# maruscia/fastkmer

Hardware: AMD Instinct MI355X
Metric: input bases/sec (whole node), k=28 short reads, 1/2/4/8 GPUs (higher is better)
Workload: dtype u64; 1 GPU; BASELINE configs[1]: k=28 m=10 x=3 B=2048, 1 GB synthetic 100 bp reads per GPU; k=28, m=10, x=3, B=2048, useHT=0, sequenceType=0, fasta_bytes_per_gpu=999999906, bases_per_gpu=877192900, parallelism=one GPU

## Files before the change

fastkmer_amd/__init__.py:

```python
from __future__ import annotations

import ctypes
import dataclasses
import os
import re

import numpy as np

_PKG = os.path.dirname(os.path.abspath(__file__))
LIB_PATH = os.environ.get("FASTKMER_LIB") or os.path.join(_PKG, "lib", "libfastkmer.so")
CLI_PATH = os.path.join(_PKG, "bin", "fastkmer-cli")
HEADER_PATH = os.path.join(os.path.dirname(_PKG), "include", "fastkmer.h")

FK_OK = 0
ERRORS = {-1: "FK_E_INVALID", -2: "FK_E_STATE", -3: "FK_E_DEVICE", -4: "FK_E_NOMEM", -5: "FK_E_IO",
          -6: "FK_E_RANGE", -7: "FK_E_COMM"}
ABI_VERSION = 3


class FastKmerError(RuntimeError):
    def __init__(self, code: int, message: str):
        super().__init__(f"{ERRORS.get(code, code)}: {message}")
        self.code = code

# ... 121 lines not shown
        "fk_bin_sizes_range": (ctypes.c_int, [P, ctypes.c_uint32, ctypes.c_uint32, P]),
        "fk_get_bin_range": (ctypes.c_int, [P, I32, ctypes.c_uint32, ctypes.c_uint32, P, P, SZ,
                                            ctypes.POINTER(SZ)]),
        "fk_write_bins_range": (ctypes.c_int, [P, ctypes.c_char_p, ctypes.c_uint32, ctypes.c_uint32]),
        "fk_compare": (ctypes.c_int, [P, P, P, SZ, SZ]),
        "fk_compare_device": (ctypes.c_int, [P, P, P, SZ, SZ]),
        "fk_bin_sizes_joined": (ctypes.c_int, [P, P, ctypes.c_uint32, ctypes.c_uint32, ctypes.c_uint32,
                                               ctypes.c_uint32, P]),
        "fk_get_bin_joined": (ctypes.c_int, [P, P, I32, ctypes.c_uint32, ctypes.c_uint32, ctypes.c_uint32,
                                             ctypes.c_uint32, P, P, P, SZ, ctypes.POINTER(SZ)]),
        "fk_map_bin_kmers": (ctypes.c_int, [P, P]),
        "fk_lpt_owners": (ctypes.c_int, [P, I32, I32, P]),
        "fk_set_bin_owners": (ctypes.c_int, [P, P, P]),
        "fk_bin_owners": (ctypes.c_int, [P, P]),
        "fk_signature_slots": (U64, [P]),
        "fk_signature_counts": (ctypes.c_int, [P, P, U64]),
        "fk_write_bin_signatures": (ctypes.c_int, [P, P, U64, ctypes.c_char_p]),
        "fk_find_bin_signatures": (ctypes.c_int, [P, ctypes.c_char_p]),
        "fk_comm_unique_id": (ctypes.c_int, [P]),
        "fk_comm_init": (ctypes.c_int, [P, P]),
        "fk_comm_init_local": (ctypes.c_int, [P, I32]),
        "fk_comm_transport": (ctypes.c_char_p, [P]),
        "fk_comm_allreduce_u64": (ctypes.c_int, [P, P, SZ]),
        "fk_balance_bins": (ctypes.c_int, [P, ctypes.c_char_p, SZ]),
        "fk_balance_bins_file": (ctypes.c_int, [P, ctypes.c_char_p, I32, I32, ctypes.c_double]),
        "fk_exchange_plan": (ctypes.c_int, [I32, I32, P, P, U64, P, P, P, P, P]),
        "fk_debug_map_cycles": (ctypes.c_int, [P, I32]),
        "fk_debug_comm_hold": (ctypes.c_int, [P, I32]),
        "fk_debug_comm_release": (ctypes.c_int, [P]),
        "fk_debug_comm_held": (ctypes.c_int, [P]),
        "fk_debug_fingerprint_bits": (ctypes.c_int, [I32, I32]),
        "fk_debug_wave_count": (ctypes.c_int, [I32, I32, I32, ctypes.c_uint32, ctypes.c_uint32, I32, P,
                                               ctypes.c_uint32, P, P, P]),
    }
    for name, (res, args) in sig.items():
        fn = getattr(L, name)
        fn.restype = res
        fn.argtypes = args
    if L.fk_abi_version() != ABI_VERSION:
        raise RuntimeError(f"{LIB_PATH} has ABI version {L.fk_abi_version()}, this binding mirrors {ABI_VERSION}: "
                           "rebuild it (python -m fastkmer_amd.build)")
    _lib = L
    return L


def _check(rc: int) -> None:
    if rc != FK_OK:
        raise FastKmerError(rc, lib().fk_last_error().decode(errors="replace"))


def make_config(k: int, m: int, x: int = 3, B: int = 2048, use_ht: bool = False, sequence_type: int = 0,
                write: bool = False, n_ranks: int = 1, rank: int = 0, device: int = -1) -> fk_config:
    c = fk_config()
    lib().fk_config_init(ctypes.byref(c))
    c.k, c.m, c.x, c.B = k, m, x, B
    c.use_ht, c.sequence_type, c.write = int(bool(use_ht)), sequence_type, int(bool(write))
    c.n_ranks, c.rank, c.device = n_ranks, rank, device
    return c


def validate(**kw) -> None:
    c = make_config(**kw)
    _check(lib().fk_config_validate(ctypes.byref(c)))


def clamped_bins(m: int, B: int) -> int:
# ... 505 lines not shown
            return ""
        return "".join(lines) + ("" if self.use_ht else "EOF")

    def write_bins(self, out_dir: str, min_count: int = 1, max_count: int | None = None) -> None:
        rg = _count_range(min_count, max_count)
        if rg is None:
            _check(lib().fk_write_bins(self._h, out_dir.encode()))
        else:
            _check(lib().fk_write_bins_range(self._h, out_dir.encode(), rg[0], rg[1]))

    def signature_counts(self, out=None):
        import torch
        n = lib().fk_signature_slots(self._h)
        if out is None:
            out = torch.empty(n, dtype=torch.int64, device=self._torch_device())
        if out.numel() < n or out.dtype != torch.int64 or not out.is_cuda or not out.is_contiguous():
            raise ValueError(f"signature counts need a contiguous device int64 tensor of {n} entries")
        _check(lib().fk_signature_counts(self._h, ctypes.c_void_p(out.data_ptr()), out.numel()))
        return out

    def write_bin_signatures(self, counts, out_dir: str) -> None:
        _check(lib().fk_write_bin_signatures(self._h, ctypes.c_void_p(counts.data_ptr()), counts.numel(),
                                             out_dir.encode()))

    def _torch_device(self):
        import torch
        return torch.device("cuda", self._device if self._device >= 0 else torch.cuda.current_device())

    def stats(self) -> dict:
        st = fk_stats()
        _check(lib().fk_get_stats(self._h, ctypes.byref(st)))
        return {n: getattr(st, n) for n, _ in fk_stats._fields_}


def debug_wave_count(keys: np.ndarray, k: int, F: int, c0: int, c1: int, slots: int, device: int = 0):
    kw = 1 if k <= 32 else 2
    keys = np.ascontiguousarray(keys, dtype=np.uint64).reshape(-1, kw)
    n = len(keys)
    ok = np.zeros(n * kw, dtype=np.uint64)
    oc = np.zeros(n, dtype=np.uint32)
    nout = ctypes.c_uint32(0)
    _check(lib().fk_debug_wave_count(device, k, F, c0, c1, slots, keys.ctypes.data, n, ok.ctypes.data,
                                     oc.ctypes.data, ctypes.byref(nout)))
    u = nout.value
    return (ok[:u] if kw == 1 else ok[:2 * u].reshape(-1, 2)), oc[:u]


def comm_unique_id() -> bytes:
    buf = ctypes.create_string_buffer(COMM_ID_BYTES)
    _check(lib().fk_comm_unique_id(buf))
    return buf.raw


def comm_init_local(counters) -> None:
    arr = (ctypes.c_void_p * len(counters))(*[c._h.value for c in counters])
    _check(lib().fk_comm_init_local(arr, len(counters)))


def exchange_plan(sent, received, record_bytes: int):
    snd = np.ascontiguousarray(sent, dtype=np.uint64)
    rcv = np.ascontiguousarray(received, dtype=np.uint64)
    if snd.ndim != 2 or snd.shape != rcv.shape or snd.shape[1] % 2 != 1:
        raise ValueError("sent / received must be [n_ranks, 2 * parts + 1] arrays of one shape")
    n, parts = snd.shape[0], (snd.shape[1] - 1) // 2
    so, sb, ro, rb = (np.zeros(n, dtype=np.uint64) for _ in range(4))
    fin = ctypes.c_int32(0)
    _check(lib().fk_exchange_plan(n, parts, snd.ctypes.data, rcv.ctypes.data, record_bytes, so.ctypes.data,
                                  sb.ctypes.data, ro.ctypes.data, rb.ctypes.data, ctypes.byref(fin)))
    return so, sb, ro, rb, bool(fin.value)


def lpt_owners(sizes, n_ranks: int) -> np.ndarray:
    sz = np.ascontiguousarray(sizes, dtype=np.uint64)
    owner = np.zeros(len(sz), dtype=np.int32)
    _check(lib().fk_lpt_owners(sz.ctypes.data, len(sz), n_ranks, owner.ctypes.data))
    return owner
# ... 26 lines not shown
```

fastkmer_amd/csrc/fk_api.cpp:

```cpp
#include <errno.h>
#include <fcntl.h>
#include <unistd.h>
#include <stdarg.h>
#include <stdio.h>
#include <string.h>
#include <sys/stat.h>

#include <unordered_map>
#include <chrono>
#include <cstdlib>
#include <cstring>
#include <thread>

#include "fk_ctx.h"
#include "fk_split.h"

static thread_local std::string g_err;
int fk::set_err(int code, const char *fmt, ...) {
    char buf[1024];
    va_list ap;
    va_start(ap, fmt);
    vsnprintf(buf, sizeof(buf), fmt, ap);
    va_end(ap);
    g_err = buf;
// ... 198 lines not shown
    c->Bc = clamp_bins(cfg->m, cfg->B);
    c->G = (uint32_t)cfg->n_ranks;
    c->nlb = (uint32_t)((c->Bc - cfg->rank + (int)c->G - 1) / (int)c->G);
    if (cfg->rank >= c->Bc) c->nlb = 0;
    c->W = cfg->k <= 32 ? 2 : 3;
    c->KW = cfg->k <= 32 ? 1 : 2;
    c->fm = make_fastmod((uint32_t)c->Bc);
    auto env = [](const char *name) -> const char * {
        const char *v = getenv(name);
        return v && v[0] ? v : nullptr;
    };
    if (const char *v = env("FASTKMER_PIECE_BYTES")) {
        c->piece_bytes = std::max(1ull << 16, strtoull(v, nullptr, 10));
        c->piece_bytes_set = true;
    }
    if (const char *v = env("FASTKMER_PIECE_CUTS")) {
        c->st_cuts.clear();
        c->xst_cuts.clear();
        for (const char *q = v; *q;) {
            char *e = nullptr;
            const double f = strtod(q, &e);
            if (e == q) break;
            if (f > 0.0 && f < 1.0 && c->st_cuts.size() < STAGE_MAXP - 1) c->st_cuts.push_back(f), c->xst_cuts.push_back(f);
            c->cuts_env = true;
            q = *e == ',' ? e + 1 : e;
        }
    }
    if (const char *v = env("FASTKMER_INGEST_SEG")) c->ingest_seg = std::max(1ull << 16, strtoull(v, nullptr, 10));
    if (const char *v = env("FASTKMER_DEBUG_LARGE_BUCKETS")) c->force_large = v[0] == '1';
    if (const char *v = env("FASTKMER_DEBUG_CELL_TARGET")) c->cell_target = (uint32_t)atoi(v);
    if (const char *v = env("FASTKMER_DEBUG_MID_PARTS")) c->mid_parts = atoi(v);
    if (const char *v = env("FASTKMER_DEBUG_SPLIT_RETRY")) c->split_retry = v[0] == '1';
    if (const char *v = env("FASTKMER_DEBUG_SPECTRUM_WIDE")) c->spectrum_wide = v[0] == '1';
    if (const char *v = env("FASTKMER_X2_L1")) c->x2_l1 = atoi(v);
    if (const char *v = env("FASTKMER_FUSED")) c->fused = atoi(v);
#ifdef FK_PROBES
    if (const char *v = env("FASTKMER_DEBUG_PHASE")) c->dbg_phase = atoi(v);
    if (const char *v = env("FASTKMER_FUSED_PROBE")) c->fused_probe = atoi(v);
    if (const char *v = env("FASTKMER_SPLIT_MAP")) c->split_map = atoi(v);
#endif
    if (cfg->device >= 0) {
        if (cfg->device >= ndev) {
            delete c;
            return set_err(FK_E_DEVICE, "device %d out of range (%d devices)", cfg->device, ndev);
        }
        c->device = cfg->device;
    } else {
        (void)hipGetDevice(&c->device);
    }
    DeviceGuard dg_(c->device);
    {
        int cur = -1;
        if (hipGetDevice(&cur) != hipSuccess || cur != c->device) {
            (void)hipGetLastError();
            delete c;
            return set_err(FK_E_DEVICE, "cannot select device %d", c->device);
        }
    }
    e = hipStreamCreateWithFlags(&c->stream, hipStreamNonBlocking);
    if (e != hipSuccess) {
        delete c;
        return set_err(FK_E_DEVICE, "hipStreamCreate: %s", hipGetErrorString(e));
    }
    c->own_stream = true;
    e = hipStreamCreateWithFlags(&c->copy_stream, hipStreamNonBlocking);
    if (e == hipSuccess) e = hipEventCreateWithFlags(&c->seg_ev, hipEventDisableTiming);
// ... 40 lines not shown
FK_EXPORT void fk_destroy(fk_ctx *c) {
    if (!c) return;
    DeviceGuard dg_(c->device);
    if (c->hold_flag) __atomic_store_n(c->hold_flag, 1u, __ATOMIC_RELEASE);
    if (c->copy_stream) (void)hipStreamSynchronize(c->copy_stream);
    if (c->stream) (void)hipStreamSynchronize(c->stream);
    if (c->xstage) (void)hipStreamSynchronize(c->xstage);
    if (c->tier_side) (void)hipStreamSynchronize(c->tier_side);
    DevBuf *bufs[] = {&c->fasta_own, &c->tile_last_nl, &c->tile_off,
                      &c->npos_dev, &c->codes, &c->valid, &c->records, &c->counters, &c->sig_status, &c->sig_kmers, &c->tcnt, &c->rec_hdr, &c->rec_pos, &c->rec_code, &c->tstat, &c->map_vslots,
                      &c->precs, &c->chunks, &c->bin_chunk_begin, &c->hpieces, &c->hpiece_first, &c->hpiece_tot, &c->chunk_nk, &c->grp_table,
                      &c->chunk_base, &c->lp, &c->scratch,
                      &c->cell_total, &c->cell_base, &c->flags, &c->flag_scan, &c->buckets, &c->keys,
                      &c->out_keys, &c->out_counts, &c->bucket_unique, &c->dense_off, &c->dense_keys,
                      &c->dense_counts, &c->bin_off, &c->misc, &c->tier_list, &c->mid, &c->sc_total,
                      &c->sp_base, &c->sp_keys, &c->sp_subs, &c->sp_par, &c->sp_fb, &c->mid_fb};
    for (DevBuf *b : bufs) release(*b);
    c->vw.release_all();
    release(c->fq_ws);
    release(c->fq_info);
    for (auto &e : c->fq_evs)
        if (e) (void)hipEventDestroy(e);
    c->fq_pin.release();
    for (int i = 0; i < 2; ++i) {
        if (c->pinned[i]) (void)hipHostFree(c->pinned[i]);
        if (c->pin_ev[i]) (void)hipEventDestroy(c->pin_ev[i]);
    }
    if (c->comm_stream) (void)hipStreamSynchronize(c->comm_stream);
    delete c->comm;
    c->comm = nullptr;
    c->pin_up.release();
    c->pin_down.release();
    c->pin_tier.release();
    c->file_pin[0].release();
    c->file_pin[1].release();
    if (c->tier_ev) (void)hipEventDestroy(c->tier_ev);
    if (c->pin_up_ev) (void)hipEventDestroy(c->pin_up_ev);
    if (c->cmp_ev) (void)hipEventDestroy(c->cmp_ev);
    if (c->hold_flag) (void)hipHostFree(c->hold_flag);
    release(c->xsend);
    release(c->xrecv);
    for (auto &e : c->xev)
        if (e) (void)hipEventDestroy(e);
    for (auto &e : c->seg_evs)
        if (e) (void)hipEventDestroy(e);
    for (auto &e : c->map_evs)
        if (e) (void)hipEventDestroy(e);
    if (c->emit_ev) (void)hipEventDestroy(c->emit_ev);
    if (c->comm_stream) (void)hipStreamDestroy(c->comm_stream);
    if (c->xstage) (void)hipStreamSynchronize(c->xstage), (void)hipStreamDestroy(c->xstage);
    if (c->xstage_ev) (void)hipEventDestroy(c->xstage_ev);
    if (c->ws_x.ptr) (void)hipFree(c->ws_x.ptr);
    c->dest.release_all();
    c->part.release_all();
    c->binhist.release_all();
    release(c->d_owner);
    release(c->d_local);
    if (c->ws.ptr) (void)hipFree(c->ws.ptr);
    for (auto &ev : c->ev)
        if (ev) (void)hipEventDestroy(ev);
    for (auto &ev : c->st_ev)
        if (ev) (void)hipEventDestroy(ev);
    for (int p = 0; p < STAGE_MAXP; ++p) release(c->st_keys[p]), release(c->st_cb[p]);
    release(c->st_total);
    release(c->piece_starts);
    if (c->seg_ev) (void)hipEventDestroy(c->seg_ev);
    for (auto &ev : c->h2d_ev)
        if (ev) (void)hipEventDestroy(ev);
    if (c->tier_side) (void)hipStreamSynchronize(c->tier_side), (void)hipStreamDestroy(c->tier_side);
    for (auto &ev : c->side_ev)
        if (ev) (void)hipEventDestroy(ev);
    if (c->copy_stream) (void)hipStreamDestroy(c->copy_stream);
    if (c->own_stream && c->stream) (void)hipStreamDestroy(c->stream);
    delete c;
}

FK_EXPORT int fk_set_stream(fk_ctx *c, void *s) {
    if (!c) return set_err(FK_E_INVALID, "null ctx");
    DeviceGuard dg_(c->device);
    if (c->own_stream && c->stream) {
        (void)hipStreamSynchronize(c->stream);
        (void)hipStreamDestroy(c->stream);
    }
    c->stream = (hipStream_t)s;
    c->own_stream = false;
    return FK_OK;
}

FK_EXPORT size_t fk_record_bytes(const fk_ctx *c) { return c ? (size_t)c->W * 8 : 0; }
FK_EXPORT int32_t fk_num_bins(const fk_ctx *c) { return c ? c->Bc : 0; }

static void reset_results(fk_ctx *c) {
    c->mapped = false;
    c->have_result = false;
    c->gapped = c->dense_ready = false;
    c->distinct = 0;
    c->h_bin_off.clear();
// ... 1022 lines not shown
};

static hipError_t launch_wave_tier(const BucketCount &t, hipStream_t s) {
    if (t.c->KW == 1)
        return launch_bucket_count64_wave(t.src, t.buckets(), t.nbuckets, t.k, t.out_keys(), t.out_counts(), t.unique(),
                                          nullptr, s, t.ordered);
    return launch_bucket_count128_wave(t.src, t.buckets(), t.nbuckets, t.k, t.out_keys(), t.out_counts(), t.unique(), s,
                                       t.ordered);
}
static hipError_t launch_wave_mid(const BucketCount &t, const uint32_t *list, uint32_t n, hipStream_t s) {
    if (t.c->KW == 1)
        return launch_bucket_count64_wave_mid(t.src, t.buckets(), list, n, t.k, t.out_keys(), t.out_counts(), t.unique(),
                                              s, t.ordered);
    return launch_bucket_count128_wave_mid(t.src, t.buckets(), list, n, t.k, t.out_keys(), t.out_counts(), t.unique(), s,
                                           t.ordered);
}
static hipError_t launch_split(const BucketCount &t, const uint32_t *l1, uint32_t nl, SubBucket *subs,
                               unsigned int *counts, uint32_t *fb, hipStream_t s) {
    fk_ctx *c = t.c;
    return launch_bucket_split64(t.src, t.buckets(), t.lists, 0, l1, nl, c->sp_base.as<uint64_t>(),
                                 c->sp_keys.as<uint64_t>(), subs, c->sp_par.as<SplitParent>(), counts, fb, fb + nl,
                                 t.cap, t.k, t.src.F, s, c->split_retry);
}
static hipError_t launch_split(const BucketCount &t, const uint32_t *l1, uint32_t nl, SubBucket128 *subs,
                               unsigned int *counts, uint32_t *fb, hipStream_t s) {
    fk_ctx *c = t.c;
    return launch_bucket_split128(t.src, t.buckets(), l1, nl, c->sp_base.as<uint64_t>(), c->sp_keys.as<uint64_t>(), subs,
                                  c->sp_par.as<SplitParent>(), counts, fb, fb + nl, t.cap, t.k, t.src.F, s,
                                  c->split_retry);
}
static hipError_t launch_sub_count_seq(const BucketCount &t, const uint32_t *l1, uint32_t nl, const SubBucket *subs,
                                       hipStream_t s) {
    return launch_sub_count64_seq(t.buckets(), l1, nl, t.c->sp_par.as<SplitParent>(), subs, t.c->sp_keys.as<uint64_t>(),
                                  t.out_keys(), t.out_counts(), t.unique(), s, t.ordered);
}
static hipError_t launch_sub_count_seq(const BucketCount &t, const uint32_t *l1, uint32_t nl, const SubBucket128 *subs,
                                       hipStream_t s) {
    return launch_sub_count128_seq(t.buckets(), l1, nl, t.c->sp_par.as<SplitParent>(), subs, t.c->sp_keys.as<uint64_t>(),
                                   t.out_keys(), t.out_counts(), t.unique(), s, t.ordered);
}

static int block_tier(const BucketCount &t, const uint32_t *list, uint32_t n, hipStream_t s) {
    fk_ctx *c = t.c;
    if (c->KW == 1)
        HIP_TRY(launch_bucket_count64(t.src, t.buckets(), n, t.k, t.out_keys(), t.out_counts(), t.unique(),
                                      c->misc.as<unsigned long long>() + 1, t.cap, 99, list, s, 0));
    else
        HIP_TRY(launch_bucket_sort(2, t.src, t.buckets(), n, t.k, t.out_keys(), t.out_counts(), t.unique(),
                                   c->misc.as<unsigned long long>() + 1, t.cap, list, s, 0));
    return FK_OK;
}

static int bucket_cut(BucketCount &t, const SortedPlan &pl, uint64_t total_kmers, const uint64_t *cell_total,
                      const uint64_t *cell_base) {
    fk_ctx *c = t.c;
    const CountBufs &B = t.B;
    const hipStream_t cs = t.cut.s;
    const int F = pl.F;
    const uint32_t cap = pl.cap;
    const uint64_t ncell_all = (uint64_t)c->nlb << F;
    FK_TRY(ensure(*B.flags, ncell_all * 4));
    FK_TRY(ensure(*B.flag_scan, (ncell_all + 1) * 8));
    FK_TRY(ensure(c->misc, 64));
    if (pl.tiered)
        HIP_TRY(launch_bucket_flags_greedy(cell_total, c->nlb, F, pl.wave_cap, -1, B.flags->as<uint32_t>(), cs));
    else
        HIP_TRY(launch_bucket_flags(cell_base, cell_total, c->nlb, F, cap / 4, cap - cap / 4, B.flags->as<uint32_t>(), cs));
    HIP_TRY(scan_excl_sum_u32_to_u64(B.flags->as<uint32_t>(), B.flag_scan->as<uint64_t>(), ncell_all,
                                     B.flag_scan->as<uint64_t>() + ncell_all, *t.cut.ws, cs));
    uint64_t nbuckets = 0;
    HIP_TRY(hipMemcpyAsync(&nbuckets, B.flag_scan->as<uint64_t>() + ncell_all, 8, hipMemcpyDeviceToHost, cs));
    HIP_TRY(hipStreamSynchronize(cs));
    htrace("sorted: nbuckets read");
    t.nbuckets = nbuckets;
    FK_TRY(ensure(*B.buckets, nbuckets * sizeof(Bucket)));
    FK_TRY(ensure(t.okb, total_kmers * 8 * c->KW));
    FK_TRY(ensure(*B.out_counts, total_kmers * 4));
    FK_TRY(ensure(*B.bucket_unique, (nbuckets + 1) * 8));
    HIP_TRY(launch_bucket_write(cell_base, B.flags->as<uint32_t>(), B.flag_scan->as<uint64_t>(), c->nlb, F, nbuckets,
                                total_kmers, B.buckets->as<Bucket>(), cs));
    BucketSrc &src = t.src;
    src.F = F;
    if (src.np > 0) FK_TRY(ensure(*B.piece_starts, nbuckets * sizeof(PieceStarts)));
    HIP_TRY(launch_bucket_finish(src, B.buckets->as<Bucket>(), nbuckets, c->nlb, total_kmers,
                                 src.np > 0 ? B.piece_starts->as<PieceStarts>() : nullptr, cs));
    if (src.np > 0) src.starts = B.piece_starts->as<PieceStarts>();
    HIP_TRY(hipMemsetAsync(c->misc.p, 0, 64, cs));
    c->stats.buckets = nbuckets;
    c->stats.fine_bits = (uint64_t)F;
    c->stats.heavy_keys = 0;
    c->stats.split_buckets = c->stats.sub_buckets = 0;
    return FK_OK;
}

static int wave_tier(BucketCount &t, uint32_t wave_cap) {
    fk_ctx *c = t.c;
    const hipStream_t s = t.s.s, cs = t.cut.s, hs = t.heavy.s;
    FK_TRY(ensure(*t.B.tier_list, t.nbuckets * 8));
    t.lists = t.B.tier_list->as<uint32_t>();
    HIP_TRY(launch_bucket_tiers(t.buckets(), t.nbuckets, wave_cap, t.mid_cap(), t.unique(), t.lists,
                                c->misc.as<unsigned int>(), c->misc.as<unsigned long long>() + 3, cs));
    if (c->pin_tier.ensure(64)) return set_err(FK_E_NOMEM, "hipHostMalloc failed");
    HIP_TRY(hipMemcpyAsync(c->pin_tier.p, c->misc.p, 32, hipMemcpyDeviceToHost, cs));
    HIP_TRY(hipEventRecord(c->tier_ev, cs));
    if (cs != s) {
        HIP_TRY(hipEventRecord(c->side_ev[0], cs));
        HIP_TRY(hipStreamWaitEvent(s, c->side_ev[0], 0));
    }
    HIP_TRY(hipEventRecord(c->side_ev[3], s));
    HIP_TRY(hipStreamWaitEvent(hs, c->side_ev[3], 0));
    HIP_TRY(launch_wave_tier(t, s));
    HIP_TRY(hipEventSynchronize(c->tier_ev));
    t.ntier[0] = c->pin_tier.as<uint32_t>()[0], t.ntier[1] = c->pin_tier.as<uint32_t>()[1];
    t.listed_keys = c->pin_tier.as<uint64_t>()[3];
    htrace("sorted: tiers read");
    c->stats.heavy_keys = t.listed_keys;
    c->stats.block_buckets = t.ntier[0];
// ... 430 lines not shown
    c->have_result = false;
    const uint32_t nlb = c->nlb;
    if ((uint32_t)parts_per_seg < nlb) return set_err(FK_E_INVALID, "%d parts per segment < %u local bins",
                                                      parts_per_seg, nlb);
    HIP_TRY(hipEventRecord(c->ev[4], s));
    std::vector<std::vector<std::pair<uint64_t, uint64_t>>> ranges(nlb);
    std::vector<uint64_t> bkm(nlb, 0);
    uint64_t off = 0;
    for (int32_t sg = 0; sg < nseg; ++sg) {
        for (int32_t lb = 0; lb < parts_per_seg; ++lb) {
            const uint64_t n = seg_records[(uint64_t)sg * parts_per_seg + lb];
            if (n && (uint32_t)lb >= nlb) return set_err(FK_E_INVALID, "records for local bin %d of %u", lb, nlb);
            if (n) {
                ranges[lb].push_back({off, off + n});
                bkm[lb] += seg_kmers[(uint64_t)sg * parts_per_seg + lb];
            }
            off += n;
        }
    }
    if (off != nrecv)
        return set_err(FK_E_INVALID, "segment table holds %llu records, buffer %llu", (unsigned long long)off,
                       (unsigned long long)nrecv);
    return reduce_ranges(c, (const uint64_t *)d_recv, nrecv, ranges, bkm, t0);
}


static void pieces_reset(fk_ctx *c) {
    c->st_np = 0;
    c->st_cut = 0;
    c->st_kmers = 0;
    c->pieces_void = false;
    c->tiles_counted = 0;
    c->segs_counted = 0;
}

static uint32_t stage_maxp(const fk_ctx *c) { return c->KW == 2 ? (uint32_t)STAGE_MAXP128 : (uint32_t)STAGE_MAXP; }
static const std::vector<double> &local_cuts(const fk_ctx *c) {
    if (!c->cuts_env && c->KW == 1 && c->job_bytes >= (4ull << 30) && STAGE_MAXP >= 5) return c->st_cuts5;
    return c->st_cuts;
}

static bool staged_eligible(const fk_ctx *c) { return staged_ok(c) && c->G == 1 && !c->comm; }

static int staged_expand_chunks(fk_ctx *c, StreamWs on, hipStream_t cut, uint32_t nchunks,
                                const std::vector<uint64_t> &bkm, double frac) {
    hipStream_t s = on.s;
    const uint32_t p = c->st_np;
    uint64_t pk = 0, maxb = 0;
    for (uint64_t v : bkm) pk += v, maxb = std::max(maxb, v);
    if (pk == 0) return FK_OK;
    if (p == 0) {
        const double scale = frac > 0.0 ? std::max(1.0, 1.0 / frac) : 2.0;
        c->st_plan = sorted_plan(c, (uint64_t)((double)maxb * scale));
        if (!c->st_plan.tiered || !c->st_plan.two_level)
            return set_err(FK_E_STATE, "staged pieces need the tiered two-level count");
    }
    SortedPlan pl = c->st_plan;
    HIP_TRY(hipEventRecord(c->st_ev[4 * p + 2], s));
    FK_TRY(sorted_expand(c, on, cut, pl, nchunks, pk, c->st_keys[p], c->st_cb[p]));
    const uint64_t ncell_all = (uint64_t)c->nlb << c->st_plan.F;
    FK_TRY(ensure(c->st_total, ncell_all * 8));
    if (cut) {
        HIP_TRY(hipStreamWaitEvent(cut, c->side_ev[2], 0));
        HIP_TRY(launch_add_u64(c->st_total.as<uint64_t>(), c->cell_total.as<uint64_t>(), ncell_all, p == 0, cut));
    } else {
        HIP_TRY(launch_add_u64(c->st_total.as<uint64_t>(), c->cell_total.as<uint64_t>(), ncell_all, p == 0, s));
// ... 2 lines not shown
    c->st_kmers += pk;
    c->st_np = p + 1;
    htrace("staged: piece expanded");
    return FK_OK;
}

static int staged_expand(fk_ctx *c, StreamWs on, hipStream_t cut, const RecSrc &src, double frac) {
    const uint32_t p = c->st_np;
    if (p >= stage_maxp(c)) return set_err(FK_E_STATE, "more than %u staged pieces", stage_maxp(c));
    uint64_t nrecv = 0;
    std::vector<Chunk> chunks;
    std::vector<uint32_t> bcb;
    std::vector<uint64_t> bkm;
    FK_TRY(partition_src(c, on, src, nrecv, chunks, bcb, bkm, c->st_ev[4 * p], c->st_ev[4 * p + 1]));
    return staged_expand_chunks(c, on, cut, (uint32_t)chunks.size(), bkm, frac);
}

static int staged_count(fk_ctx *c, hipStream_t cut) {
    const double t0 = now_ms();
    const StreamWs on = c->main_on();
    hipStream_t s = on.s;
    const SortedPlan pl = c->st_plan;
    const uint32_t nlb = c->nlb;
    const uint64_t ncell_all = (uint64_t)nlb << pl.F;
    HIP_TRY(hipEventRecord(c->ev[6], s));
    std::swap(c->cell_total, c->st_total);
    FK_TRY(ensure(c->cell_base, (ncell_all + 1) * 8));
    const hipStream_t cs = cut ? cut : s;
    if (cut) HIP_TRY(hipStreamWaitEvent(cut, c->side_ev[2], 0));
    HIP_TRY(scan_excl_sum_u64(c->cell_total.as<uint64_t>(), c->cell_base.as<uint64_t>(), ncell_all,
                              c->cell_base.as<uint64_t>() + ncell_all, *on.ws, cs));
    BucketSrc src{nullptr, pl.F};
    src.np = (int)c->st_np;
    for (uint32_t p = 0; p < c->st_np; ++p) {
        src.pk[p] = c->st_keys[p].as<uint64_t>();
        src.pcb[p] = c->st_cb[p].as<uint64_t>();
    }
    FK_TRY(sorted_count(c, on, cut, pl, src, c->st_kmers));
    HIP_TRY(hipEventRecord(c->ev[7], s));
    FK_TRY(read_bin_offsets(c, s));
    htrace("staged: bin offsets read");
    double mp = 0.0, mx = 0.0;
    for (uint32_t p = 0; p < c->st_np; ++p) {
        mp += ev_ms(c->st_ev[4 * p], c->st_ev[4 * p + 1]);
        mx += ev_ms(c->st_ev[4 * p + 2], c->st_ev[4 * p + 3]);
    }
    c->stats.ms_partition = mp;
    c->stats.ms_count = mx + ev_ms(c->ev[6], c->ev[7]);
    c->stats.pieces_counted = c->st_np;
    count_done(c, c->nrec, t0);
    return FK_OK;
}

static bool local_piece_due(const fk_ctx *c, uint64_t tiles) {
    constexpr uint64_t MIN_PIECE = 256ull << 20;
    if (c->st_np >= stage_maxp(c) - 1) return false;
    const uint64_t tile = fm_tile_bytes(FUSED_NT);
    if (c->job_bytes && !c->piece_bytes_set) {
        const std::vector<double> &cuts = local_cuts(c);
        if (c->job_bytes < 2 * MIN_PIECE || c->st_cut >= cuts.size()) return false;
        const uint64_t end = (uint64_t)(cuts[c->st_cut] * (double)c->job_bytes);
        return tiles * tile >= end && (tiles - c->tiles_counted) * tile >= MIN_PIECE / 2;
    }
    return c->st_np < 3 && (tiles - c->tiles_counted) * tile >= c->piece_bytes;
}

static int local_maybe_piece(fk_ctx *c, uint64_t tiles, hipEvent_t mapped) {
    if (!staged_eligible(c) || c->pieces_void || !local_piece_due(c, tiles)) return FK_OK;
    const StreamWs on = c->stage_on();
    hipStream_t s = on.s;
    HIP_TRY(hipStreamWaitEvent(s, mapped, 0));
    uint64_t h[4] = {0, 0, 0, 0};
    HIP_TRY(hipMemcpyAsync(h, c->counters.p, 32, hipMemcpyDeviceToHost, s));
    HIP_TRY(hipStreamSynchronize(s));
    if (h[2]) {
        c->pieces_void = true;
        return FK_OK;
    }
    const uint64_t t0 = c->tiles_counted, nt = tiles - t0;
    const RecSrc src = fused_src(c, t0, nt, nt * map_fused_tcap());
    c->tiles_counted = tiles;
    c->st_cut += 1;
    FK_TRY(staged_expand(c, on, nullptr, src,
                         c->job_bytes ? (double)(nt * fm_tile_bytes(FUSED_NT)) / (double)c->job_bytes : 0.0));
    HIP_TRY(hipEventRecord(c->xstage_ev, s));
    return FK_OK;
}


enum : uint64_t { XF_FINAL = 1, XF_RETRACT = 2 };

static int plan_step(uint32_t G, uint32_t L, const uint64_t *sent, const uint64_t *got, uint64_t rb, uint64_t *soff,
                     uint64_t *sbytes, uint64_t *roff, uint64_t *rbytes, bool *all_final) {
    const size_t msg = 2 * (size_t)L + 1;
    uint64_t so = 0, ro = 0;
    bool fin = true;
    for (uint32_t d = 0; d < G; ++d) {
        uint64_t ns = 0, nr = 0;
        for (uint32_t lb = 0; lb < L; ++lb) {
            ns += sent[d * msg + lb];
            nr += got[d * msg + lb];
        }
        const uint64_t fs = sent[d * msg + 2 * L], fr = got[d * msg + 2 * L];
        if ((fs | fr) & ~(XF_FINAL | XF_RETRACT)) return set_err(FK_E_INVALID, "exchange step: unknown flag bits");
        if ((fr & XF_RETRACT) && !(fr & XF_FINAL))
            return set_err(FK_E_INVALID, "exchange step: rank %u retracts outside its last piece", d);
        fin = fin && (fr & XF_FINAL);
        soff[d] = so;
        sbytes[d] = ns * rb;
        roff[d] = ro;
        rbytes[d] = nr * rb;
        so += ns * rb;
        ro += nr * rb;
    }
    *all_final = fin;
    return FK_OK;
}
// ... 296 lines not shown
}

static int finish_local(fk_ctx *c);

FK_EXPORT int fk_finish(fk_ctx *c) {
    htrace("fk_finish: enter");
    if (!c) return set_err(FK_E_INVALID, "null ctx");
    if (c->comm) {
        DeviceGuard dg_(c->device);
        const int rc = finish_exchange(c);
        return rc ? comm_fail(c, rc) : rc;
    }
    return note_held(c, finish_local(c));
}

static int finish_local(fk_ctx *c) {
    if (c->G != 1)
        return set_err(FK_E_STATE, "fk_finish over %u ranks needs a communicator (fk_comm_init); or use "
                                   "fk_map/fk_map_emit/fk_reduce", c->G);
    FK_TRY(fk_map(c, nullptr));
    DeviceGuard dg_(c->device);
    if (c->st_np && c->rec_tiled && !c->pieces_void && c->tiles_counted <= c->rec_tiles) {
        int rc = FK_OK;
        const hipStream_t cut = c->rec_tiles > c->tiles_counted ? c->tier_side : nullptr;
        if (cut) HIP_TRY(hipEventRecord(c->side_ev[2], c->stream));
        if (c->rec_tiles > c->tiles_counted) {
            const uint64_t t0 = c->tiles_counted, nt = c->rec_tiles - t0;
            rc = staged_expand(c, c->main_on(), cut, fused_src(c, t0, nt, nt * map_fused_tcap()),
                               c->job_bytes ? (double)(nt * fm_tile_bytes(FUSED_NT)) / (double)c->job_bytes : 0.0);
        }
        if (rc == FK_OK) rc = staged_count(c, cut);
        if (cut) (void)hipStreamSynchronize(cut);
        FK_TRY(rc);
        pieces_reset(c);
        return FK_OK;
    }
    pieces_reset(c);
    return reduce_src(c, map_src(c));
}

static int attach_comm(fk_ctx *c, fk::Comm *comm) {
    DeviceGuard dg_(c->device);
    if (!c->comm_stream) HIP_TRY(hipStreamCreateWithFlags(&c->comm_stream, hipStreamNonBlocking));
    if (!c->xstage) HIP_TRY(hipStreamCreateWithFlags(&c->xstage, hipStreamNonBlocking));
    if (!c->xstage_ev) HIP_TRY(hipEventCreateWithFlags(&c->xstage_ev, hipEventDisableTiming));
    if (!c->emit_ev) HIP_TRY(hipEventCreateWithFlags(&c->emit_ev, hipEventDisableTiming));
    c->comm = comm;
    if (!c->piece_bytes_set) c->piece_bytes = 1ull << 30;
    FK_TRY(fk_set_grouped_emit(c, 1));
    xch_reset(c);
    return FK_OK;
}

FK_EXPORT int fk_comm_unique_id(uint8_t *id) {
    if (!id) return set_err(FK_E_INVALID, "null argument");
    std::string err;
    if (fk::comm_unique_id(id, err)) return set_err(FK_E_DEVICE, "%s", err.c_str());
    return FK_OK;
}

FK_EXPORT int fk_comm_init(fk_ctx *c, const uint8_t *id) {
    if (!c || !id) return set_err(FK_E_INVALID, "null argument");
    if (c->comm) return set_err(FK_E_STATE, "the context already has a communicator");
    DeviceGuard dg_(c->device);
    std::string err;
    fk::Comm *comm = fk::comm_create_rccl(id, (int)c->G, c->cfg.rank, c->device, err);
    if (!comm) return set_err(FK_E_DEVICE, "%s", err.c_str());
    const int rc = attach_comm(c, comm);
    if (rc) {
// ... 160 lines not shown
    }
    __atomic_store_n(c->hold_flag, 0u, __ATOMIC_RELEASE);
    void *dflag = nullptr;
    HIP_TRY(hipHostGetDevicePointer(&dflag, c->hold_flag, 0));
    int khz = 0;
    HIP_TRY(hipDeviceGetAttribute(&khz, hipDeviceAttributeWallClockRate, c->device));
    const uint64_t ticks = (uint64_t)max_seconds * (uint64_t)std::max(khz, 100000) * 1000ull;
    const hipStream_t cs2 = c->comm->counts_stream();
    for (hipStream_t st : {c->comm_stream, cs2})
        if (st) HIP_TRY(launch_hold_stream(static_cast<const uint32_t *>(dflag), ticks, st));
    return FK_OK;
}

FK_EXPORT int fk_debug_fingerprint_bits(int32_t device, int32_t bits) {
    DeviceGuard dg_(device);
    HIP_TRY(set_fingerprint_bits(bits));
    return FK_OK;
}

FK_EXPORT int fk_debug_comm_held(fk_ctx *c) {
    if (!c || !c->comm_stream) return 0;
    DeviceGuard dg_(c->device);
    const hipError_t e = hipStreamQuery(c->comm_stream);
    if (e != hipErrorNotReady) (void)hipGetLastError();
    return e == hipErrorNotReady ? 1 : 0;
}

FK_EXPORT int fk_debug_comm_release(fk_ctx *c) {
    if (!c) return set_err(FK_E_INVALID, "null ctx");
    if (c->hold_flag) __atomic_store_n(c->hold_flag, 1u, __ATOMIC_RELEASE);
    return FK_OK;
}

FK_EXPORT int fk_debug_wave_count(int32_t device, int32_t k, int32_t F, uint32_t c0, uint32_t c1, int32_t slots,
                                  const uint64_t *keys, uint32_t n, uint64_t *out_keys, uint32_t *out_counts,
                                  uint32_t *n_out) {
    if (!keys || !out_keys || !out_counts || !n_out || k < 1 || k > 63 || F < 1 || F > MAX_FINE_BITS || c1 <= c0 ||
        c1 > (1u << F))
        return set_err(FK_E_INVALID, "bad argument");
    const int KW = k <= 32 ? 1 : 2;
    const uint32_t cap = KW == 1 ? WAVE_BUCKET_CAP : WAVE128_BUCKET_CAP;
    if (n == 0 || n > cap) return set_err(FK_E_RANGE, "a wave bucket holds 1..%u keys", cap);
    if (slots != (int32_t)(KW == 1 ? WAVE_SLOTS : 384))
        return set_err(FK_E_INVALID, "slots: %u (k <= 32) or 384 (k > 32)", WAVE_SLOTS);
    const int sh = 2 * k - F;
    for (uint32_t i = 0; i < n; ++i) {
        const uint64_t hi = KW == 1 ? 0 : keys[2 * i], lo = KW == 1 ? keys[i] : keys[2 * i + 1];
        const uint64_t cell = sh >= 64 ? (hi >> (sh - 64)) : (sh == 0 ? lo : ((hi << (64 - sh)) | (lo >> sh)));
        if ((KW == 1 && k < 32 && (lo >> (2 * k)) != 0) || cell < c0 || cell >= c1)
            return set_err(FK_E_RANGE, "key %u lies outside cells [%u, %u)", i, c0, c1);
    }
    DeviceGuard dg_(device);
    TempBuf dk, dok, doc, du, db;
    FK_TRY(ensure(dk, (uint64_t)n * 8 * KW));
    FK_TRY(ensure(dok, (uint64_t)n * 8 * KW));
    FK_TRY(ensure(doc, (uint64_t)n * 4));
    FK_TRY(ensure(du, 16));
    FK_TRY(ensure(db, sizeof(Bucket)));
    const Bucket b{0, n, 0, c0, c1};
    int rc = FK_OK;
    hipError_t e = hipMemcpy(dk.p, keys, (uint64_t)n * 8 * KW, hipMemcpyHostToDevice);
    if (e == hipSuccess) e = hipMemcpy(db.p, &b, sizeof(Bucket), hipMemcpyHostToDevice);
    if (e == hipSuccess)
        e = KW == 1 ? launch_bucket_count64_wave(BucketSrc{dk.as<uint64_t>(), F}, db.as<Bucket>(), 1, k, dok.as<uint64_t>(),
                                                 doc.as<uint32_t>(), du.as<uint64_t>(), nullptr, nullptr)
                    : launch_bucket_count128_wave(BucketSrc{dk.as<uint64_t>(), F}, db.as<Bucket>(), 1, k, dok.as<uint64_t>(),
                                                  doc.as<uint32_t>(), du.as<uint64_t>(), nullptr);
    uint64_t U = 0;
    if (e == hipSuccess) e = hipMemcpy(&U, du.p, 8, hipMemcpyDeviceToHost);
    if (e == hipSuccess && U <= n) e = hipMemcpy(out_keys, dok.p, U * 8 * KW, hipMemcpyDeviceToHost);
    if (e == hipSuccess && U <= n) e = hipMemcpy(out_counts, doc.p, U * 4, hipMemcpyDeviceToHost);
    if (e != hipSuccess) rc = set_err(FK_E_DEVICE, "%s", hipGetErrorString(e));
    else if (U > n) rc = set_err(FK_E_INVALID, "bucket reported %llu distinct keys of %u", (unsigned long long)U, n);
    *n_out = (uint32_t)U;
    return rc;
}

FK_EXPORT int fk_debug_map_cycles(uint64_t *out16, int32_t reset) {
    if (!out16) return set_err(FK_E_INVALID, "null argument");
    const hipError_t e = map_fused_cycles(reinterpret_cast<unsigned long long *>(out16), reset != 0);
    if (e == hipErrorNotSupported) {
        (void)hipGetLastError();
        return set_err(FK_E_STATE, "phase stamps exist only in a library built with -DFK_PROBES");
    }
    HIP_TRY(e);
    return FK_OK;
}

FK_EXPORT int fk_get_stats(fk_ctx *c, fk_stats *out) {
    if (!c || !out) return set_err(FK_E_INVALID, "null argument");
    *out = c->stats;
    return FK_OK;
}


FK_EXPORT uint64_t fk_signature_slots(const fk_ctx *c) { return c ? (1ull << (2 * c->cfg.m)) + 1ull : 0ull; }

FK_EXPORT int fk_signature_counts(fk_ctx *c, void *d_counts, uint64_t n_counts) {
    if (!c || !d_counts) return set_err(FK_E_INVALID, "null argument");
    DeviceGuard dg_(c->device);
    const uint64_t slots = fk_signature_slots(c);
    if (n_counts < slots)
        return set_err(FK_E_RANGE, "signature counts hold %llu entries, need 4^m + 1 = %llu",
                       (unsigned long long)n_counts, (unsigned long long)slots);
    if (c->pm_active && !c->pm_last_seen)
        return set_err(FK_E_STATE, "fk_signature_counts inside a streamed input: finish it with fk_ingest(..., last = 1)");
    hipStream_t s = c->stream;
    const uint64_t n = c->d_fasta ? c->n_fasta : 0;
// ... 102 lines not shown
```

fastkmer_amd/csrc/fk_count_sorted.inc:

```


struct ExpandLds {
    uint64_t s0[NT], s1[NT], s2[NT];
    uint32_t first[NT];
    uint8_t owner[NT / 64][64 * SIG_PPT];
};

template <int W, int KW, typename Fn>
__device__ __forceinline__ void for_each_chunk_kmer(const uint64_t *__restrict__ rec, const Chunk &ch, int k,
                                                    ExpandLds &e, Fn fn) {
    const int lane = threadIdx.x & 63, wid = threadIdx.x >> 6;
    const uint64_t nrec = ch.rec_end - ch.rec_begin;
    const uint64_t rounds = (nrec + NT - 1) / NT;
    for (uint64_t rd = 0; rd < rounds; ++rd) {
        const uint64_t i = ch.rec_begin + rd * NT + threadIdx.x;
        uint32_t n = 0;
        if (i < ch.rec_end) {
            RecView<W> r;
            r.load(rec, i);
            n = r.n;
            e.s0[threadIdx.x] = r.s0;
            e.s1[threadIdx.x] = r.s1;
            if (W == 3) e.s2[threadIdx.x] = r.s2;
        }
// ... 360 lines not shown
    }
    const uint64_t g0 = ((uint64_t)b.lbin << src.F) + b.c0, g1 = ((uint64_t)b.lbin << src.F) + b.c1;
    uint32_t acc = 0;
#pragma unroll
    for (int q = 0; q < NPC; ++q) {
        if (q == 0 || q < src.np) {
            const uint64_t s0 = src.pcb[q][g0], s1 = src.pcb[q][g1];
            v.b[q] = src.pk[q] + KW * ((int64_t)s0 - (int64_t)acc);
            v.p[q] = q ? acc : 0u;
            acc += (uint32_t)(s1 - s0);
        } else {
            v.b[q] = v.b[q - 1];
            v.p[q] = ~0u;
        }
    }
    return v;
}

template <int KW = 1>
__device__ __forceinline__ BucketView bucket_view_starts(const BucketSrc &src, const PieceStarts &ps) {
    BucketView v;
    v.b[0] = src.pk[0] + KW * ps.s[0];
    v.p[0] = 0;
#pragma unroll
    for (int q = 1; q < stage_npc<KW>(); ++q) {
        v.b[q] = src.pk[q] + KW * ((int64_t)ps.s[q] - (int64_t)ps.pre[q]);
        v.p[q] = ps.pre[q];
    }
    return v;
}

template <bool PIECES>
__global__ __launch_bounds__(NT) void k_bucket_finish(BucketSrc src, Bucket *__restrict__ buckets, uint64_t nb,
                                                      uint32_t nlbins, uint64_t total_keys,
                                                      PieceStarts *__restrict__ out) {
    const uint64_t i = (uint64_t)blockIdx.x * NT + threadIdx.x;
    const bool mine = i < nb;
    const uint32_t ncell = 1u << src.F;
    Bucket b{};
    uint64_t e_beg = total_keys, g1 = (uint64_t)nlbins << src.F;
    if (mine) {
        b = buckets[i];
        if (i + 1 < nb) {
            const Bucket nx = buckets[i + 1];
            e_beg = nx.begin;
            g1 = ((uint64_t)nx.lbin << src.F) + nx.c0;
        }
        buckets[i].n = (uint32_t)(e_beg - b.begin);
        buckets[i].c1 = (g1 >> src.F) == b.lbin ? (uint32_t)(g1 & (ncell - 1)) : ncell;
    }
    if constexpr (PIECES) {
        const uint64_t g0 = ((uint64_t)b.lbin << src.F) + b.c0;
        const bool own_end = (threadIdx.x & 63) == 63 || i + 1 >= nb;
        PieceStarts ps;
        uint32_t acc = 0;
#pragma unroll
        for (int p = 0; p < STAGE_MAXP; ++p) {
            if (p < src.np) {
                const uint64_t s0 = mine ? src.pcb[p][g0] : 0;
                uint64_t s1 = (uint64_t)__shfl_down((long long)s0, 1, 64);
                if (mine && own_end) s1 = src.pcb[p][g1];
                ps.s[p] = s0;
                ps.pre[p] = acc;
                acc += (uint32_t)(s1 - s0);
            } else {
                ps.s[p] = 0;
                ps.pre[p] = ~0u;
            }
        }
        if (mine) out[i] = ps;
    }
}

hipError_t launch_bucket_finish(const BucketSrc &src, Bucket *buckets, uint64_t nb, uint32_t nlbins,
                                uint64_t total_keys, PieceStarts *out, hipStream_t s) {
    if (!nb) return hipSuccess;
    const unsigned grid = (unsigned)((nb + NT - 1) / NT);
    if (src.np > 0)
        k_bucket_finish<true><<<grid, NT, 0, s>>>(src, buckets, nb, nlbins, total_keys, out);
    else
        k_bucket_finish<false><<<grid, NT, 0, s>>>(src, buckets, nb, nlbins, total_keys, out);
    return hipGetLastError();
}


template <class T>
__device__ __forceinline__ T ldg_nt(const void *p) {
    typedef const __attribute__((address_space(1))) T *gp;
    return __builtin_nontemporal_load((gp)(uintptr_t)p);
}


template <int KW = 1>
__device__ __forceinline__ const uint64_t *bucket_key_ptr(const BucketView &v, uint32_t i) {
    uintptr_t a = (uintptr_t)v.b[0] + (uintptr_t)i * (8u * KW);
#pragma unroll
    for (int q = 1; q < stage_npc<KW>(); ++q) a += i >= v.p[q] ? (uintptr_t)v.b[q] - (uintptr_t)v.b[q - 1] : 0;
    return reinterpret_cast<const uint64_t *>(a);
}

struct RowBases {
    uintptr_t base;
    uint64_t inner;
};
template <int KW = 1>
__device__ __forceinline__ RowBases row_bases(const BucketView &v, uint32_t first_row = 0) {
    const uint32_t r0 = (first_row + (threadIdx.x & 63)) * 64u;
    uintptr_t a = (uintptr_t)v.b[0];
    bool inner = false;
#pragma unroll
    for (int q = 1; q < stage_npc<KW>(); ++q) {
        a = r0 >= v.p[q] ? (uintptr_t)v.b[q] : a;
        inner = inner || (r0 < v.p[q] && r0 + 63u >= v.p[q]);
    }
    return RowBases{a, __ballot(inner)};
}
template <int KW = 1>
__device__ __forceinline__ const uint64_t *row_key_ptr(const BucketView &v, const RowBases &rb, int row, uint32_t i) {
    if ((rb.inner >> row) & 1ull) return bucket_key_ptr<KW>(v, i);
    const uint32_t lo = (uint32_t)__builtin_amdgcn_readlane((int)(uint32_t)rb.base, row);
    const uint32_t hi = (uint32_t)__builtin_amdgcn_readlane((int)(uint32_t)((uint64_t)rb.base >> 32), row);
    return reinterpret_cast<const uint64_t *>((((uint64_t)hi << 32) | lo) + (uintptr_t)i * (8u * KW));
}

constexpr int GB = 8;



constexpr uint32_t HCAP = 2048;
constexpr uint32_t HSLOTS = 2 * HCAP;
constexpr uint32_t HSPT = HSLOTS / NT;
constexpr int UIPT = HCAP / NT;
constexpr uint32_t RANK_MAX = HCAP - 3 * NT / 2 - 2;
constexpr uint64_t REDO = ~0ull;
constexpr uint64_t EMPTY_KEY = ~0ull;
constexpr uint32_t BLOCK_SPLIT_GROUP = 64;

__device__ __forceinline__ uint32_t hslot(uint64_t key) {
    return (uint32_t)((key * 0x9e3779b97f4a7c15ull) >> 52) & (HSLOTS - 1);
}

template <uint32_t HC, uint32_t HS, bool STREAM = false>
__global__ __launch_bounds__(NT) void k_bucket_count64(BucketSrc src, const Bucket *__restrict__ buckets, int k,
                                                       uint64_t *__restrict__ out_keys,
                                                       uint32_t *__restrict__ out_counts, uint64_t *bucket_unique,
                                                       unsigned long long *oversize, uint32_t small_limit,
                                                       int dbg_phase, const uint32_t *__restrict__ list,
                                                       uint32_t skip_le = 0) {
    constexpr uint32_t HSPT_ = HS / NT;
    constexpr int UIPT_ = HC / NT;
    constexpr uint32_t RANK_MAX_ = (HC < HS - HC ? HC : HS - HC) - 3 * NT / 2 - 2;
    static_assert(HC <= 65535 && 2 * HC <= HS + HS / 2 && HS % NT == 0, "u16 counts, load <= 3/4");
    static_assert((HS - HC) * 8 >= 16 * NT * 4 && HC % NT == 0, "radix counters (tile_rank) fit above HC");
    constexpr bool POW2 = (HS & (HS - 1)) == 0;
    constexpr int HBITS = __builtin_ctz(HS);
    __shared__ unsigned long long s_k[HS];
    __shared__ uint16_t s_c[HS];
    __shared__ uint32_t s_tmp[NT / 64];
    uint32_t *const s_cnt = reinterpret_cast<uint32_t *>(&s_k[HC]);
    __shared__ uint64_t s_red[2][NT / 64];
    static_assert(!STREAM || HS - HC >= NT * GB, "a batch of new keys leaves the table below full");
    __shared__ uint32_t s_nu, s_ovf;
    __shared__ unsigned long long s_spl[NT];
    const uint32_t qi = list ? list[blockIdx.x] : blockIdx.x;
    const Bucket b = buckets[qi];
    if (b.n <= skip_le) return;
    const BucketView bv = bucket_view(src, b);
    if (!STREAM && (b.n > HC || b.n > small_limit)) {
        if (threadIdx.x == 0) {
            bucket_unique[qi] = REDO;
            atomicAdd(oversize, 1ull);
        }
        return;
    }
    if (b.n == 0) {
        if (threadIdx.x == 0) bucket_unique[qi] = 0;
        return;
    }
    for (uint32_t s = threadIdx.x; s < HS; s += NT) {
        s_k[s] = EMPTY_KEY;
        s_c[s] = 0;
    }
    if (STREAM && threadIdx.x == 0) s_nu = 0, s_ovf = 0;
    __syncthreads();
    for (uint32_t i0 = 0; i0 < b.n; i0 += NT * GB) {
        if constexpr (STREAM) {
            if (i0) {
                __syncthreads();
                if (s_ovf || s_nu > HC) {
                    if (threadIdx.x == 0) atomicAdd(oversize, 1ull);
                    return;
                }
            }
        }
        uint64_t kk[GB];
#pragma unroll
        for (int q = 0; q < GB; ++q) {
            const uint32_t i = i0 + q * NT + threadIdx.x;
            kk[q] = i < b.n ? *bucket_key_ptr(bv, i) : EMPTY_KEY;
        }
        if (dbg_phase == 0) {
            uint64_t acc = 0;
#pragma unroll
            for (int q = 0; q < GB; ++q) acc += kk[q];
            if (acc == 42) out_counts[b.begin] = 1;
            continue;
        }
#pragma unroll
        for (int q = 0; q < GB; ++q) {
            const uint64_t key = kk[q];
            if (key == EMPTY_KEY) continue;
            uint32_t s = POW2 ? (uint32_t)((key * 0x9e3779b97f4a7c15ull) >> (64 - HBITS))
                              : (uint32_t)((((key * 0x9e3779b97f4a7c15ull) >> 32) * HS) >> 32);
            for (;;) {
                unsigned long long cur = s_k[s];
                if (cur == EMPTY_KEY) cur = atomicCAS(&s_k[s], EMPTY_KEY, (unsigned long long)key);
                if (cur == EMPTY_KEY || cur == key) {
                    const uint32_t old =
                        atomicAdd(reinterpret_cast<uint32_t *>(&s_c[s & ~1u]), 1u << (16 * (s & 1u)));
                    if constexpr (STREAM) {
                        if (cur == EMPTY_KEY) atomicAdd(&s_nu, 1u);
                        if (((old >> (16 * (s & 1u))) & 0xffffu) == 0xffffu) s_ovf = 1u;
                    }
                    break;
                }
                s = POW2 ? (s + 1) & (HS - 1) : (s + 1 == HS ? 0u : s + 1);
            }
        }
    }
    if (dbg_phase < 99 && threadIdx.x == 0) bucket_unique[qi] = 0;
    if (dbg_phase == 0) return;
    __syncthreads();
    if constexpr (STREAM) {
        if (s_ovf || s_nu > HC) {
            if (threadIdx.x == 0) atomicAdd(oversize, 1ull);
            return;
        }
    }
    if (dbg_phase == 1) return;
    uint64_t tk[HSPT_];
    uint16_t tc[HSPT_];
    uint32_t occ = 0;
#pragma unroll
    for (uint32_t q = 0; q < HSPT_; ++q) {
        tk[q] = s_k[q * NT + threadIdx.x];
        tc[q] = s_c[q * NT + threadIdx.x];
        occ += tk[q] != EMPTY_KEY;
    }
    uint32_t U;
    uint32_t u = block_excl_sum<uint32_t>(occ, s_tmp, &U);
#pragma unroll
    for (uint32_t q = 0; q < HSPT_; ++q) {
        if (tk[q] != EMPTY_KEY) {
            s_k[u] = tk[q];
            s_c[u] = tc[q];
// ... 352 lines not shown
    for (uint32_t p = lane; p < U; p += 64) {
        const unsigned long long kx = s_gk[p];
        const uint32_t g = (uint32_t)((kx - lo) >> gsh);
        const uint32_t gv = s_grp[g], n = gv >> 16;
        if (n > RANK_BIG) continue;
        const uint32_t g1 = gv & 0xffffu, g0 = g1 - n;
        uint32_t r = g0;
        for (uint32_t j = g0; j < g1; j += 4) {
            const unsigned long long a0 = s_gk[j], a1 = s_gk[j + 1], a2 = s_gk[j + 2], a3 = s_gk[j + 3];
            r += (uint32_t)(a0 < kx) + (uint32_t)(j + 1 < g1 && a1 < kx) + (uint32_t)(j + 2 < g1 && a2 < kx) +
                 (uint32_t)(j + 3 < g1 && a3 < kx);
        }
        out_keys[begin + r] = kx;
        out_counts[begin + r] = s_gc[p];
#ifdef FK_PROBES
        it += g1 - g0;
        uint32_t w = g1 - g0;
#pragma unroll
        for (int d = 32; d > 0; d >>= 1) w = max(w, (uint32_t)__shfl_xor((int)w, d, 64));
        wall += w;
#endif
    }
#ifdef FK_PROBES
    it = wave_incl_sum<uint32_t>(it);
    if (lane == 63) {
        atomicAdd(&g_rank_probe[0], (unsigned long long)it);
        atomicAdd(&g_rank_probe[1], (unsigned long long)U);
        atomicAdd(&g_rank_probe[2], 1ull);
        atomicAdd(&g_rank_probe[3], (unsigned long long)wall);
    }
#endif
}

template <uint32_t CAP, uint32_t SL, bool ORD = true, int WKPT = WaveCfg<CAP>::KPT, int NROW = WKPT>
__device__ __forceinline__ uint32_t wave_count_keys(WaveLds<CAP, SL> &w, uint64_t begin, uint32_t n, uint64_t lo,
                                                int span_bits, uint64_t q, const uint64_t (&kk)[NROW],
                                                uint64_t *__restrict__ out_keys, uint32_t *__restrict__ out_counts,
                                                uint64_t *__restrict__ uniq) {
    const int lane = threadIdx.x & 63;
    unsigned long long *s_k = w.k;
    uint16_t *s_c = w.c;
    uint16_t *s_list = w.list;
    if (n == 0) {
        if (lane == 0 && uniq) uniq[q] = 0;
        return 0;
    }
    {
        ulonglong2 *k2 = reinterpret_cast<ulonglong2 *>(s_k);
#pragma unroll
        for (uint32_t r = 0; r < (SL / 2 + 63) / 64; ++r)
            if (r * 64 + lane < SL / 2) k2[r * 64 + lane] = make_ulonglong2(EMPTY_KEY, EMPTY_KEY);
        uint4 *c4 = reinterpret_cast<uint4 *>(s_c);
#pragma unroll
        for (uint32_t r = 0; r < (SL / 8 + 63) / 64; ++r)
            if (r * 64 + lane < SL / 8) c4[r * 64 + lane] = make_uint4(0, 0, 0, 0);
    }
    wave_lds_sync();
    static_assert(NROW == WKPT || (NROW > WKPT && SL - CAP >= 64), "a row's new keys fit above CAP");
    uint32_t sl[NROW];
#pragma unroll
    for (int j = 0; j < NROW; ++j) sl[j] = wslot<SL>(kk[j]);
    uint32_t U = 0;
#pragma unroll
    for (int j = 0; j < NROW; ++j) {
        bool over = false;
        if constexpr (NROW > WKPT) over = U > CAP;
        const uint64_t key = over ? EMPTY_KEY : kk[j];
        bool fresh = false;
        if (key != EMPTY_KEY) {
            uint32_t s = sl[j];
            for (;;) {
                const unsigned long long prev = atomicCAS(&s_k[s], EMPTY_KEY, (unsigned long long)key);
                fresh = prev == EMPTY_KEY;
                if (fresh || prev == key) break;
                s = s + 1 == SL ? 0u : s + 1;
            }
            atomicAdd(reinterpret_cast<uint32_t *>(&s_c[s & ~1u]), 1u << (16 * (s & 1u)));
            sl[j] = s;
        }
        const uint64_t m = __ballot(fresh);
        if (fresh) {
            const uint32_t at = U + __builtin_amdgcn_mbcnt_hi((uint32_t)(m >> 32), __builtin_amdgcn_mbcnt_lo((uint32_t)m, 0u));
            if (NROW == WKPT || at < CAP) s_list[at] = (uint16_t)sl[j];
        }
        U += (uint32_t)__popcll(m);
    }
    wave_lds_sync();
    if constexpr (NROW > WKPT) {
        if (U > CAP) return ~0u;
    }
#if defined(FK_W64_STOP) && FK_W64_STOP == 1
    if (lane == 0 && uniq) uniq[q] = U;
    return U;
#endif
    uint64_t tk[WKPT];
    uint16_t tc[WKPT];
#pragma unroll
    for (int j = 0; j < WKPT; ++j) {
        const uint32_t i = j * 64 + lane;
        if (i < U) {
            const uint32_t s = s_list[i];
            tk[j] = s_k[s];
            tc[j] = s_c[s];
        }
    }
#if defined(FK_W64_STOP) && FK_W64_STOP == 2
    {
        uint64_t x = 0;
#pragma unroll
        for (int j = 0; j < WKPT; ++j) x ^= (j * 64 + lane < (int)U) ? tk[j] + tc[j] : 0ull;
        if (x == 0x0123456789abcdefull) out_counts[0] = 1u;
        if (lane == 0 && uniq) uniq[q] = U;
        wave_lds_sync();
        return U;
    }
#endif
    if constexpr (!ORD) {
#pragma unroll
        for (int j = 0; j < WKPT; ++j) {
            const uint32_t i = j * 64 + lane;
            if (i < U) {
                out_keys[begin + i] = tk[j];
                out_counts[begin + i] = tc[j];
            }
        }
        if (lane == 0 && uniq) uniq[q] = U;
        wave_lds_sync();
        return U;
    }
    wave_rank64<CAP, WKPT>(s_k, s_c, reinterpret_cast<uint32_t *>(&s_k[CAP]), reinterpret_cast<uint32_t *>(s_list),
                           U, tk, tc, lo, span_bits, begin, out_keys, out_counts);
    if (lane == 0 && uniq) uniq[q] = U;
    wave_lds_sync();
    return U;
}

template <uint32_t CAP, uint32_t SL, bool ORD = true, int WKPT = WaveCfg<CAP>::KPT>
__device__ __forceinline__ void wave_count_bucket(WaveLds<CAP, SL> &w, const Bucket &b, uint64_t q,
                                                  const uint64_t (&kk)[WKPT], int k, int F,
                                                  uint64_t *__restrict__ out_keys, uint32_t *__restrict__ out_counts,
                                                  uint64_t *__restrict__ bucket_unique) {
    const int sh = 2 * k - F;
    const int span_bits = b.n ? (32 - __builtin_clz(b.c1 - b.c0)) + sh : 0;
    wave_count_keys<CAP, SL, ORD, WKPT>(w, b.begin, b.n, (uint64_t)b.c0 << sh, span_bits, q, kk, out_keys,
                                        out_counts, bucket_unique);
}

template <int BPW, uint32_t CAP, uint32_t SL, bool MS = false, bool ORD = true>
__global__ __launch_bounds__(64) void k_bucket_count64_wave(BucketSrc src,
                                                            const Bucket *__restrict__ buckets, uint64_t nbuckets,
                                                            int k, uint64_t *__restrict__ out_keys,
                                                            uint32_t *__restrict__ out_counts,
                                                            uint64_t *__restrict__ bucket_unique,
                                                            const uint32_t *__restrict__ list) {
    constexpr int WKPT = WaveCfg<CAP>::KPT;
    __shared__ __attribute__((aligned(16))) WaveLds<CAP, SL> w;
    const uint64_t q0 = (uint64_t)blockIdx.x * BPW;
    Bucket b[BPW];
    bool mine[BPW];
    uint64_t qq[BPW];
    uint64_t kk[BPW][WKPT];
    const uint64_t *dummy = reinterpret_cast<const uint64_t *>(buckets);
#pragma unroll
    for (int t = 0; t < BPW; ++t) {
        const uint64_t i = q0 + t;
        qq[t] = i < nbuckets ? (list ? (uint64_t)list[i] : i) : 0;
        if (i < nbuckets) b[t] = buckets[qq[t]];
        PieceStarts ps{};
        if constexpr (MS)
            if (src.starts && i < nbuckets) ps = src.starts[qq[t]];
        mine[t] = i < nbuckets && b[t].n <= CAP;
        wave_bucket_load<CAP, MS>(src, b[t], ps, mine[t], kk[t], dummy);
    }
#if defined(FK_W64_STOP) && FK_W64_STOP == 0
    if (!list) {
#pragma unroll
        for (int t = 0; t < BPW; ++t) {
            uint64_t x = 0;
#pragma unroll
            for (int j = 0; j < WKPT; ++j) x ^= kk[t][j];
            if ((threadIdx.x & 63) == 0 && bucket_unique && mine[t]) bucket_unique[qq[t]] = 0;
            if (x == 0x0123456789abcdefull) out_counts[0] = 1u;
        }
        return;
    }
#endif
#pragma unroll
    for (int t = 0; t < BPW; ++t)
        if (mine[t])
            wave_count_bucket<CAP, SL, ORD>(w, b[t], qq[t], kk[t], k, src.F, out_keys, out_counts, bucket_unique);
}

constexpr int FLAGS_NT = 256;
__global__ __launch_bounds__(FLAGS_NT) void k_bucket_flags_greedy(const uint64_t *__restrict__ cell_total, int F,
                                                            uint32_t cap, int period_bits,
                                                            uint32_t *__restrict__ flags) {
    extern __shared__ uint32_t s_t[];
    const uint32_t ncell = 1u << F;
    const uint32_t pmask = period_bits >= 0 ? (1u << period_bits) - 1u : 0xffffffffu;
    const uint64_t *t = cell_total + ((uint64_t)blockIdx.x << F);
    uint32_t *f = flags + ((uint64_t)blockIdx.x << F);
    for (uint32_t c = threadIdx.x; c < ncell; c += FLAGS_NT) {
        const uint64_t v = t[c];
        s_t[c] = v > 0xffffffffull ? 0xffffffffu : (uint32_t)v;
    }
    __syncthreads();
    if (threadIdx.x < 64) {
        const uint32_t seg = (ncell + 63) / 64;
        const uint32_t c0 = threadIdx.x * seg, c1 = min(c0 + seg, ncell);
        uint64_t acc = 0;
        bool prev_big = false;
        for (uint32_t c = c0; c < c1; ++c) {
            const uint32_t v = s_t[c];
            const bool big = v > cap;
            const bool cut = c == c0 || (c & pmask) == 0 || big || prev_big || acc + v > cap;
            acc = cut ? v : acc + v;
            prev_big = big;
            s_t[c] = cut;
        }
    }
    __syncthreads();
    for (uint32_t c = threadIdx.x; c < ncell; c += FLAGS_NT) f[c] = s_t[c];
}
// ... 36 lines not shown
    __syncthreads();
    if (!mine) return;
    uint32_t ob = s_base[0] + (off >> 16), ol = s_base[1] + (off & 0xffffu);
#pragma unroll
    for (int t = 0; t < TIER_IPT; ++t) {
        if (n[t] > wave_cap && n[t] <= block_cap) block_list[ob++] = (uint32_t)(i0 + t);
        if (n[t] > block_cap) large_list[ol++] = (uint32_t)(i0 + t);
    }
}

hipError_t launch_bucket_flags_greedy(const uint64_t *cell_total, uint32_t nlbins, int F, uint32_t cap,
                                      int period_bits, uint32_t *flags, hipStream_t s) {
    if (!nlbins) return hipSuccess;
    hipError_t e = part_lds_attr((const void *)k_bucket_flags_greedy, (size_t)4 << F);
    if (e != hipSuccess) return e;
    k_bucket_flags_greedy<<<nlbins, FLAGS_NT, (size_t)4 << F, s>>>(cell_total, F, cap, period_bits, flags);
    return hipGetLastError();
}

hipError_t launch_bucket_tiers(const Bucket *buckets, uint64_t nb, uint32_t wave_cap, uint32_t block_cap,
                               uint64_t *bucket_unique, uint32_t *lists, unsigned int *counts,
                               unsigned long long *listed_keys, hipStream_t s) {
    if (!nb) return hipSuccess;
    k_bucket_tiers<<<(unsigned)((nb + (uint64_t)NT * TIER_IPT - 1) / ((uint64_t)NT * TIER_IPT)), NT, 0, s>>>(
        buckets, nb, wave_cap, block_cap, bucket_unique, lists, lists + nb, counts, listed_keys);
    return hipGetLastError();
}

hipError_t launch_bucket_count64_wave(const BucketSrc &src, const Bucket *buckets, uint64_t nbuckets, int k,
                                      uint64_t *out_keys, uint32_t *out_counts, uint64_t *bucket_unique,
                                      const uint32_t *list, hipStream_t s, bool ordered) {
    if (!nbuckets) return hipSuccess;
    const unsigned grid = (unsigned)((nbuckets + 1) / 2);
#define FK_W64(MS_, ORD_)                                                                                  \
    k_bucket_count64_wave<2, WAVE_BUCKET_CAP, WAVE_SLOTS, MS_, ORD_><<<grid, 64, 0, s>>>(src, buckets, nbuckets, k, \
                                                                                 out_keys, out_counts,     \
                                                                                 bucket_unique, list)
    if (src.np > 0 && ordered)
        FK_W64(true, true);
    else if (src.np > 0)
        FK_W64(true, false);
    else if (ordered)
        FK_W64(false, true);
    else
        FK_W64(false, false);
#undef FK_W64
    return hipGetLastError();
}

hipError_t launch_bucket_count64_wave_mid(const BucketSrc &src, const Bucket *buckets, const uint32_t *list,
                                          uint64_t nlist, int k, uint64_t *out_keys, uint32_t *out_counts,
                                          uint64_t *bucket_unique, hipStream_t s, bool ordered) {
    if (!nlist) return hipSuccess;
#define FK_W64M(MS_, ORD_)                                                                                  \
    k_bucket_count64_wave<1, WAVE_MID_CAP, WAVE_MID_SLOTS, MS_, ORD_><<<(unsigned)nlist, 64, 0, s>>>( \
        src, buckets, nlist, k, out_keys, out_counts, bucket_unique, list)
    if (src.np > 0 && ordered)
        FK_W64M(true, true);
    else if (src.np > 0)
        FK_W64M(true, false);
    else if (ordered)
        FK_W64M(false, true);
    else
        FK_W64M(false, false);
#undef FK_W64M
    return hipGetLastError();
}



template <bool MS, bool ORD>
__global__ __launch_bounds__(64) void k_bucket_count64_parts(BucketSrc src, const Bucket *__restrict__ buckets,
                                                             const uint32_t *__restrict__ list, int k,
                                                             uint64_t *__restrict__ out_keys,
                                                             uint32_t *__restrict__ out_counts,
                                                             uint64_t *__restrict__ bucket_unique,
                                                             uint32_t *__restrict__ fb, unsigned int *fb_count) {
    constexpr uint32_t CAP = WAVE_BUCKET_CAP, SL = WAVE_SLOTS;
    constexpr int WKPT = WaveCfg<CAP>::KPT, R = 2 * WKPT;
    static_assert(R * 64 == WAVE_MID_CAP && SL >= CAP, "two rounds of the wave tier's keys per lane");
    __shared__ __attribute__((aligned(16))) WaveLds<CAP, SL> w;
    const uint32_t lane = threadIdx.x & 63;
    const uint32_t q = list[blockIdx.x];
    const Bucket b = buckets[q];
    BucketView v{};
    if constexpr (MS) v = src.starts ? bucket_view_starts(src, src.starts[q]) : bucket_view(src, b);
    else v = bucket_view(src, b);
    const uint32_t n = b.n;
    const uint64_t *klast = bucket_key_ptr(v, n - 1);
    const RowBases rb = row_bases(v);
    auto key_at = [&](uint32_t row0, uint32_t i) {
        const uint64_t *pa = row_key_ptr(v, rb, (int)(row0 >> 6), i);
        return ldg_nt<uint64_t>(i < n ? pa : klast);
    };
    unsigned long long x = *bucket_key_ptr(v, (uint32_t)(((uint64_t)lane * n) >> 6));
#pragma unroll
    for (uint32_t kk = 2; kk <= 64; kk <<= 1) {
#pragma unroll
        for (uint32_t j = kk >> 1; j > 0; j >>= 1) {
            const unsigned long long y = (unsigned long long)__shfl_xor((long long)x, (int)j, 64);
            const bool up = (lane & kk) == 0, low = (lane & j) == 0;
            x = (low == up) ? (x < y ? x : y) : (x > y ? x : y);
        }
    }
    const uint32_t P = n <= 768 ? 2u : 3u;
    const unsigned long long sp0 = (unsigned long long)__shfl((long long)x, (int)(64 / P) - 1, 64);
    const unsigned long long sp1 = (unsigned long long)__shfl((long long)x, (int)(2 * 64 / P) - 1, 64);
    auto range_of = [&](unsigned long long key) -> uint32_t {
        return (key > sp0 ? 1u : 0u) + (P == 3 && key > sp1 ? 1u : 0u);
    };
    uint64_t kr[R];
#pragma unroll
    for (int r = 0; r < R; ++r) kr[r] = key_at(r * 64, r * 64 + lane);
    uint32_t c0 = 0, c1 = 0;
#pragma unroll
    for (int r = 0; r < R; ++r) {
        const uint32_t i = r * 64 + lane;
        const unsigned long long key = kr[r];
        const uint32_t g = range_of(key);
        c0 += (i < n && g == 0) ? 1u : 0u;
        c1 += (i < n && g == 1) ? 1u : 0u;
    }
    c0 = wave_incl_sum<uint32_t>(c0), c1 = wave_incl_sum<uint32_t>(c1);
    const uint32_t n0 = (uint32_t)__shfl((int)c0, 63, 64), n1 = (uint32_t)__shfl((int)c1, 63, 64);
    const uint32_t n2 = n - n0 - n1;
    if (n0 > CAP || n1 > CAP || n2 > CAP) {
        if (lane == 0) fb[atomicAdd(fb_count, 1u)] = q;
        return;
    }
    const int sh = 2 * k - src.F;
    const uint64_t klo = (uint64_t)b.c0 << sh, khi = ((uint64_t)b.c1 << sh) - 1ull;
    uint64_t pre = 0;
    for (uint32_t g = 0; g < P; ++g) {
        const uint32_t ng = g == 0 ? n0 : g == 1 ? n1 : n2;
        uint32_t at = 0;
    #pragma unroll
        for (int r = 0; r < R; ++r) {
            const uint32_t i = r * 64 + lane;
            const unsigned long long key = kr[r];
            const bool mine = i < n && range_of(key) == g;
            const uint64_t m = __ballot(mine);
            if (mine)
                w.k[at + __builtin_amdgcn_mbcnt_hi((uint32_t)(m >> 32), __builtin_amdgcn_mbcnt_lo((uint32_t)m, 0u))] = key;
            at += (uint32_t)__popcll(m);
        }
        wave_lds_sync();
        uint64_t kk[WKPT];
#pragma unroll
        for (int j = 0; j < WKPT; ++j) {
            const uint32_t i = j * 64 + lane;
            kk[j] = i < ng ? w.k[i] : EMPTY_KEY;
        }
        wave_lds_sync();
        const uint64_t lo = g == 0 ? klo : (g == 1 ? sp0 : sp1) + 1ull;
        const uint64_t hi = g + 1 == P ? khi : (g == 0 ? sp0 : sp1);
        const int span = hi > lo ? 64 - __builtin_clzll(hi - lo) : 0;
        pre += wave_count_keys<CAP, SL, ORD>(w, b.begin + pre, ng, lo, span, 0, kk, out_keys, out_counts, nullptr);
    }
    if (lane == 0) bucket_unique[q] = pre;
}

hipError_t launch_bucket_count64_parts(const BucketSrc &src, const Bucket *buckets, const uint32_t *list,
                                       uint64_t nlist, int k, uint64_t *out_keys, uint32_t *out_counts,
                                       uint64_t *bucket_unique, uint32_t *fb, unsigned int *fb_count, hipStream_t s,
                                       bool ordered) {
    if (!nlist) return hipSuccess;
#define FK_W64P(MS_, ORD_)                                                                                   \
    k_bucket_count64_parts<MS_, ORD_><<<(unsigned)nlist, 64, 0, s>>>(src, buckets, list, k, out_keys, out_counts, \
                                                                     bucket_unique, fb, fb_count)
    if (src.np > 0 && ordered)
        FK_W64P(true, true);
    else if (src.np > 0)
        FK_W64P(true, false);
    else if (ordered)
        FK_W64P(false, true);
    else
        FK_W64P(false, false);
#undef FK_W64P
    return hipGetLastError();
}
template <bool MS, bool ORD>
__global__ __launch_bounds__(64) void k_bucket_count64_mid512(BucketSrc src, const Bucket *__restrict__ buckets,
                                                              const uint32_t *__restrict__ list, int k,
                                                              uint64_t *__restrict__ out_keys,
                                                              uint32_t *__restrict__ out_counts,
                                                              uint64_t *__restrict__ bucket_unique,
                                                              uint32_t *__restrict__ fb, unsigned int *fb_count) {
    constexpr uint32_t CAP = WAVE_BUCKET_CAP, SL = WAVE_SLOTS;
    constexpr int WKPT = WaveCfg<CAP>::KPT, R = 2 * WKPT;
    static_assert(R * 64 == WAVE_MID_CAP, "two rows of the wave tier's keys per lane cover the mid tier");
    __shared__ __attribute__((aligned(16))) WaveLds<CAP, SL> w;
    const uint32_t q = list[blockIdx.x];
    const Bucket b = buckets[q];
    PieceStarts ps{};
    if constexpr (MS)
        if (src.starts) ps = src.starts[q];
    uint64_t kk[R];
    wave_bucket_load<WAVE_MID_CAP, MS, R>(src, b, ps, true, kk, reinterpret_cast<const uint64_t *>(buckets));
    const int sh = 2 * k - src.F;
    const int span_bits = (32 - __builtin_clz(b.c1 - b.c0)) + sh;
    const uint32_t U = wave_count_keys<CAP, SL, ORD, WKPT, R>(w, b.begin, b.n, (uint64_t)b.c0 << sh, span_bits, q, kk,
                                                              out_keys, out_counts, bucket_unique);
    if (U == ~0u && (threadIdx.x & 63) == 0) fb[atomicAdd(fb_count, 1u)] = q;
}

hipError_t launch_bucket_count64_mid512(const BucketSrc &src, const Bucket *buckets, const uint32_t *list,
                                        uint64_t nlist, int k, uint64_t *out_keys, uint32_t *out_counts,
                                        uint64_t *bucket_unique, uint32_t *fb, unsigned int *fb_count, hipStream_t s,
                                        bool ordered) {
    if (!nlist) return hipSuccess;
#define FK_W64M5(MS_, ORD_)                                                                                    \
    k_bucket_count64_mid512<MS_, ORD_><<<(unsigned)nlist, 64, 0, s>>>(src, buckets, list, k, out_keys, out_counts, \
                                                                      bucket_unique, fb, fb_count)
    if (src.np > 0 && ordered)
        FK_W64M5(true, true);
    else if (src.np > 0)
        FK_W64M5(true, false);
    else if (ordered)
        FK_W64M5(false, true);
    else
        FK_W64M5(false, false);
#undef FK_W64M5
    return hipGetLastError();
}

constexpr uint32_t SPL_TGT = 256;
constexpr uint32_t SPL_OVER = 16;

constexpr uint32_t SPL_SLOT = WAVE_BUCKET_CAP;
__device__ __host__ inline uint64_t split_room(uint32_t n, bool slots) {
    if (!slots) return n;
    uint32_t ns = (n + SPL_TGT - 1) / SPL_TGT;
    ns = ns < 256u ? ns : 256u;
    const uint64_t r = (uint64_t)ns * SPL_SLOT;
    return r > n ? r : n;
}
__global__ void k_listed_sizes(const Bucket *__restrict__ buckets, const uint32_t *__restrict__ list0, uint32_t n0,
                               const uint32_t *__restrict__ list1, uint32_t n1, uint64_t *__restrict__ sizes,
                               bool slots) {
    const uint32_t i = blockIdx.x * blockDim.x + threadIdx.x;
    if (i >= n0 + n1) return;
    sizes[i] = split_room(buckets[i < n0 ? list0[i] : list1[i - n0]].n, slots);
}

hipError_t launch_listed_sizes(const Bucket *buckets, const uint32_t *list0, uint32_t n0, const uint32_t *list1,
                               uint32_t n1, uint64_t *sizes, hipStream_t s, bool slots) {
    if (!(n0 + n1)) return hipSuccess;
    k_listed_sizes<<<(n0 + n1 + NT - 1) / NT, NT, 0, s>>>(buckets, list0, n0, list1, n1, sizes, slots);
    return hipGetLastError();
}

constexpr uint32_t WSPL_MAXS = 256;
static_assert(WSPL_MAXS == 256, "split_room's sub-bucket cap");
constexpr uint32_t WSPL_SMAX = 1024;
constexpr int WSPL_PER = WSPL_MAXS / 64;
constexpr int WSPL_KB = 8;

__global__ __launch_bounds__(64) void k_bucket_split64(BucketSrc src, const Bucket *__restrict__ buckets,
                                                       const uint32_t *__restrict__ list0, uint32_t n0,
                                                       const uint32_t *__restrict__ list1,
                                                       const uint64_t *__restrict__ sbase,
                                                       uint64_t *__restrict__ skeys, SubBucket *__restrict__ subs,
                                                       SplitParent *__restrict__ parents, unsigned int *counts,
                                                       uint32_t *__restrict__ fb0, uint32_t *__restrict__ fb1,
                                                       uint32_t block_cap, int sh, int retry) {
    __shared__ uint64_t s_smp[WSPL_SMAX];
    __shared__ uint32_t s_cnt[WSPL_MAXS];
    const uint32_t lane = threadIdx.x;
    const uint32_t i = blockIdx.x;
    const uint32_t q = i < n0 ? list0[i] : list1[i - n0];
    const Bucket b = buckets[q];
    const BucketView v = (src.np > 0 && src.starts) ? bucket_view_starts(src, src.starts[q]) : bucket_view(src, b);
    uint32_t ns0 = (b.n + SPL_TGT - 1) / SPL_TGT;
    ns0 = ns0 < WSPL_MAXS ? ns0 : WSPL_MAXS;
    uint32_t ns = ns0, nsp = 0, S = 64;
    const uint32_t c0 = lane * WSPL_PER;
    uint32_t cv[WSPL_PER], sum = 0, ne = 0, big = 0, isum = 0, ine = 0, netot = 0, bigmax = 0;
    auto sub_of = [&](uint64_t x) {
        uint32_t lo = 0, len = nsp;
        while (len > 0) {
            const uint32_t half = len >> 1;
            if (s_smp[lo + half] < x) lo += half + 1, len -= half + 1;
            else len = half;
        }
        return lo;
    };
    const uint64_t *klast = bucket_key_ptr(v, b.n - 1);
    RowBases rb{};
    uint32_t rb_first = ~0u;
    auto key_at = [&](uint32_t row0, uint32_t j) {
        const uint32_t row = row0 >> 6;
        if ((row & ~63u) != rb_first) {
            rb_first = row & ~63u;
            rb = row_bases(v, rb_first);
        }
        const uint64_t *pa = row_key_ptr(v, rb, (int)(row & 63u), j);
        return ldg_nt<uint64_t>(j < b.n ? pa : klast);
    };
    const uint64_t sb = sbase[i];
    bool direct = false;
    for (int att = 0; att < 2; ++att) {
        if (att) {
            ns = 2 * ns0 < WSPL_MAXS ? 2 * ns0 : WSPL_MAXS;
            wave_lds_sync();
        }
        S = 64;
        while (S < ns * SPL_OVER && S < WSPL_SMAX) S <<= 1;
        const uint64_t soff = att ? (uint64_t)b.n / (2 * S) : 0;
        for (uint32_t j = lane; j < S; j += 64)
            s_smp[j] = *bucket_key_ptr(v, (uint32_t)(((uint64_t)j * b.n) / S + soff));
        for (uint32_t t = lane; t < WSPL_MAXS; t += 64) s_cnt[t] = 0;
        wave_lds_sync();
        for (uint32_t kk = 2; kk <= S; kk <<= 1) {
            for (uint32_t j = kk >> 1; j > 0; j >>= 1) {
                for (uint32_t t = lane; t < S / 2; t += 64) {
                    const uint32_t a = ((t & ~(j - 1)) << 1) | (t & (j - 1)), c = a + j;
                    const uint64_t x = s_smp[a], y = s_smp[c];
                    if ((x > y) == ((a & kk) == 0)) s_smp[a] = y, s_smp[c] = x;
                }
                wave_lds_sync();
            }
        }
        nsp = ns - 1;
        uint64_t spv[WSPL_PER];
#pragma unroll
        for (int r = 0; r < WSPL_PER; ++r) {
            const uint32_t t = r * 64 + lane;
            if (t < nsp) spv[r] = s_smp[((uint64_t)(t + 1) * S) / ns - 1];
        }
        wave_lds_sync();
#pragma unroll
        for (int r = 0; r < WSPL_PER; ++r) {
            const uint32_t t = r * 64 + lane;
            if (t < nsp) s_smp[t] = spv[r];
        }
        wave_lds_sync();
        for (uint32_t j0 = 0; j0 < b.n; j0 += 64 * WSPL_KB) {
            uint64_t x[WSPL_KB];
#pragma unroll
            for (int r = 0; r < WSPL_KB; ++r) x[r] = key_at(j0 + r * 64, j0 + r * 64 + lane);
#pragma unroll
            for (int r = 0; r < WSPL_KB; ++r)
                if (j0 + r * 64 + lane < b.n) {
                    const uint32_t sub = sub_of(x[r]);
                    const uint32_t at = atomicAdd(&s_cnt[sub], 1u);
                    if (att == 0 && at < SPL_SLOT) skeys[sb + (uint64_t)sub * SPL_SLOT + at] = x[r];
                }
        }
        wave_lds_sync();
        sum = 0, ne = 0, big = 0;
#pragma unroll
        for (int t = 0; t < WSPL_PER; ++t) {
            cv[t] = s_cnt[c0 + t];
            sum += cv[t];
            ne += cv[t] ? 1u : 0u;
            big = cv[t] > big ? cv[t] : big;
        }
        isum = wave_incl_sum<uint32_t>(sum), ine = wave_incl_sum<uint32_t>(ne);
        netot = (uint32_t)__shfl((int)ine, 63, 64);
        bigmax = (uint32_t)__shfl((int)wave_incl_max<uint32_t>(big), 63, 64);
        direct = att == 0;
        if ((bigmax <= WAVE_BUCKET_CAP && !(retry && att == 0)) || ns0 >= WSPL_MAXS) break;
    }
    static_assert(SPL_SLOT >= WAVE_BUCKET_CAP, "a sub-bucket the wave tier takes fits its slot region");
    if (bigmax > WAVE_BUCKET_CAP) {
        if (lane == 0) {
            parents[i] = SplitParent{0u, 0u};
            if (b.n <= block_cap)
                fb0[atomicAdd(&counts[1], 1u)] = q;
            else
                fb1[atomicAdd(&counts[2], 1u)] = q;
        }
        return;
    }
    uint32_t first = 0;
    if (lane == 0) first = atomicAdd(&counts[0], netot);
    first = (uint32_t)__shfl((int)first, 0, 64);
    if (lane == 0) parents[i] = SplitParent{first, netot};
    const uint64_t klo = (uint64_t)b.c0 << sh, khi = ((uint64_t)b.c1 << sh) - 1ull;
    uint32_t off = isum - sum, nei = ine - ne;
#pragma unroll
    for (int t = 0; t < WSPL_PER; ++t) {
        const uint32_t sidx = c0 + t, c = cv[t];
        if (c) {
            const uint64_t lo = sidx == 0 ? klo : s_smp[sidx - 1] + 1ull;
            const uint64_t hi = sidx == nsp ? khi : s_smp[sidx];
            SubBucket d;
            d.src = direct ? sb + (uint64_t)sidx * SPL_SLOT : sb + off;
            d.lo = lo;
            d.n = c;
            d.span = hi > lo ? 64u - (uint32_t)__builtin_clzll(hi - lo) : 0u;
            subs[first + nei] = d;
            ++nei;
        }
        s_cnt[sidx] = off;
        off += c;
    }
    if (direct) return;
    wave_lds_sync();
    for (uint32_t j0 = 0; j0 < b.n; j0 += 64 * WSPL_KB) {
        uint64_t x[WSPL_KB];
#pragma unroll
        for (int r = 0; r < WSPL_KB; ++r) x[r] = key_at(j0 + r * 64, j0 + r * 64 + lane);
#pragma unroll
        for (int r = 0; r < WSPL_KB; ++r)
            if (j0 + r * 64 + lane < b.n) skeys[sb + atomicAdd(&s_cnt[sub_of(x[r])], 1u)] = x[r];
    }
}

hipError_t launch_bucket_split64(const BucketSrc &src, const Bucket *buckets, const uint32_t *list0, uint32_t n0,
                                 const uint32_t *list1, uint32_t n1, const uint64_t *sbase, uint64_t *skeys,
                                 SubBucket *subs, SplitParent *parents, unsigned int *counts, uint32_t *fb0,
                                 uint32_t *fb1, uint32_t block_cap, int k, int F, hipStream_t s, bool retry) {
    if (!(n0 + n1)) return hipSuccess;
    k_bucket_split64<<<n0 + n1, 64, 0, s>>>(src, buckets, list0, n0, list1, sbase, skeys, subs, parents, counts, fb0,
                                            fb1, block_cap, 2 * k - F, retry ? 1 : 0);
    return hipGetLastError();
}

template <bool ORD>
__global__ __launch_bounds__(64) void k_sub_count64_seq(const Bucket *__restrict__ buckets,
                                                        const uint32_t *__restrict__ list,
                                                        const SplitParent *__restrict__ parents,
                                                        const SubBucket *__restrict__ subs,
                                                        const uint64_t *__restrict__ skeys,
                                                        uint64_t *__restrict__ out_keys,
                                                        uint32_t *__restrict__ out_counts,
                                                        uint64_t *__restrict__ bucket_unique) {
    constexpr uint32_t CAP = WAVE_BUCKET_CAP, SL = WAVE_SLOTS;
    constexpr int WKPT = WaveCfg<CAP>::KPT;
    __shared__ __attribute__((aligned(16))) WaveLds<CAP, SL> w;
    const SplitParent P = parents[blockIdx.x];
    if (P.nsub == 0) return;
    const uint32_t q = list[blockIdx.x];
    const uint64_t begin = buckets[q].begin;
    const int lane = threadIdx.x & 63;
    auto load = [&](const SubBucket &d, uint64_t (&kk)[WKPT]) {
#pragma unroll
        for (int jj = 0; jj < WKPT; ++jj) {
            const uint32_t i = jj * 64 + lane;
            const bool ok = i < d.n;
            const uint64_t x = ldg_nt<uint64_t>(&skeys[d.src + (ok ? i : 0u)]);
            kk[jj] = ok ? x : EMPTY_KEY;
        }
    };
    SubBucket d0 = subs[P.first], d1;
    uint64_t ka[WKPT], kb[WKPT];
    load(d0, ka);
    uint64_t pre = 0;
    for (uint32_t j = 0;; ++j) {
        const bool more = j + 1 < P.nsub;
        d1 = subs[P.first + (more ? j + 1 : j)];
        load(d1, kb);
        pre += wave_count_keys<CAP, SL, ORD>(w, begin + pre, d0.n, d0.lo, (int)d0.span, 0, ka, out_keys, out_counts,
                                             nullptr);
        if (!more) break;
        d0 = d1;
#pragma unroll
        for (int jj = 0; jj < WKPT; ++jj) ka[jj] = kb[jj];
    }
    if (lane == 0) bucket_unique[q] = pre;
}

hipError_t launch_sub_count64_seq(const Bucket *buckets, const uint32_t *list, uint32_t nl, const SplitParent *parents,
                                  const SubBucket *subs, const uint64_t *skeys, uint64_t *out_keys,
                                  uint32_t *out_counts, uint64_t *bucket_unique, hipStream_t s, bool ordered) {
    if (!nl) return hipSuccess;
    if (ordered)
        k_sub_count64_seq<true><<<nl, 64, 0, s>>>(buckets, list, parents, subs, skeys, out_keys, out_counts,
                                                  bucket_unique);
    else
        k_sub_count64_seq<false><<<nl, 64, 0, s>>>(buckets, list, parents, subs, skeys, out_keys, out_counts,
                                                   bucket_unique);
    return hipGetLastError();
}


constexpr uint32_t W2CAP = WAVE128_BUCKET_CAP;

template <uint32_t CAP, uint32_t SL>
struct WaveLds128 {
    static_assert(SL >= CAP && SL % 8 == 0, "the table holds every distinct key; cleared 8 counts at a time");
    static_assert((SL - CAP) * 8 >= (CAP > 256 ? 2048u : 1024u), "group arrays above CAP");
    unsigned long long hi[SL], lo[SL];
    uint16_t c[SL];
    uint16_t list[CAP];
};

template <uint32_t SL>
__device__ __forceinline__ uint32_t wslot128(uint64_t hi, uint64_t lo) {
    const uint32_t h = (uint32_t)(((lo ^ (hi * 0xc2b2ae3d27d4eb4full)) * 0x9e3779b97f4a7c15ull) >> 32);
    return (uint32_t)(((uint64_t)h * SL) >> 32);
}

__device__ __forceinline__ void store_key128(uint64_t *out, uint64_t i, uint64_t hi, uint64_t lo) {
    typedef uint64_t u64x2s __attribute__((ext_vector_type(2)));
    u64x2s v;
    v.x = hi;
    v.y = lo;
    reinterpret_cast<u64x2s *>(out)[i] = v;
}

template <uint32_t CAP, int W2KPT>
__device__ __forceinline__ void wave_rank128(unsigned long long *g_hi, unsigned long long *g_lo, uint16_t *g_c,
                                             uint32_t *s_gcnt, uint32_t *s_scnt, uint32_t U, const uint64_t (&th)[W2KPT],
// ... 755 lines not shown
```

fastkmer_amd/csrc/fk_ctx.h:

```cpp
#pragma once

#include <algorithm>
#include <string>
#include <vector>

#include "../../include/fastkmer.h"
#include "fk_comm.h"
#include "fk_internal.h"

#define FK_EXPORT extern "C" __attribute__((visibility("default")))

namespace fk {
int set_err(int code, const char *fmt, ...);
int mkdir_p(const std::string &path);

#define HIP_TRY(expr)                                                                                \
    do {                                                                                             \
        hipError_t e_ = (expr);                                                                      \
        if (e_ != hipSuccess)                                                                        \
            return set_err(e_ == hipErrorOutOfMemory ? FK_E_NOMEM : FK_E_DEVICE, "%s failed: %s (%s:%d)", \
                           #expr, hipGetErrorString(e_), __FILE__, __LINE__);                        \
    } while (0)

#define FK_TRY(expr)             \
// ... 223 lines not shown
    std::vector<hipEvent_t> seg_evs;
    std::vector<hipEvent_t> map_evs;
    std::vector<uint64_t> seg_tiles;
    PinBuf pin_up, pin_down;
    hipEvent_t pin_up_ev = nullptr;
    bool pin_up_busy = false;
    PinBuf pin_tier;
    PinBuf file_pin[2];
    hipEvent_t tier_ev = nullptr;
    bool distinct_pending = false;
    bool gapped = false, dense_ready = false;
    const uint64_t *res_keys = nullptr;
    const uint64_t *res_fs = nullptr;
    uint64_t res_nbuckets = 0;
    int res_F = 0;
    ViewBufs vw;
    hipEvent_t cmp_ev = nullptr;

    bool pieces_void = false;
    uint64_t tiles_counted = 0;
    uint64_t job_bytes = 0;
    uint64_t reserve_bytes = 0;
    size_t segs_counted = 0;
    std::vector<double> st_cuts{0.4, 0.7, 0.9};
    std::vector<double> st_cuts5{0.38, 0.64, 0.82, 0.93};
    bool cuts_env = false;
    std::vector<double> xst_cuts{0.35, 0.65, 0.84};
    uint32_t st_np = 0;
    uint32_t st_cut = 0;
    SortedPlan st_plan;
    uint64_t st_kmers = 0;
    DevBuf st_keys[STAGE_MAXP], st_cb[STAGE_MAXP], st_total, piece_starts;
    hipEvent_t st_ev[4 * STAGE_MAXP] = {};

    fk::Comm *comm = nullptr;
    hipStream_t comm_stream = nullptr;
    uint32_t *hold_flag = nullptr;
    hipStream_t xstage = nullptr;
    hipEvent_t xstage_ev = nullptr;
    ScanWorkspace ws_x;
    StreamWs main_on() { return StreamWs{stream, &ws}; }
    StreamWs stage_on() { return StreamWs{xstage, &ws_x}; }
    hipEvent_t emit_ev = nullptr;
    std::vector<hipEvent_t> xev;
    uint64_t piece_bytes = 512ull << 20;
    bool piece_bytes_set = false;
    uint64_t ingest_seg = 32ull << 20;
    DevBuf xsend, xrecv;
    struct XSeg {
        uint64_t off;
        int32_t sender;
        uint64_t step;
        std::vector<uint64_t> rec, kmer;
    };
    struct Xch {
        bool open = false;
        bool sent_final = false;
        bool all_final = false;
        bool stop_pieces = false;
        uint64_t tiles_sent = 0;
        uint64_t send_used = 0, recv_used = 0;
        uint64_t pieces = 0, bytes_sent = 0, bytes_received = 0, expect_bytes = 0;
        std::vector<XSeg> segs;
    } xch;
};

// ... 14 lines not shown
```

fastkmer_amd/csrc/fk_internal.h:

```cpp
#pragma once

#include <hip/hip_runtime.h>
#include <stdint.h>

#include "fk_common.h"

namespace fk {

constexpr int ENC_NT = 512;
constexpr int ENC_TILE = ENC_NT * 64;
constexpr int SIG_NT = 512;
constexpr int SIG_TILE = SIG_NT * 16;
constexpr int SIG_PPT = 16;
constexpr int POS_PAD_WORDS = 64;
constexpr int SORT_CAP = 4096;
constexpr int MAX_FINE_BITS = 15;

constexpr int REC_BIN_BITS = 22;
constexpr int REC_FINE_SHIFT = 26;
constexpr uint32_t REC_BIN_MASK = (1u << REC_BIN_BITS) - 1u;

struct Bucket {
    uint64_t begin;
    uint32_t n;
    uint32_t lbin;
    uint32_t c0, c1;
};

constexpr int STAGE_MAXP = 5;
static_assert(STAGE_MAXP >= 4 && STAGE_MAXP <= 8, "staged pieces per job");
constexpr int STAGE_MAXP128 = 4;
template <int KW>
constexpr int stage_npc() { return KW == 2 ? STAGE_MAXP128 : STAGE_MAXP; }
struct BucketSrc {
    const uint64_t *keys;
    int F;
    int np = 0;
    const uint64_t *pk[STAGE_MAXP] = {};
    const uint64_t *pcb[STAGE_MAXP] = {};
    const struct PieceStarts *starts = nullptr;
};
struct PieceStarts {
    uint64_t s[STAGE_MAXP];
    uint32_t pre[STAGE_MAXP];
};
hipError_t launch_bucket_finish(const BucketSrc &src, struct Bucket *buckets, uint64_t nb, uint32_t nlbins,
                                uint64_t total_keys, PieceStarts *out, hipStream_t s);

struct Chunk {
    uint64_t rec_begin, rec_end;
    uint32_t lbin, pad;
};

struct ScanWorkspace {
    void *ptr = nullptr;
    size_t bytes = 0;
};

hipError_t scan_excl_sum_u64(const uint64_t *in, uint64_t *out, uint64_t n, uint64_t *total, ScanWorkspace &ws,
                             hipStream_t s);
hipError_t scan_excl_sum_u32_to_u64(const uint32_t *in, uint64_t *out, uint64_t n, uint64_t *total,
                                    ScanWorkspace &ws, hipStream_t s);
hipError_t scan_excl_max_i64(const int64_t *in, int64_t *out, uint64_t n, ScanWorkspace &ws, hipStream_t s);

hipError_t launch_fasta_parse(bool scan, const uint8_t *fa, uint64_t n, uint64_t *st_line, uint64_t *st_pos,
                              uint32_t *codes, uint32_t *valid, uint64_t *npos_dev, hipStream_t s);
hipError_t launch_superkmers(int W, const uint32_t *codes, const uint32_t *valid, uint64_t npos_bound,
                             const uint64_t *npos_dev, int k, int m, FastMod fm, uint64_t *records, uint64_t rec_cap,
                             uint64_t *status, uint64_t *tile_kmers, unsigned long long *counters, hipStream_t s);
hipError_t launch_fill_u64(uint64_t *p, uint64_t n, uint64_t v, hipStream_t s);
hipError_t launch_bin_signatures(const uint32_t *codes, const uint32_t *valid, uint64_t npos_bound,
                                 const uint64_t *npos_dev, int k, int m, unsigned long long *counts, hipStream_t s);
hipError_t launch_sig_compact(const unsigned long long *counts, uint64_t n, uint64_t *pairs, unsigned long long *nout,
                              hipStream_t s);

bool map_fused_supported(int k, int m, uint32_t nbins);
uint64_t fm_tile_bytes(int nth);
uint64_t fm_span_bytes(int nth);
uint32_t map_fused_tcap();
hipError_t map_fused_cycles(unsigned long long *out16, bool reset);
// ... 39 lines not shown
                            uint32_t *H, uint32_t *K, hipStream_t s);
hipError_t launch_part_segsum(const uint32_t *H, const uint32_t *K, uint32_t nparts, uint32_t nwg, uint64_t *T,
                              uint64_t *KT, hipStream_t s);
hipError_t launch_part_segfill(const uint32_t *H, const uint64_t *Ts, uint32_t nparts, uint32_t nwg, uint64_t *Hs,
                               hipStream_t s);
hipError_t launch_part_totals(const uint64_t *Hs, const uint64_t *Ks, uint32_t nparts, uint32_t nwg,
                              uint64_t *part_rec, uint64_t *part_kmer, uint64_t *part_off, hipStream_t s);
hipError_t launch_part_scatter(const RecSrc &src, int mode, uint32_t G, const uint32_t *table, uint32_t nparts,
                               const uint64_t *Hs, uint64_t *out, hipStream_t s);
hipError_t launch_part_hist_global(const RecSrc &src, int mode, uint32_t G, const uint32_t *table, uint32_t nparts,
                                   uint64_t *part_rec, uint64_t *part_kmer, hipStream_t s);
hipError_t launch_part_scatter_global(const RecSrc &src, int mode, uint32_t G, const uint32_t *table,
                                      uint32_t nparts, const uint64_t *part_off, uint64_t *part_cursor,
                                      uint64_t *out, hipStream_t s);

hipError_t launch_expand_hist(int W, const uint64_t *rec, const Chunk *chunks, uint32_t nchunks, int k, int F,
                              uint32_t *hist, hipStream_t s);
hipError_t launch_cell_prefix(const uint32_t *bin_chunk_begin, uint32_t nlbins, int F, uint32_t *hist,
                              uint64_t *cell_total, hipStream_t s);
hipError_t launch_expand_scatter(int W, const uint64_t *rec, const Chunk *chunks, uint32_t nchunks, int k, int F,
                                 const uint32_t *hist, const uint64_t *cell_base, uint64_t *keys, hipStream_t s);
hipError_t launch_bucket_flags(const uint64_t *cell_base, const uint64_t *cell_total, uint32_t nlbins, int F,
                               uint32_t small_cap, uint32_t group, uint32_t *flags, hipStream_t s);
hipError_t launch_bucket_write(const uint64_t *cell_base, const uint32_t *flags, const uint64_t *flag_scan,
                               uint32_t nlbins, int F, uint64_t nbuckets, uint64_t total_keys, Bucket *buckets,
                               hipStream_t s);
hipError_t launch_bucket_count64(const BucketSrc &src, const Bucket *buckets, uint64_t nbuckets, int k,
                                 uint64_t *out_keys, uint32_t *out_counts, uint64_t *bucket_unique,
                                 unsigned long long *oversize, uint32_t small_limit, int dbg_phase,
                                 const uint32_t *list, hipStream_t s, uint32_t skip_le = 0);
hipError_t launch_bucket_count64_big(const BucketSrc &src, const Bucket *buckets, uint64_t nlist, int k,
                                     uint64_t *out_keys, uint32_t *out_counts, uint64_t *bucket_unique,
                                     unsigned long long *oversize, const uint32_t *list, hipStream_t s);
constexpr uint32_t WAVE_BUCKET_CAP = 512;
constexpr uint32_t WAVE_SLOTS = 640;
constexpr uint32_t WAVE_MID_CAP = 1024;
constexpr uint32_t WAVE_MID_SLOTS = 1280;
constexpr uint32_t WAVE128_BUCKET_CAP = 256;
hipError_t launch_bucket_count128_wave(const BucketSrc &src, const Bucket *buckets, uint64_t nbuckets, int k,
                                       uint64_t *out_keys, uint32_t *out_counts, uint64_t *bucket_unique,
                                       hipStream_t s, bool ordered = true);
hipError_t launch_expand_two_level(int KW, const uint64_t *rec, const Chunk *chunks, uint32_t nchunks,
                                   uint32_t nlbins, int k, int F, int F2, const uint32_t *sc_pre,
                                   const uint64_t *cell_base, uint64_t *mid, uint64_t *keys, hipStream_t s,
                                   int l1_threads = 0, uint64_t nkeys = 0);
hipError_t launch_expand_hist_pieces(int KW, const uint64_t *rec, const Chunk *chunks, const uint4 *pieces,
                                     const uint32_t *first_piece, uint32_t npieces, int k, int F, int F2,
                                     uint64_t *cell_total, uint32_t *hist_sc, uint32_t *piece_tot, hipStream_t s);
hipError_t launch_expand_hist_bin(int KW, const uint64_t *rec, const Chunk *chunks, const uint32_t *bin_chunk_begin,
                                  uint32_t nlbins, int k, int F, int F2, uint64_t *cell_total, uint32_t *hist_sc,
                                  hipStream_t s);
hipError_t launch_bucket_flags_greedy(const uint64_t *cell_total, uint32_t nlbins, int F, uint32_t cap,
                                      int period_bits, uint32_t *flags, hipStream_t s);
hipError_t launch_bucket_tiers(const Bucket *buckets, uint64_t nb, uint32_t wave_cap, uint32_t block_cap,
                               uint64_t *bucket_unique, uint32_t *lists, unsigned int *counts,
                               unsigned long long *listed_keys, hipStream_t s);
hipError_t launch_bucket_count64_wave(const BucketSrc &src, const Bucket *buckets, uint64_t nbuckets, int k,
                                      uint64_t *out_keys, uint32_t *out_counts, uint64_t *bucket_unique,
                                      const uint32_t *list, hipStream_t s, bool ordered = true);
hipError_t launch_bucket_count64_parts(const BucketSrc &src, const Bucket *buckets, const uint32_t *list,
                                       uint64_t nlist, int k, uint64_t *out_keys, uint32_t *out_counts,
                                       uint64_t *bucket_unique, uint32_t *fb, unsigned int *fb_count, hipStream_t s,
                                       bool ordered);
hipError_t launch_bucket_count64_mid512(const BucketSrc &src, const Bucket *buckets, const uint32_t *list,
                                        uint64_t nlist, int k, uint64_t *out_keys, uint32_t *out_counts,
                                        uint64_t *bucket_unique, uint32_t *fb, unsigned int *fb_count, hipStream_t s,
                                        bool ordered);
hipError_t launch_bucket_count64_wave_mid(const BucketSrc &src, const Bucket *buckets, const uint32_t *list,
                                          uint64_t nlist, int k, uint64_t *out_keys, uint32_t *out_counts,
                                          uint64_t *bucket_unique, hipStream_t s, bool ordered = true);
struct SubBucket {
    uint64_t src;
    uint64_t lo;
    uint32_t n, span;
};
struct SplitParent {
    uint32_t first, nsub;
};
hipError_t launch_listed_sizes(const Bucket *buckets, const uint32_t *list0, uint32_t n0, const uint32_t *list1,
                               uint32_t n1, uint64_t *sizes, hipStream_t s,
                               bool slots = false);
hipError_t launch_bucket_split64(const BucketSrc &src, const Bucket *buckets, const uint32_t *list0, uint32_t n0,
                                 const uint32_t *list1, uint32_t n1, const uint64_t *sbase, uint64_t *skeys,
                                 SubBucket *subs, SplitParent *parents, unsigned int *counts, uint32_t *fb0,
                                 uint32_t *fb1, uint32_t block_cap, int k, int F, hipStream_t s, bool retry = false);
hipError_t launch_sub_count64_seq(const Bucket *buckets, const uint32_t *list, uint32_t nl, const SplitParent *parents,
                                  const SubBucket *subs, const uint64_t *skeys, uint64_t *out_keys,
                                  uint32_t *out_counts, uint64_t *bucket_unique, hipStream_t s, bool ordered);
struct SubBucket128 {
    uint64_t src;
    uint64_t lo_hi, lo_lo;
    uint32_t n, span;
};
hipError_t launch_bucket_split128(const BucketSrc &src, const Bucket *buckets, const uint32_t *list, uint32_t nl,
                                  const uint64_t *sbase, uint64_t *skeys, SubBucket128 *subs, SplitParent *parents,
                                  unsigned int *counts, uint32_t *fb0, uint32_t *fb1, uint32_t block_cap, int k, int F,
                                  hipStream_t s, bool retry = false);
hipError_t launch_sub_count128_seq(const Bucket *buckets, const uint32_t *list, uint32_t nl, const SplitParent *parents,
                                   const SubBucket128 *subs, const uint64_t *skeys, uint64_t *out_keys,
                                   uint32_t *out_counts, uint64_t *bucket_unique, hipStream_t s, bool ordered);
hipError_t launch_add_u64(uint64_t *dst, const uint64_t *src, uint64_t n, bool copy, hipStream_t s);
hipError_t launch_bucket_sort(int KW, const BucketSrc &src, const Bucket *buckets, uint64_t nbuckets, int k,
                              uint64_t *out_keys, uint32_t *out_counts, uint64_t *bucket_unique,
                              unsigned long long *oversize, uint32_t small_limit, const uint32_t *list, hipStream_t s,
                              uint32_t skip_le = 0);
constexpr uint32_t WAVE128_MID_CAP = 512;
hipError_t launch_bucket_count128_wave_mid(const BucketSrc &src, const Bucket *buckets, const uint32_t *list,
                                           uint64_t nlist, int k, uint64_t *out_keys, uint32_t *out_counts,
                                           uint64_t *bucket_unique, hipStream_t s, bool ordered = true);
hipError_t launch_bucket_sort_large(int KW, const BucketSrc &src, const Bucket *buckets, uint64_t nbuckets, int k,
                                    uint64_t *scratch, uint64_t *out_keys, uint32_t *out_counts,
                                    uint64_t *bucket_unique, const uint32_t *list, hipStream_t s,
                                    unsigned long long *scratch_cursor = nullptr);
hipError_t launch_bucket_compact(int KW, const uint64_t *out_keys, const uint32_t *out_counts,
                                 const Bucket *buckets, uint64_t nbuckets, const uint64_t *dense_off,
                                 uint64_t *dense_keys, uint32_t *dense_counts, hipStream_t s);
hipError_t launch_bin_offsets(const uint64_t *flag_scan, const uint64_t *dense_off, uint32_t nlbins, int F,
                              uint64_t nbuckets, uint64_t *bin_off, hipStream_t s);

struct QueryTables {
    const uint64_t *flag_scan;
// ... 61 lines not shown
```

fastkmer_amd/csrc/fk_kernels.hip:

```cpp
#include <hip/hip_runtime.h>
#include <stdint.h>

#include <algorithm>
#include <limits>
#include <type_traits>

#include "fk_internal.h"

namespace fk {

constexpr int NT = 256;


template <int CTRL, int ROWM>
__device__ __forceinline__ uint32_t dpp32(uint32_t old, uint32_t v) {
    return (uint32_t)__builtin_amdgcn_update_dpp((int)old, (int)v, CTRL, ROWM, 0xf, false);
}
template <int CTRL, int ROWM, typename T>
__device__ __forceinline__ T dpp_move(T ident, T v) {
    static_assert(sizeof(T) == 4 || sizeof(T) == 8, "32- or 64-bit scan values");
    if constexpr (sizeof(T) == 4) {
        return __builtin_bit_cast(T, dpp32<CTRL, ROWM>(__builtin_bit_cast(uint32_t, ident), __builtin_bit_cast(uint32_t, v)));
    } else {
        const uint64_t i = __builtin_bit_cast(uint64_t, ident), x = __builtin_bit_cast(uint64_t, v);
// ... 245 lines not shown
    if (e == hipSuccess) ws.bytes = need;
    return e;
}

hipError_t scan_excl_sum_u64(const uint64_t *in, uint64_t *out, uint64_t n, uint64_t *total, ScanWorkspace &ws,
                             hipStream_t s) {
    hipError_t e = ensure_ws(ws, scan_ws_need(n, 8));
    if (e != hipSuccess) return e;
    return scan_impl<uint64_t, uint64_t, OpSum, false>(in, out, n, (uint64_t)0, total, (char *)ws.ptr, ws.bytes, s);
}

hipError_t scan_excl_sum_u32_to_u64(const uint32_t *in, uint64_t *out, uint64_t n, uint64_t *total,
                                    ScanWorkspace &ws, hipStream_t s) {
    hipError_t e = ensure_ws(ws, scan_ws_need(n, 8));
    if (e != hipSuccess) return e;
    return scan_impl<uint32_t, uint64_t, OpSum, false>(in, out, n, (uint64_t)0, total, (char *)ws.ptr, ws.bytes, s);
}

hipError_t scan_excl_max_i64(const int64_t *in, int64_t *out, uint64_t n, ScanWorkspace &ws, hipStream_t s) {
    hipError_t e = ensure_ws(ws, scan_ws_need(n, 8));
    if (e != hipSuccess) return e;
    return scan_impl<int64_t, int64_t, OpMax, true>(in, out, n, (int64_t)-1, (int64_t *)nullptr, (char *)ws.ptr,
                                                    ws.bytes, s);
}

#include "fk_parse.inc"
#include "fk_fastq.inc"
#include "fk_signature.inc"
#include "fk_map_fused.inc"
#include "fk_records.inc"
#include "fk_partition.inc"
#include "fk_radix_rank.inc"
#include "fk_count_sorted.inc"
#include "fk_expand2.inc"
#include "fk_sort_radix.inc"
#include "fk_compact.inc"
#include "fk_synth.inc"
#include "fk_format.inc"
#include "fk_bin_signatures.inc"
#include "fk_query.inc"
#include "fk_spectrum.inc"
#include "fk_compare.inc"
#include "fk_reads.inc"

__global__ void __launch_bounds__(64) k_hold_stream(const uint32_t *flag, uint64_t max_ticks) {
    if (threadIdx.x != 0) return;
    const uint64_t t0 = wall_clock64();
    while (__hip_atomic_load(flag, __ATOMIC_ACQUIRE, __HIP_MEMORY_SCOPE_SYSTEM) == 0u) {
        if (wall_clock64() - t0 > max_ticks) break;
        __builtin_amdgcn_s_sleep(127);
    }
}

hipError_t launch_hold_stream(const uint32_t *flag, uint64_t max_ticks, hipStream_t s) {
    hipLaunchKernelGGL(k_hold_stream, dim3(1), dim3(64), 0, s, flag, max_ticks);
    return hipGetLastError();
}
}
```

fastkmer_amd/csrc/fk_radix_rank.inc:

```

template <int KW>
__device__ __forceinline__ uint32_t digit_of(uint64_t key, int sh) { return (uint32_t)(key >> sh) & 15u; }
template <int KW>
__device__ __forceinline__ uint32_t digit_of(u128 key, int sh) { return (uint32_t)(key >> sh) & 15u; }

template <typename K, int IPT>
__device__ __forceinline__ void tile_rank(const K (&key)[IPT], int n_valid_here, int sh, uint32_t *s_cnt,
                                          uint32_t *s_tmp, uint32_t (&pos)[IPT], uint32_t (&dig)[IPT],
                                          uint32_t *digit_total ) {
    uint64_t lo = 0, hi = 0;
#pragma unroll
    for (int it = 0; it < IPT; ++it) {
        const uint32_t d = (uint32_t)(key[it] >> sh) & 15u;
        dig[it] = d;
        if (it < n_valid_here) {
            const int f = 8 * (d & 7);
            const uint64_t word = (d < 8) ? lo : hi;
            pos[it] = (uint32_t)(word >> f) & 0xffu;
            if (d < 8)
                lo += 1ull << f;
            else
                hi += 1ull << f;
        }
    }
#pragma unroll
    for (int d = 0; d < 16; ++d) {
        const uint64_t word = d < 8 ? lo : hi;
        s_cnt[d * NT + threadIdx.x] = (uint32_t)(word >> (8 * (d & 7))) & 0xffu;
    }
    __syncthreads();
    uint32_t v[16];
    uint32_t sum = 0;
#pragma unroll
    for (int j = 0; j < 16; ++j) {
        v[j] = s_cnt[threadIdx.x * 16 + j];
        sum += v[j];
    }
    uint32_t tot;
    uint32_t run = block_excl_sum<uint32_t>(sum, s_tmp, &tot);
#pragma unroll
    for (int j = 0; j < 16; ++j) {
        s_cnt[threadIdx.x * 16 + j] = run;
        run += v[j];
    }
    __syncthreads();
    if (digit_total && threadIdx.x < 16) {
// ... 10 lines not shown
```

fastkmer_amd/csrc/fk_sort_radix.inc:

```

template <int KW>
__global__ __launch_bounds__(NT) void k_bucket_sort(BucketSrc src, const Bucket *__restrict__ buckets, int k,
                                                    uint64_t *__restrict__ out_keys,
                                                    uint32_t *__restrict__ out_counts, uint64_t *bucket_unique,
                                                    unsigned long long *oversize, uint32_t small_limit,
                                                    const uint32_t *__restrict__ list, uint32_t skip_le) {
    typedef typename KeyOf<KW>::T K;
    constexpr int CAP = SORT_CAP / KW;
    constexpr int IPT = CAP / NT;
    __shared__ K s_keys[CAP];
    __shared__ uint32_t s_cnt[16 * NT + 1];
    __shared__ uint32_t s_tmp[NT / 64];
    __shared__ K s_red[2][NT / 64];

    const uint32_t qi = list ? list[blockIdx.x] : blockIdx.x;
    const Bucket b = buckets[qi];
    const int n = (int)b.n;
    if (skip_le && b.n <= skip_le) return;
    if (b.n > (uint32_t)CAP || b.n > small_limit) {
        if (threadIdx.x == 0) {
            bucket_unique[qi] = REDO;
            atomicAdd(oversize, 1ull);
        }
        return;
// ... 18 lines not shown
#pragma unroll
    for (int it = 0; it < IPT; ++it) {
        if (it < nv) {
            key[it] = s_keys[my0 + it];
            kor |= key[it];
            kand &= key[it];
        } else {
            key[it] = ~(K)0;
        }
    }
    {
        const int lane = threadIdx.x & 63, wid = threadIdx.x >> 6;
#pragma unroll
        for (int d = 32; d > 0; d >>= 1) {
            if constexpr (KW == 1) {
                kor |= __shfl_xor(kor, d, 64);
                kand &= __shfl_xor(kand, d, 64);
            } else {
                const uint64_t a = (uint64_t)kor, bb = (uint64_t)(kor >> 64);
                const uint64_t c = (uint64_t)kand, e = (uint64_t)(kand >> 64);
                kor |= ((u128)__shfl_xor(bb, d, 64) << 64) | __shfl_xor(a, d, 64);
                kand &= ((u128)__shfl_xor(e, d, 64) << 64) | __shfl_xor(c, d, 64);
            }
        }
        if (lane == 0) {
            s_red[0][wid] = kor;
            s_red[1][wid] = kand;
        }
        __syncthreads();
        kor = s_red[0][0] | s_red[0][1] | s_red[0][2] | s_red[0][3];
        kand = s_red[1][0] & s_red[1][1] & s_red[1][2] & s_red[1][3];
        __syncthreads();
    }
    const K diff = kor ^ kand;
    int lo_bit = 0, hi_bit = -1;
    if (diff != 0) {
        if constexpr (KW == 1) {
            lo_bit = __builtin_ctzll(diff);
            hi_bit = 63 - __builtin_clzll(diff);
        } else {
            const uint64_t dl = (uint64_t)diff, dh = (uint64_t)(diff >> 64);
            lo_bit = dl ? __builtin_ctzll(dl) : 64 + __builtin_ctzll(dh);
            hi_bit = dh ? 127 - __builtin_clzll(dh) : 63 - __builtin_clzll(dl);
        }
    }
    for (int sh = lo_bit & ~3; sh <= hi_bit; sh += 4) {
        uint32_t pos[IPT], dig[IPT];
        tile_rank<K, IPT>(key, nv, sh, s_cnt, s_tmp, pos, dig, nullptr);
#pragma unroll
        for (int it = 0; it < IPT; ++it)
            if (it < nv) s_keys[pos[it]] = key[it];
        __syncthreads();
#pragma unroll
        for (int it = 0; it < IPT; ++it) key[it] = (it < nv) ? s_keys[my0 + it] : ~(K)0;
        __syncthreads();
    }
    if (hi_bit < 0) {
        if (threadIdx.x == 0) {
            store_key(out_keys, b.begin, key[0]);
            out_counts[b.begin] = (uint32_t)n;
            bucket_unique[qi] = 1;
        }
        return;
    }
#pragma unroll
    for (int it = 0; it < IPT; ++it) s_keys[my0 + it] = key[it];
    __syncthreads();
    uint32_t heads = 0;
#pragma unroll
    for (int it = 0; it < IPT; ++it) {
        const int i = my0 + it;
        if (i < n && (i == 0 || s_keys[i - 1] != key[it])) heads |= 1u << it;
    }
    uint32_t nu;
    uint32_t u = block_excl_sum<uint32_t>((uint32_t)__popc(heads), s_tmp, &nu);
#pragma unroll
    for (int it = 0; it < IPT; ++it)
        if ((heads >> it) & 1u) s_cnt[u++] = (uint32_t)(my0 + it);
    if (threadIdx.x == 0) s_cnt[nu] = (uint32_t)n;
    __syncthreads();
    for (uint32_t q = threadIdx.x; q < nu; q += NT) {
        const uint32_t hp = s_cnt[q];
        store_key(out_keys, b.begin + q, s_keys[hp]);
        out_counts[b.begin + q] = s_cnt[q + 1] - hp;
    }
    if (threadIdx.x == 0) bucket_unique[qi] = nu;
}

hipError_t launch_bucket_sort(int KW, const BucketSrc &src, const Bucket *buckets, uint64_t nbuckets, int k,
                              uint64_t *out_keys, uint32_t *out_counts, uint64_t *bucket_unique,
                              unsigned long long *oversize, uint32_t small_limit, const uint32_t *list, hipStream_t s,
                              uint32_t skip_le) {
    if (!nbuckets) return hipSuccess;
    if (KW == 1)
        k_bucket_sort<1><<<(unsigned)nbuckets, NT, 0, s>>>(src, buckets, k, out_keys, out_counts, bucket_unique,
                                                             oversize, small_limit, list, skip_le);
    else
        k_bucket_sort<2><<<(unsigned)nbuckets, NT, 0, s>>>(src, buckets, k, out_keys, out_counts, bucket_unique,
                                                             oversize, small_limit, list, skip_le);
    return hipGetLastError();
}


template <int KW>
__global__ __launch_bounds__(NT) void k_bucket_sort_large(BucketSrc src, const Bucket *buckets, int k,
                                                          uint64_t *scratch, uint64_t *out_keys,
                                                          uint32_t *out_counts, uint64_t *bucket_unique,
                                                          const uint32_t *__restrict__ list,
                                                          unsigned long long *scratch_cursor) {
    typedef typename KeyOf<KW>::T K;
    constexpr int IPT = (SORT_CAP / KW) / NT;
    constexpr int TILE = NT * IPT;
    __shared__ uint32_t s_cnt[16 * NT + 1];
    __shared__ uint32_t s_tmp[NT / 64];
    __shared__ uint32_t s_dtot[16];
    __shared__ uint64_t s_dbase[16];
    __shared__ uint64_t s_hist[16];
    __shared__ K s_red[2][NT / 64];
    __shared__ K s_carry;
    __shared__ uint64_t s_state[2];
    __shared__ uint64_t s_soff;

    const uint32_t qi = list ? list[blockIdx.x] : blockIdx.x;
    const Bucket b = buckets[qi];
    if (bucket_unique[qi] != REDO) return;
    const uint64_t n = b.n;
    if (threadIdx.x == 0) s_soff = scratch_cursor ? atomicAdd(scratch_cursor, (unsigned long long)n) : b.begin;
    __syncthreads();
    const uint64_t soff = s_soff;
    {
        const BucketView bv = bucket_view<KW>(src, b);
        for (uint64_t li = threadIdx.x; li < n; li += NT) {
            K x;
            load_key(bucket_key_ptr<KW>(bv, (uint32_t)li), 0, x);
            store_key(scratch, soff + li, x);
        }
    }
    __syncthreads();
    uint64_t *bufA = scratch, *bufB = out_keys;
    uint64_t offA = soff, offB = b.begin;
    K kor = 0, kand = ~(K)0;
    for (uint64_t i = threadIdx.x; i < n; i += NT) {
        K x;
        load_key(bufA, offA + i, x);
        kor |= x;
        kand &= x;
    }
    {
        const int lane = threadIdx.x & 63, wid = threadIdx.x >> 6;
        for (int d = 32; d > 0; d >>= 1) {
            if constexpr (KW == 1) {
                kor |= __shfl_xor(kor, d, 64);
                kand &= __shfl_xor(kand, d, 64);
            } else {
                const uint64_t a = (uint64_t)kor, bb = (uint64_t)(kor >> 64);
                const uint64_t c = (uint64_t)kand, e = (uint64_t)(kand >> 64);
                kor |= ((u128)__shfl_xor(bb, d, 64) << 64) | __shfl_xor(a, d, 64);
                kand &= ((u128)__shfl_xor(e, d, 64) << 64) | __shfl_xor(c, d, 64);
            }
        }
        if (lane == 0) {
            s_red[0][wid] = kor;
            s_red[1][wid] = kand;
        }
        __syncthreads();
        kor = s_red[0][0] | s_red[0][1] | s_red[0][2] | s_red[0][3];
        kand = s_red[1][0] & s_red[1][1] & s_red[1][2] & s_red[1][3];
        __syncthreads();
    }
    const K diff = kor ^ kand;
    int lo_bit = 0, hi_bit = -1;
    if (diff != 0) {
        if constexpr (KW == 1) {
            lo_bit = __builtin_ctzll(diff);
            hi_bit = 63 - __builtin_clzll(diff);
        } else {
            const uint64_t dl = (uint64_t)diff, dh = (uint64_t)(diff >> 64);
            lo_bit = dl ? __builtin_ctzll(dl) : 64 + __builtin_ctzll(dh);
            hi_bit = dh ? 127 - __builtin_clzll(dh) : 63 - __builtin_clzll(dl);
        }
    }
    for (int sh = lo_bit & ~3; sh <= hi_bit; sh += 4) {
        if (threadIdx.x < 16) s_hist[threadIdx.x] = 0;
        __syncthreads();
        for (uint64_t i = threadIdx.x; i < n; i += NT) {
            K x;
            load_key(bufA, offA + i, x);
            atomicAdd((unsigned long long *)&s_hist[(uint32_t)(x >> sh) & 15u], 1ull);
        }
        __syncthreads();
        if (threadIdx.x == 0) {
            uint64_t acc = 0;
            for (int d = 0; d < 16; ++d) {
                s_dbase[d] = acc;
                acc += s_hist[d];
            }
        }
        __syncthreads();
        for (uint64_t t0 = 0; t0 < n; t0 += TILE) {
            K key[IPT];
            const uint64_t my0 = t0 + (uint64_t)threadIdx.x * IPT;
            const int nv = (int)max((int64_t)0, min((int64_t)IPT, (int64_t)n - (int64_t)my0));
#pragma unroll
            for (int it = 0; it < IPT; ++it) {
                if (it < nv)
                    load_key(bufA, offA + my0 + it, key[it]);
                else
                    key[it] = ~(K)0;
            }
            uint32_t pos[IPT], dig[IPT];
            tile_rank<K, IPT>(key, nv, sh, s_cnt, s_tmp, pos, dig, s_dtot);
#pragma unroll
            for (int it = 0; it < IPT; ++it) {
                if (it < nv) {
                    const uint32_t d = dig[it];
                    const uint64_t dst = s_dbase[d] + (pos[it] - s_cnt[d * NT]);
                    store_key(bufB, offB + dst, key[it]);
                }
            }
            __syncthreads();
            if (threadIdx.x < 16) s_dbase[threadIdx.x] += s_dtot[threadIdx.x];
            __syncthreads();
        }
        uint64_t *t = bufA;
        bufA = bufB;
        bufB = t;
        const uint64_t to = offA;
        offA = offB;
        offB = to;
        __syncthreads();
    }
    if (threadIdx.x == 0) {
        s_state[0] = 0;
        s_state[1] = ~0ull;
    }
    __syncthreads();
    for (uint64_t t0 = 0; t0 < n; t0 += TILE) {
        const uint64_t tlen = min((uint64_t)TILE, n - t0);
        K key[IPT];
        const uint64_t my0 = t0 + (uint64_t)threadIdx.x * IPT;
        const int nv = (int)max((int64_t)0, min((int64_t)IPT, (int64_t)n - (int64_t)my0));
#pragma unroll
        for (int it = 0; it < IPT; ++it) {
            if (it < nv)
                load_key(bufA, offA + my0 + it, key[it]);
            else
                key[it] = ~(K)0;
        }
        K pk;
        if (threadIdx.x == 0)
            pk = s_carry;
        else if (nv > 0)
            load_key(bufA, offA + my0 - 1, pk);
        else
            pk = ~(K)0;
        uint32_t heads = 0;
#pragma unroll
        for (int it = 0; it < IPT; ++it) {
            if (it < nv && ((my0 + it) == 0 || key[it] != pk)) heads |= 1u << it;
            pk = key[it];
        }
        __syncthreads();
#pragma unroll
        for (int it = 0; it < IPT; ++it)
            if ((uint64_t)it + my0 == t0 + tlen - 1) s_carry = key[it];
        uint32_t nh;
        uint32_t u = block_excl_sum<uint32_t>((uint32_t)__popc(heads), s_tmp, &nh);
        const uint64_t ubase = s_state[0];
        const uint64_t open_head = s_state[1];
        const uint32_t u0 = u;
#pragma unroll
        for (int it = 0; it < IPT; ++it)
            if ((heads >> it) & 1u) s_cnt[u++] = (uint32_t)(threadIdx.x * IPT + it);
        if (threadIdx.x == 0) s_cnt[nh] = (uint32_t)tlen;
        __syncthreads();
        if (nh > 0 && threadIdx.x == 0 && open_head != ~0ull)
            out_counts[b.begin + ubase - 1] = (uint32_t)(t0 + s_cnt[0] - open_head);
        u = u0;
#pragma unroll
        for (int it = 0; it < IPT; ++it) {
            if ((heads >> it) & 1u) {
                store_key(out_keys, b.begin + ubase + u, key[it]);
                if (u + 1 < nh) out_counts[b.begin + ubase + u] = s_cnt[u + 1] - s_cnt[u];
                ++u;
            }
        }
        __syncthreads();
        if (threadIdx.x == 0 && nh > 0) {
            s_state[0] = ubase + nh;
            s_state[1] = t0 + s_cnt[nh - 1];
        }
        __syncthreads();
    }
    if (threadIdx.x == 0) {
        const uint64_t ub = s_state[0];
        if (ub > 0) out_counts[b.begin + ub - 1] = (uint32_t)(n - s_state[1]);
        bucket_unique[qi] = ub;
    }
}

hipError_t launch_bucket_sort_large(int KW, const BucketSrc &src, const Bucket *buckets, uint64_t nbuckets, int k,
                                    uint64_t *scratch, uint64_t *out_keys, uint32_t *out_counts,
                                    uint64_t *bucket_unique, const uint32_t *list, hipStream_t s,
                                    unsigned long long *scratch_cursor) {
    if (!nbuckets) return hipSuccess;
    if (KW == 1)
        k_bucket_sort_large<1><<<(unsigned)nbuckets, NT, 0, s>>>(src, buckets, k, scratch, out_keys, out_counts,
                                                                   bucket_unique, list, scratch_cursor);
    else
        k_bucket_sort_large<2><<<(unsigned)nbuckets, NT, 0, s>>>(src, buckets, k, scratch, out_keys, out_counts,
                                                                   bucket_unique, list, scratch_cursor);
    return hipGetLastError();
}
```

include/fastkmer.h:

```cpp
#ifndef FASTKMER_H
#define FASTKMER_H

#include <stddef.h>
#include <stdint.h>

#ifdef __cplusplus
extern "C" {
#endif

#define FK_ABI_VERSION 3

#define FK_OK 0
#define FK_E_INVALID (-1)
#define FK_E_STATE (-2)
#define FK_E_DEVICE (-3)
#define FK_E_NOMEM (-4)
#define FK_E_IO (-5)
#define FK_E_RANGE (-6)
#define FK_E_COMM (-7)

typedef struct fk_config {
    int32_t k;
    int32_t m;
    int32_t x;
// ... 131 lines not shown
                        uint32_t other_min, uint32_t other_max, uint64_t *kept_per_bin);
int fk_get_bin_joined(fk_ctx *ctx, fk_ctx *other, int32_t bin, uint32_t min_count, uint32_t max_count,
                      uint32_t other_min, uint32_t other_max, uint64_t *keys, uint32_t *counts,
                      uint32_t *other_counts, size_t cap, size_t *n);

#define FK_READ_TILE 4096
typedef struct fk_read_stat {
    uint32_t windows;
    uint32_t hits;
    uint32_t min;
    uint32_t median;
    uint32_t max;
    uint32_t reserved;
    uint64_t sum;
} fk_read_stat;
int fk_reads_csr(const uint8_t *text, size_t n, int32_t format, int32_t min_quality, int32_t quality_offset,
                 uint8_t *bases, size_t cap_bases, uint64_t *offsets, size_t cap_reads,
                 size_t *n_reads, size_t *n_bases);
int fk_read_counts_device(fk_ctx *ctx, const void *d_bases, const void *d_offsets, size_t n_reads,
                          void *d_counts, void *d_valid);
int fk_read_counts(fk_ctx *ctx, const uint8_t *bases, const uint64_t *offsets, size_t n_reads,
                   uint32_t *counts, uint8_t *valid);
int fk_read_stats_of_counts_device(fk_ctx *ctx, const void *d_counts, const void *d_valid, const void *d_offsets,
                                   size_t n_reads, uint32_t min_count, uint32_t max_count, void *d_stats);
int fk_read_stats_device(fk_ctx *ctx, const void *d_bases, const void *d_offsets, size_t n_reads,
                         uint32_t min_count, uint32_t max_count, void *d_scratch, size_t scratch_bytes, void *d_stats);
int fk_read_stats(fk_ctx *ctx, const uint8_t *bases, const uint64_t *offsets, size_t n_reads,
                  uint32_t min_count, uint32_t max_count, fk_read_stat *stats);
size_t fk_read_stats_scratch_bytes(size_t n_bases);

int fk_debug_wave_count(int32_t device, int32_t k, int32_t F, uint32_t c0, uint32_t c1, int32_t slots,
                        const uint64_t *keys, uint32_t n, uint64_t *out_keys, uint32_t *out_counts,
                        uint32_t *n_out);

int fk_debug_comm_hold(fk_ctx *ctx, int32_t max_seconds);
int fk_debug_comm_release(fk_ctx *ctx);
int fk_debug_comm_held(fk_ctx *ctx);

int fk_debug_fingerprint_bits(int32_t device, int32_t bits);

int fk_debug_map_cycles(uint64_t *out16, int32_t reset);

int fk_debug_fastq_ms(fk_ctx *ctx, double *ms, uint64_t *launches);

uint64_t fk_signature_slots(const fk_ctx *ctx);
int fk_signature_counts(fk_ctx *ctx, void *d_counts, uint64_t n_counts);
int fk_write_bin_signatures(fk_ctx *ctx, const void *d_counts, uint64_t n_counts, const char *out_dir);
int fk_find_bin_signatures(fk_ctx *ctx, const char *out_dir);

#ifdef __cplusplus
}
#endif
#endif
```

Measured before the change: 40.46 billion bases/s.

## Fold staged k-mer pieces into weighted keys before final bucket counting

Adds an optional fold pass that collapses duplicate k-mers within each staged piece. The multiplicity is packed into the spare high bits above the 2k-bit key, and a compaction pass shrinks the piece. In mode 1 a sampling kernel estimates the duplicate ratio on the first piece and enables folding only when enough entries would collapse. The bucket count, sort and sub-count kernels are taught to mask the key and sum the packed weights. The aim is to cut the entries that later sort and count stages must process, at the cost of an extra host sync for sampling, extra scan and compact kernels, and masking work in hot kernels even when folding is off.

```diff
diff --git a/fastkmer_amd/__init__.py b/fastkmer_amd/__init__.py
--- a/fastkmer_amd/__init__.py
+++ b/fastkmer_amd/__init__.py
@@ -177,6 +177,9 @@
         "fk_debug_fingerprint_bits": (ctypes.c_int, [I32, I32]),
         "fk_debug_wave_count": (ctypes.c_int, [I32, I32, I32, ctypes.c_uint32, ctypes.c_uint32, I32, P,
                                                ctypes.c_uint32, P, P, P]),
+        "fk_debug_wave_count_w": (ctypes.c_int, [I32, I32, I32, ctypes.c_uint32, ctypes.c_uint32, I32, P,
+                                                 ctypes.c_uint32, P, P, P]),
+        "fk_debug_fold_stats": (ctypes.c_int, [P, P]),
     }
     for name, (res, args) in sig.items():
         fn = getattr(L, name)
@@ -748,16 +751,23 @@
         _check(lib().fk_get_stats(self._h, ctypes.byref(st)))
         return {n: getattr(st, n) for n, _ in fk_stats._fields_}
 
-
-def debug_wave_count(keys: np.ndarray, k: int, F: int, c0: int, c1: int, slots: int, device: int = 0):
+    def fold_stats(self) -> dict:
+        out = (ctypes.c_uint64 * 4)()
+        _check(lib().fk_debug_fold_stats(self._h, out))
+        return {"pieces_folded": int(out[0]), "entries_in": int(out[1]), "entries_out": int(out[2]),
+                "sample_ratio": int(out[3]) / 1e6 if out[3] else None}
+
+
+def debug_wave_count(keys: np.ndarray, k: int, F: int, c0: int, c1: int, slots: int, device: int = 0,
+                     weighted: bool = False):
     kw = 1 if k <= 32 else 2
     keys = np.ascontiguousarray(keys, dtype=np.uint64).reshape(-1, kw)
     n = len(keys)
     ok = np.zeros(n * kw, dtype=np.uint64)
     oc = np.zeros(n, dtype=np.uint32)
     nout = ctypes.c_uint32(0)
-    _check(lib().fk_debug_wave_count(device, k, F, c0, c1, slots, keys.ctypes.data, n, ok.ctypes.data,
-                                     oc.ctypes.data, ctypes.byref(nout)))
+    fn = lib().fk_debug_wave_count_w if weighted else lib().fk_debug_wave_count
+    _check(fn(device, k, F, c0, c1, slots, keys.ctypes.data, n, ok.ctypes.data, oc.ctypes.data, ctypes.byref(nout)))
     u = nout.value
     return (ok[:u] if kw == 1 else ok[:2 * u].reshape(-1, 2)), oc[:u]
 
diff --git a/fastkmer_amd/csrc/fk_api.cpp b/fastkmer_amd/csrc/fk_api.cpp
--- a/fastkmer_amd/csrc/fk_api.cpp
+++ b/fastkmer_amd/csrc/fk_api.cpp
@@ -254,6 +254,9 @@
     if (const char *v = env("FASTKMER_DEBUG_MID_PARTS")) c->mid_parts = atoi(v);
     if (const char *v = env("FASTKMER_DEBUG_SPLIT_RETRY")) c->split_retry = v[0] == '1';
     if (const char *v = env("FASTKMER_DEBUG_SPECTRUM_WIDE")) c->spectrum_wide = v[0] == '1';
+    if (const char *v = env("FASTKMER_FOLD")) c->fold_mode = std::clamp(atoi(v), 0, 2);
+    if (const char *v = env("FASTKMER_DEBUG_FOLD_WMAX"))
+        c->fold_wmax = (uint32_t)std::clamp(atoi(v), 1, (int)WKEY_WMAX);
     if (const char *v = env("FASTKMER_X2_L1")) c->x2_l1 = atoi(v);
     if (const char *v = env("FASTKMER_FUSED")) c->fused = atoi(v);
 #ifdef FK_PROBES
@@ -360,6 +363,7 @@
     c->pin_up.release();
     c->pin_down.release();
     c->pin_tier.release();
+    c->fold_pin.release();
     c->file_pin[0].release();
     c->file_pin[1].release();
     if (c->tier_ev) (void)hipEventDestroy(c->tier_ev);
@@ -391,6 +395,7 @@
         if (ev) (void)hipEventDestroy(ev);
     for (int p = 0; p < STAGE_MAXP; ++p) release(c->st_keys[p]), release(c->st_cb[p]);
     release(c->st_total);
+    release(c->fold_cnt), release(c->fold_cb), release(c->fold_io);
     release(c->piece_starts);
     if (c->seg_ev) (void)hipEventDestroy(c->seg_ev);
     for (auto &ev : c->h2d_ev)
@@ -1479,7 +1484,7 @@
 static hipError_t launch_sub_count_seq(const BucketCount &t, const uint32_t *l1, uint32_t nl, const SubBucket *subs,
                                        hipStream_t s) {
     return launch_sub_count64_seq(t.buckets(), l1, nl, t.c->sp_par.as<SplitParent>(), subs, t.c->sp_keys.as<uint64_t>(),
-                                  t.out_keys(), t.out_counts(), t.unique(), s, t.ordered);
+                                  t.k, t.src.weighted, t.out_keys(), t.out_counts(), t.unique(), s, t.ordered);
 }
 static hipError_t launch_sub_count_seq(const BucketCount &t, const uint32_t *l1, uint32_t nl, const SubBucket128 *subs,
                                        hipStream_t s) {
@@ -1529,7 +1534,7 @@
     BucketSrc &src = t.src;
     src.F = F;
     if (src.np > 0) FK_TRY(ensure(*B.piece_starts, nbuckets * sizeof(PieceStarts)));
-    HIP_TRY(launch_bucket_finish(src, B.buckets->as<Bucket>(), nbuckets, c->nlb, total_kmers,
+    HIP_TRY(launch_bucket_finish(src, B.buckets->as<Bucket>(), nbuckets, c->nlb, cell_base + ncell_all,
                                  src.np > 0 ? B.piece_starts->as<PieceStarts>() : nullptr, cs));
     if (src.np > 0) src.starts = B.piece_starts->as<PieceStarts>();
     HIP_TRY(hipMemsetAsync(c->misc.p, 0, 64, cs));
@@ -2026,6 +2031,10 @@
     c->pieces_void = false;
     c->tiles_counted = 0;
     c->segs_counted = 0;
+    c->fold_decided = c->fold_on = false;
+    c->fold_sample_ppm = 0;
+    c->fold_in = 0;
+    c->fold_pieces.clear();
 }
 
 static uint32_t stage_maxp(const fk_ctx *c) { return c->KW == 2 ? (uint32_t)STAGE_MAXP128 : (uint32_t)STAGE_MAXP; }
@@ -2094,6 +2103,7 @@
                               c->cell_base.as<uint64_t>() + ncell_all, *on.ws, cs));
     BucketSrc src{nullptr, pl.F};
     src.np = (int)c->st_np;
+    src.weighted = !c->fold_pieces.empty();
     for (uint32_t p = 0; p < c->st_np; ++p) {
         src.pk[p] = c->st_keys[p].as<uint64_t>();
         src.pcb[p] = c->st_cb[p].as<uint64_t>();
@@ -2125,6 +2135,71 @@
         return tiles * tile >= end && (tiles - c->tiles_counted) * tile >= MIN_PIECE / 2;
     }
     return c->st_np < 3 && (tiles - c->tiles_counted) * tile >= c->piece_bytes;
+}
+
+static bool fold_eligible(const fk_ctx *c) {
+    return c->fold_mode != 0 && c->KW == 1 && 2 * c->cfg.k <= WKEY_MAX_BITS && staged_eligible(c);
+}
+
+constexpr uint32_t FOLD_SAMPLE_STRIDE = 61;
+constexpr uint64_t FOLD_SAMPLE_MAX = 4096;
+constexpr uint64_t FOLD_MAX_PPM = 600000;
+static int fold_decide(fk_ctx *c, StreamWs on, uint32_t p) {
+    c->fold_decided = true;
+    c->fold_on = c->fold_mode == 2;
+    if (c->fold_mode != 1) return FK_OK;
+    const SortedPlan &pl = c->st_plan;
+    FK_TRY(ensure(c->fold_io, 16));
+    const uint64_t nsc = (uint64_t)c->nlb << pl.F1;
+    const uint32_t stride = (uint32_t)std::max<uint64_t>(FOLD_SAMPLE_STRIDE, (nsc / FOLD_SAMPLE_MAX) | 1ull);
+    HIP_TRY(hipMemsetAsync(c->fold_io.p, 0, 16, on.s));
+    HIP_TRY(launch_fold_sample(c->st_keys[p].as<uint64_t>(), c->st_cb[p].as<uint64_t>(), c->nlb, c->cfg.k, pl.F, pl.F2,
+                               c->fold_wmax, stride, c->fold_io.as<unsigned long long>(), on.s));
+    uint64_t io[2] = {0, 0};
+    HIP_TRY(hipMemcpyAsync(io, c->fold_io.p, 16, hipMemcpyDeviceToHost, on.s));
+    HIP_TRY(hipStreamSynchronize(on.s));
+    c->fold_sample_ppm = io[0] ? io[1] * 1000000ull / io[0] : 1000000ull;
+    c->fold_on = io[0] && c->fold_sample_ppm <= FOLD_MAX_PPM;
+    htrace("staged: fold sampled");
+    return FK_OK;
+}
+
+static void fold_report(fk_ctx *c, bool counted) {
+    uint64_t out = 0;
+    for (uint32_t p : c->fold_pieces) out += c->fold_pin.as<uint64_t>()[p];
+    c->fold_last[0] = counted ? c->fold_pieces.size() : 0;
+    c->fold_last[1] = counted ? c->fold_in : 0;
+    c->fold_last[2] = counted ? out : 0;
+    c->fold_last[3] = c->fold_sample_ppm;
+}
+
+static bool fold_piece_due(const fk_ctx *c) {
+    if (c->fold_mode == 2) return true;
+    if (c->job_bytes && !c->piece_bytes_set) return c->st_cut == 1;
+    return true;
+}
+
+static int fold_piece(fk_ctx *c, StreamWs on, uint32_t p, uint64_t pk) {
+    if (pk == 0 || pk >= (1ull << 32)) return FK_OK;
+    const SortedPlan &pl = c->st_plan;
+    const uint64_t ncell_all = (uint64_t)c->nlb << pl.F;
+    FK_TRY(ensure(c->fold_cnt, ncell_all * 4));
+    FK_TRY(ensure(c->fold_cb, (ncell_all + 1) * 8));
+    HIP_TRY(launch_fold_sc(c->st_keys[p].as<uint64_t>(), c->st_cb[p].as<uint64_t>(), c->nlb, c->cfg.k, pl.F, pl.F2,
+                           c->fold_wmax, c->mid.as<uint64_t>(), c->fold_cnt.as<uint32_t>(), on.s));
+    HIP_TRY(scan_excl_sum_u32_to_u64(c->fold_cnt.as<uint32_t>(), c->fold_cb.as<uint64_t>(), ncell_all,
+                                     c->fold_cb.as<uint64_t>() + ncell_all, *on.ws, on.s));
+    HIP_TRY(launch_fold_compact(c->mid.as<uint64_t>(), c->st_cb[p].as<uint64_t>(), c->fold_cb.as<uint64_t>(),
+                                c->fold_cnt.as<uint32_t>(), c->nlb, pl.F, pl.F2, c->st_keys[p].as<uint64_t>(),
+                                c->st_total.as<uint64_t>(), on.s));
+    if (c->fold_pin.ensure(8 * STAGE_MAXP)) return set_err(FK_E_NOMEM, "hipHostMalloc failed");
+    HIP_TRY(hipMemcpyAsync(c->fold_pin.as<uint64_t>() + p, c->fold_cb.as<uint64_t>() + ncell_all, 8,
+                           hipMemcpyDeviceToHost, on.s));
+    std::swap(c->st_cb[p], c->fold_cb);
+    c->fold_in += pk;
+    c->fold_pieces.push_back(p);
+    htrace("staged: piece folded");
+    return FK_OK;
 }
 
 static int local_maybe_piece(fk_ctx *c, uint64_t tiles, hipEvent_t mapped) {
@@ -2143,8 +2218,14 @@
     const RecSrc src = fused_src(c, t0, nt, nt * map_fused_tcap());
     c->tiles_counted = tiles;
     c->st_cut += 1;
+    const uint32_t p = c->st_np;
+    const uint64_t k0 = c->st_kmers;
     FK_TRY(staged_expand(c, on, nullptr, src,
                          c->job_bytes ? (double)(nt * fm_tile_bytes(FUSED_NT)) / (double)c->job_bytes : 0.0));
+    if (c->st_np > p && fold_eligible(c)) {
+        if (!c->fold_decided) FK_TRY(fold_decide(c, on, p));
+        if (c->fold_on && fold_piece_due(c)) FK_TRY(fold_piece(c, on, p, c->st_kmers - k0));
+    }
     HIP_TRY(hipEventRecord(c->xstage_ev, s));
     return FK_OK;
 }
@@ -2507,9 +2588,11 @@
         if (rc == FK_OK) rc = staged_count(c, cut);
         if (cut) (void)hipStreamSynchronize(cut);
         FK_TRY(rc);
+        fold_report(c, true);
         pieces_reset(c);
         return FK_OK;
     }
+    fold_report(c, false);
     pieces_reset(c);
     return reduce_src(c, map_src(c));
 }
@@ -2736,9 +2819,9 @@
     return FK_OK;
 }
 
-FK_EXPORT int fk_debug_wave_count(int32_t device, int32_t k, int32_t F, uint32_t c0, uint32_t c1, int32_t slots,
-                                  const uint64_t *keys, uint32_t n, uint64_t *out_keys, uint32_t *out_counts,
-                                  uint32_t *n_out) {
+static int debug_wave_count(int32_t device, int32_t k, int32_t F, uint32_t c0, uint32_t c1, int32_t slots,
+                            const uint64_t *keys, uint32_t n, uint64_t *out_keys, uint32_t *out_counts,
+                            uint32_t *n_out, bool weighted) {
     if (!keys || !out_keys || !out_counts || !n_out || k < 1 || k > 63 || F < 1 || F > MAX_FINE_BITS || c1 <= c0 ||
         c1 > (1u << F))
         return set_err(FK_E_INVALID, "bad argument");
@@ -2749,7 +2832,10 @@
         return set_err(FK_E_INVALID, "slots: %u (k <= 32) or 384 (k > 32)", WAVE_SLOTS);
     const int sh = 2 * k - F;
     for (uint32_t i = 0; i < n; ++i) {
-        const uint64_t hi = KW == 1 ? 0 : keys[2 * i], lo = KW == 1 ? keys[i] : keys[2 * i + 1];
+        const uint64_t hi = KW == 1 ? 0 : keys[2 * i];
+        uint64_t lo = KW == 1 ? keys[i] : keys[2 * i + 1];
+        if (weighted && KW == 1 && 2 * k <= WKEY_MAX_BITS && (lo >> (2 * k)) <= WKEY_WMAX - 1)
+            lo &= (1ull << (2 * k)) - 1ull;
         const uint64_t cell = sh >= 64 ? (hi >> (sh - 64)) : (sh == 0 ? lo : ((hi << (64 - sh)) | (lo >> sh)));
         if ((KW == 1 && k < 32 && (lo >> (2 * k)) != 0) || cell < c0 || cell >= c1)
             return set_err(FK_E_RANGE, "key %u lies outside cells [%u, %u)", i, c0, c1);
@@ -2762,11 +2848,13 @@
     FK_TRY(ensure(du, 16));
     FK_TRY(ensure(db, sizeof(Bucket)));
     const Bucket b{0, n, 0, c0, c1};
+    BucketSrc wsrc{dk.as<uint64_t>(), F};
+    wsrc.weighted = weighted;
     int rc = FK_OK;
     hipError_t e = hipMemcpy(dk.p, keys, (uint64_t)n * 8 * KW, hipMemcpyHostToDevice);
     if (e == hipSuccess) e = hipMemcpy(db.p, &b, sizeof(Bucket), hipMemcpyHostToDevice);
     if (e == hipSuccess)
-        e = KW == 1 ? launch_bucket_count64_wave(BucketSrc{dk.as<uint64_t>(), F}, db.as<Bucket>(), 1, k, dok.as<uint64_t>(),
+        e = KW == 1 ? launch_bucket_count64_wave(wsrc, db.as<Bucket>(), 1, k, dok.as<uint64_t>(),
                                                  doc.as<uint32_t>(), du.as<uint64_t>(), nullptr, nullptr)
                     : launch_bucket_count128_wave(BucketSrc{dk.as<uint64_t>(), F}, db.as<Bucket>(), 1, k, dok.as<uint64_t>(),
                                                   doc.as<uint32_t>(), du.as<uint64_t>(), nullptr);
@@ -2778,6 +2866,24 @@
     else if (U > n) rc = set_err(FK_E_INVALID, "bucket reported %llu distinct keys of %u", (unsigned long long)U, n);
     *n_out = (uint32_t)U;
     return rc;
+}
+
+FK_EXPORT int fk_debug_wave_count(int32_t device, int32_t k, int32_t F, uint32_t c0, uint32_t c1, int32_t slots,
+                                  const uint64_t *keys, uint32_t n, uint64_t *out_keys, uint32_t *out_counts,
+                                  uint32_t *n_out) {
+    return debug_wave_count(device, k, F, c0, c1, slots, keys, n, out_keys, out_counts, n_out, false);
+}
+
+FK_EXPORT int fk_debug_wave_count_w(int32_t device, int32_t k, int32_t F, uint32_t c0, uint32_t c1, int32_t slots,
+                                    const uint64_t *keys, uint32_t n, uint64_t *out_keys, uint32_t *out_counts,
+                                    uint32_t *n_out) {
+    return debug_wave_count(device, k, F, c0, c1, slots, keys, n, out_keys, out_counts, n_out, true);
+}
+
+FK_EXPORT int fk_debug_fold_stats(const fk_ctx *c, uint64_t out[4]) {
+    if (!c || !out) return set_err(FK_E_INVALID, "null argument");
+    std::copy(c->fold_last, c->fold_last + 4, out);
+    return FK_OK;
 }
 
 FK_EXPORT int fk_debug_map_cycles(uint64_t *out16, int32_t reset) {
diff --git a/fastkmer_amd/csrc/fk_count_sorted.inc b/fastkmer_amd/csrc/fk_count_sorted.inc
--- a/fastkmer_amd/csrc/fk_count_sorted.inc
+++ b/fastkmer_amd/csrc/fk_count_sorted.inc
@@ -416,13 +416,13 @@
 
 template <bool PIECES>
 __global__ __launch_bounds__(NT) void k_bucket_finish(BucketSrc src, Bucket *__restrict__ buckets, uint64_t nb,
-                                                      uint32_t nlbins, uint64_t total_keys,
+                                                      uint32_t nlbins, const uint64_t *__restrict__ total_keys,
                                                       PieceStarts *__restrict__ out) {
     const uint64_t i = (uint64_t)blockIdx.x * NT + threadIdx.x;
     const bool mine = i < nb;
     const uint32_t ncell = 1u << src.F;
     Bucket b{};
-    uint64_t e_beg = total_keys, g1 = (uint64_t)nlbins << src.F;
+    uint64_t e_beg = *total_keys, g1 = (uint64_t)nlbins << src.F;
     if (mine) {
         b = buckets[i];
         if (i + 1 < nb) {
@@ -457,7 +457,7 @@
 }
 
 hipError_t launch_bucket_finish(const BucketSrc &src, Bucket *buckets, uint64_t nb, uint32_t nlbins,
-                                uint64_t total_keys, PieceStarts *out, hipStream_t s) {
+                                const uint64_t *total_keys, PieceStarts *out, hipStream_t s) {
     if (!nb) return hipSuccess;
     const unsigned grid = (unsigned)((nb + NT - 1) / NT);
     if (src.np > 0)
@@ -519,6 +519,20 @@
 constexpr uint64_t REDO = ~0ull;
 constexpr uint64_t EMPTY_KEY = ~0ull;
 constexpr uint32_t BLOCK_SPLIT_GROUP = 64;
+
+struct WKeySpec {
+    uint64_t kmask;
+    int wsh;
+};
+__device__ __host__ inline WKeySpec wkey_spec(int k, bool weighted = true) {
+    return weighted && 2 * k <= WKEY_MAX_BITS ? WKeySpec{(1ull << (2 * k)) - 1ull, 2 * k} : WKeySpec{~0ull, 0};
+}
+__device__ __forceinline__ uint64_t wkey_split(uint64_t x, const WKeySpec &ws, uint32_t &w) {
+    w = 1u;
+    if (ws.wsh == 0) return x;
+    w += (uint32_t)(x >> ws.wsh);
+    return x & ws.kmask;
+}
 
 __device__ __forceinline__ uint32_t hslot(uint64_t key) {
     return (uint32_t)((key * 0x9e3779b97f4a7c15ull) >> 52) & (HSLOTS - 1);
@@ -548,8 +562,9 @@
     __shared__ unsigned long long s_spl[NT];
     const uint32_t qi = list ? list[blockIdx.x] : blockIdx.x;
     const Bucket b = buckets[qi];
-    if (b.n <= skip_le) return;
+    if (skip_le && b.n <= skip_le) return;
     const BucketView bv = bucket_view(src, b);
+    const WKeySpec ws = wkey_spec(k, src.weighted);
     if (!STREAM && (b.n > HC || b.n > small_limit)) {
         if (threadIdx.x == 0) {
             bucket_unique[qi] = REDO;
@@ -592,8 +607,9 @@
         }
 #pragma unroll
         for (int q = 0; q < GB; ++q) {
-            const uint64_t key = kk[q];
-            if (key == EMPTY_KEY) continue;
+            if (kk[q] == EMPTY_KEY) continue;
+            uint32_t wt;
+            const uint64_t key = wkey_split(kk[q], ws, wt);
             uint32_t s = POW2 ? (uint32_t)((key * 0x9e3779b97f4a7c15ull) >> (64 - HBITS))
                               : (uint32_t)((((key * 0x9e3779b97f4a7c15ull) >> 32) * HS) >> 32);
             for (;;) {
@@ -601,10 +617,10 @@
                 if (cur == EMPTY_KEY) cur = atomicCAS(&s_k[s], EMPTY_KEY, (unsigned long long)key);
                 if (cur == EMPTY_KEY || cur == key) {
                     const uint32_t old =
-                        atomicAdd(reinterpret_cast<uint32_t *>(&s_c[s & ~1u]), 1u << (16 * (s & 1u)));
+                        atomicAdd(reinterpret_cast<uint32_t *>(&s_c[s & ~1u]), wt << (16 * (s & 1u)));
                     if constexpr (STREAM) {
                         if (cur == EMPTY_KEY) atomicAdd(&s_nu, 1u);
-                        if (((old >> (16 * (s & 1u))) & 0xffffu) == 0xffffu) s_ovf = 1u;
+                        if (((old >> (16 * (s & 1u))) & 0xffffu) + wt > 0xffffu) s_ovf = 1u;
                     }
                     break;
                 }
@@ -1023,11 +1039,11 @@
 #endif
 }
 
-template <uint32_t CAP, uint32_t SL, bool ORD = true, int WKPT = WaveCfg<CAP>::KPT, int NROW = WKPT>
+template <uint32_t CAP, uint32_t SL, bool ORD = true, int WKPT = WaveCfg<CAP>::KPT, int NROW = WKPT, bool WT = true>
 __device__ __forceinline__ uint32_t wave_count_keys(WaveLds<CAP, SL> &w, uint64_t begin, uint32_t n, uint64_t lo,
                                                 int span_bits, uint64_t q, const uint64_t (&kk)[NROW],
-                                                uint64_t *__restrict__ out_keys, uint32_t *__restrict__ out_counts,
-                                                uint64_t *__restrict__ uniq) {
+                                                const WKeySpec ws, uint64_t *__restrict__ out_keys,
+                                                uint32_t *__restrict__ out_counts, uint64_t *__restrict__ uniq) {
     const int lane = threadIdx.x & 63;
     unsigned long long *s_k = w.k;
     uint16_t *s_c = w.c;
@@ -1050,15 +1066,18 @@
     static_assert(NROW == WKPT || (NROW > WKPT && SL - CAP >= 64), "a row's new keys fit above CAP");
     uint32_t sl[NROW];
 #pragma unroll
-    for (int j = 0; j < NROW; ++j) sl[j] = wslot<SL>(kk[j]);
+    for (int j = 0; j < NROW; ++j) sl[j] = wslot<SL>(WT ? kk[j] & ws.kmask : kk[j]);
     uint32_t U = 0;
 #pragma unroll
     for (int j = 0; j < NROW; ++j) {
         bool over = false;
         if constexpr (NROW > WKPT) over = U > CAP;
-        const uint64_t key = over ? EMPTY_KEY : kk[j];
+        const uint64_t x = over ? EMPTY_KEY : kk[j];
         bool fresh = false;
-        if (key != EMPTY_KEY) {
+        if (x != EMPTY_KEY) {
+            uint32_t wt = 1u;
+            uint64_t key = x;
+            if constexpr (WT) key = wkey_split(x, ws, wt);
             uint32_t s = sl[j];
             for (;;) {
                 const unsigned long long prev = atomicCAS(&s_k[s], EMPTY_KEY, (unsigned long long)key);
@@ -1066,7 +1085,7 @@
                 if (fresh || prev == key) break;
                 s = s + 1 == SL ? 0u : s + 1;
             }
-            atomicAdd(reinterpret_cast<uint32_t *>(&s_c[s & ~1u]), 1u << (16 * (s & 1u)));
+            atomicAdd(reinterpret_cast<uint32_t *>(&s_c[s & ~1u]), wt << (16 * (s & 1u)));
             sl[j] = s;
         }
         const uint64_t m = __ballot(fresh);
@@ -1126,18 +1145,18 @@
     return U;
 }
 
-template <uint32_t CAP, uint32_t SL, bool ORD = true, int WKPT = WaveCfg<CAP>::KPT>
+template <uint32_t CAP, uint32_t SL, bool ORD = true, bool WT = true, int WKPT = WaveCfg<CAP>::KPT>
 __device__ __forceinline__ void wave_count_bucket(WaveLds<CAP, SL> &w, const Bucket &b, uint64_t q,
-                                                  const uint64_t (&kk)[WKPT], int k, int F,
+                                                  const uint64_t (&kk)[WKPT], int k, int F, const WKeySpec ws,
                                                   uint64_t *__restrict__ out_keys, uint32_t *__restrict__ out_counts,
                                                   uint64_t *__restrict__ bucket_unique) {
     const int sh = 2 * k - F;
     const int span_bits = b.n ? (32 - __builtin_clz(b.c1 - b.c0)) + sh : 0;
-    wave_count_keys<CAP, SL, ORD, WKPT>(w, b.begin, b.n, (uint64_t)b.c0 << sh, span_bits, q, kk, out_keys,
-                                        out_counts, bucket_unique);
-}
-
-template <int BPW, uint32_t CAP, uint32_t SL, bool MS = false, bool ORD = true>
+    wave_count_keys<CAP, SL, ORD, WKPT, WKPT, WT>(w, b.begin, b.n, (uint64_t)b.c0 << sh, span_bits, q, kk, ws,
+                                        out_keys, out_counts, bucket_unique);
+}
+
+template <int BPW, uint32_t CAP, uint32_t SL, bool MS = false, bool ORD = true, bool WT = true>
 __global__ __launch_bounds__(64) void k_bucket_count64_wave(BucketSrc src,
                                                             const Bucket *__restrict__ buckets, uint64_t nbuckets,
                                                             int k, uint64_t *__restrict__ out_keys,
@@ -1179,7 +1198,8 @@
 #pragma unroll
     for (int t = 0; t < BPW; ++t)
         if (mine[t])
-            wave_count_bucket<CAP, SL, ORD>(w, b[t], qq[t], kk[t], k, src.F, out_keys, out_counts, bucket_unique);
+            wave_count_bucket<CAP, SL, ORD, WT>(w, b[t], qq[t], kk[t], k, src.F, wkey_spec(k, src.weighted), out_keys,
+                                            out_counts, bucket_unique);
 }
 
 constexpr int FLAGS_NT = 256;
@@ -1282,10 +1302,16 @@
                                       const uint32_t *list, hipStream_t s, bool ordered) {
     if (!nbuckets) return hipSuccess;
     const unsigned grid = (unsigned)((nbuckets + 1) / 2);
-#define FK_W64(MS_, ORD_)                                                                                  \
-    k_bucket_count64_wave<2, WAVE_BUCKET_CAP, WAVE_SLOTS, MS_, ORD_><<<grid, 64, 0, s>>>(src, buckets, nbuckets, k, \
-                                                                                 out_keys, out_counts,     \
-                                                                                 bucket_unique, list)
+#define FK_W64T(MS_, ORD_, WT_)                                                                                 \
+    k_bucket_count64_wave<2, WAVE_BUCKET_CAP, WAVE_SLOTS, MS_, ORD_, WT_><<<grid, 64, 0, s>>>(                 \
+        src, buckets, nbuckets, k, out_keys, out_counts, bucket_unique, list)
+#define FK_W64(MS_, ORD_)                    \
+    do {                                     \
+        if (src.weighted)                    \
+            FK_W64T(MS_, ORD_, true);        \
+        else                                 \
+            FK_W64T(MS_, ORD_, false);       \
+    } while (0)
     if (src.np > 0 && ordered)
         FK_W64(true, true);
     else if (src.np > 0)
@@ -1295,6 +1321,7 @@
     else
         FK_W64(false, false);
 #undef FK_W64
+#undef FK_W64T
     return hipGetLastError();
 }
 
@@ -1343,7 +1370,8 @@
         const uint64_t *pa = row_key_ptr(v, rb, (int)(row0 >> 6), i);
         return ldg_nt<uint64_t>(i < n ? pa : klast);
     };
-    unsigned long long x = *bucket_key_ptr(v, (uint32_t)(((uint64_t)lane * n) >> 6));
+    const WKeySpec ws = wkey_spec(k, src.weighted);
+    unsigned long long x = *bucket_key_ptr(v, (uint32_t)(((uint64_t)lane * n) >> 6)) & ws.kmask;
 #pragma unroll
     for (uint32_t kk = 2; kk <= 64; kk <<= 1) {
 #pragma unroll
@@ -1366,7 +1394,7 @@
 #pragma unroll
     for (int r = 0; r < R; ++r) {
         const uint32_t i = r * 64 + lane;
-        const unsigned long long key = kr[r];
+        const unsigned long long key = kr[r] & ws.kmask;
         const uint32_t g = range_of(key);
         c0 += (i < n && g == 0) ? 1u : 0u;
         c1 += (i < n && g == 1) ? 1u : 0u;
@@ -1388,7 +1416,7 @@
         for (int r = 0; r < R; ++r) {
             const uint32_t i = r * 64 + lane;
             const unsigned long long key = kr[r];
-            const bool mine = i < n && range_of(key) == g;
+            const bool mine = i < n && range_of(key & ws.kmask) == g;
             const uint64_t m = __ballot(mine);
             if (mine)
                 w.k[at + __builtin_amdgcn_mbcnt_hi((uint32_t)(m >> 32), __builtin_amdgcn_mbcnt_lo((uint32_t)m, 0u))] = key;
@@ -1405,7 +1433,7 @@
         const uint64_t lo = g == 0 ? klo : (g == 1 ? sp0 : sp1) + 1ull;
         const uint64_t hi = g + 1 == P ? khi : (g == 0 ? sp0 : sp1);
         const int span = hi > lo ? 64 - __builtin_clzll(hi - lo) : 0;
-        pre += wave_count_keys<CAP, SL, ORD>(w, b.begin + pre, ng, lo, span, 0, kk, out_keys, out_counts, nullptr);
+        pre += wave_count_keys<CAP, SL, ORD>(w, b.begin + pre, ng, lo, span, 0, kk, ws, out_keys, out_counts, nullptr);
     }
     if (lane == 0) bucket_unique[q] = pre;
 }
@@ -1450,7 +1478,8 @@
     const int sh = 2 * k - src.F;
     const int span_bits = (32 - __builtin_clz(b.c1 - b.c0)) + sh;
     const uint32_t U = wave_count_keys<CAP, SL, ORD, WKPT, R>(w, b.begin, b.n, (uint64_t)b.c0 << sh, span_bits, q, kk,
-                                                              out_keys, out_counts, bucket_unique);
+                                                              wkey_spec(k, src.weighted), out_keys, out_counts,
+                                                              bucket_unique);
     if (U == ~0u && (threadIdx.x & 63) == 0) fb[atomicAdd(fb_count, 1u)] = q;
 }
 
@@ -1513,7 +1542,7 @@
                                                        uint64_t *__restrict__ skeys, SubBucket *__restrict__ subs,
                                                        SplitParent *__restrict__ parents, unsigned int *counts,
                                                        uint32_t *__restrict__ fb0, uint32_t *__restrict__ fb1,
-                                                       uint32_t block_cap, int sh, int retry) {
+                                                       uint32_t block_cap, int sh, int retry, uint64_t kmask) {
     __shared__ uint64_t s_smp[WSPL_SMAX];
     __shared__ uint32_t s_cnt[WSPL_MAXS];
     const uint32_t lane = threadIdx.x;
@@ -1558,7 +1587,7 @@
         while (S < ns * SPL_OVER && S < WSPL_SMAX) S <<= 1;
         const uint64_t soff = att ? (uint64_t)b.n / (2 * S) : 0;
         for (uint32_t j = lane; j < S; j += 64)
-            s_smp[j] = *bucket_key_ptr(v, (uint32_t)(((uint64_t)j * b.n) / S + soff));
+            s_smp[j] = *bucket_key_ptr(v, (uint32_t)(((uint64_t)j * b.n) / S + soff)) & kmask;
         for (uint32_t t = lane; t < WSPL_MAXS; t += 64) s_cnt[t] = 0;
         wave_lds_sync();
         for (uint32_t kk = 2; kk <= S; kk <<= 1) {
@@ -1592,7 +1621,7 @@
 #pragma unroll
             for (int r = 0; r < WSPL_KB; ++r)
                 if (j0 + r * 64 + lane < b.n) {
-                    const uint32_t sub = sub_of(x[r]);
+                    const uint32_t sub = sub_of(x[r] & kmask);
                     const uint32_t at = atomicAdd(&s_cnt[sub], 1u);
                     if (att == 0 && at < SPL_SLOT) skeys[sb + (uint64_t)sub * SPL_SLOT + at] = x[r];
                 }
@@ -1654,7 +1683,7 @@
         for (int r = 0; r < WSPL_KB; ++r) x[r] = key_at(j0 + r * 64, j0 + r * 64 + lane);
 #pragma unroll
         for (int r = 0; r < WSPL_KB; ++r)
-            if (j0 + r * 64 + lane < b.n) skeys[sb + atomicAdd(&s_cnt[sub_of(x[r])], 1u)] = x[r];
+            if (j0 + r * 64 + lane < b.n) skeys[sb + atomicAdd(&s_cnt[sub_of(x[r] & kmask)], 1u)] = x[r];
     }
 }
 
@@ -1664,7 +1693,7 @@
                                  uint32_t *fb1, uint32_t block_cap, int k, int F, hipStream_t s, bool retry) {
     if (!(n0 + n1)) return hipSuccess;
     k_bucket_split64<<<n0 + n1, 64, 0, s>>>(src, buckets, list0, n0, list1, sbase, skeys, subs, parents, counts, fb0,
-                                            fb1, block_cap, 2 * k - F, retry ? 1 : 0);
+                                            fb1, block_cap, 2 * k - F, retry ? 1 : 0, wkey_spec(k, src.weighted).kmask);
     return hipGetLastError();
 }
 
@@ -1673,7 +1702,7 @@
                                                         const uint32_t *__restrict__ list,
                                                         const SplitParent *__restrict__ parents,
                                                         const SubBucket *__restrict__ subs,
-                                                        const uint64_t *__restrict__ skeys,
+                                                        const uint64_t *__restrict__ skeys, const WKeySpec ws,
                                                         uint64_t *__restrict__ out_keys,
                                                         uint32_t *__restrict__ out_counts,
                                                         uint64_t *__restrict__ bucket_unique) {
@@ -1702,8 +1731,8 @@
         const bool more = j + 1 < P.nsub;
         d1 = subs[P.first + (more ? j + 1 : j)];
         load(d1, kb);
-        pre += wave_count_keys<CAP, SL, ORD>(w, begin + pre, d0.n, d0.lo, (int)d0.span, 0, ka, out_keys, out_counts,
-                                             nullptr);
+        pre += wave_count_keys<CAP, SL, ORD>(w, begin + pre, d0.n, d0.lo, (int)d0.span, 0, ka, ws, out_keys,
+                                             out_counts, nullptr);
         if (!more) break;
         d0 = d1;
 #pragma unroll
@@ -1713,14 +1742,16 @@
 }
 
 hipError_t launch_sub_count64_seq(const Bucket *buckets, const uint32_t *list, uint32_t nl, const SplitParent *parents,
-                                  const SubBucket *subs, const uint64_t *skeys, uint64_t *out_keys,
-                                  uint32_t *out_counts, uint64_t *bucket_unique, hipStream_t s, bool ordered) {
+                                  const SubBucket *subs, const uint64_t *skeys, int k, bool weighted,
+                                  uint64_t *out_keys, uint32_t *out_counts, uint64_t *bucket_unique, hipStream_t s,
+                                  bool ordered) {
     if (!nl) return hipSuccess;
+    const WKeySpec ws = wkey_spec(k, weighted);
     if (ordered)
-        k_sub_count64_seq<true><<<nl, 64, 0, s>>>(buckets, list, parents, subs, skeys, out_keys, out_counts,
+        k_sub_count64_seq<true><<<nl, 64, 0, s>>>(buckets, list, parents, subs, skeys, ws, out_keys, out_counts,
                                                   bucket_unique);
     else
-        k_sub_count64_seq<false><<<nl, 64, 0, s>>>(buckets, list, parents, subs, skeys, out_keys, out_counts,
+        k_sub_count64_seq<false><<<nl, 64, 0, s>>>(buckets, list, parents, subs, skeys, ws, out_keys, out_counts,
                                                    bucket_unique);
     return hipGetLastError();
 }
diff --git a/fastkmer_amd/csrc/fk_ctx.h b/fastkmer_amd/csrc/fk_ctx.h
--- a/fastkmer_amd/csrc/fk_ctx.h
+++ b/fastkmer_amd/csrc/fk_ctx.h
@@ -279,6 +279,15 @@
     uint64_t st_kmers = 0;
     DevBuf st_keys[STAGE_MAXP], st_cb[STAGE_MAXP], st_total, piece_starts;
     hipEvent_t st_ev[4 * STAGE_MAXP] = {};
+    int fold_mode = 1;
+    uint32_t fold_wmax = WKEY_WMAX;
+    bool fold_decided = false, fold_on = false;
+    uint64_t fold_sample_ppm = 0;
+    uint64_t fold_in = 0;
+    std::vector<uint32_t> fold_pieces;
+    DevBuf fold_cnt, fold_cb, fold_io;
+    PinBuf fold_pin;
+    uint64_t fold_last[4] = {0, 0, 0, 0};
 
     fk::Comm *comm = nullptr;
     hipStream_t comm_stream = nullptr;
diff --git a/fastkmer_amd/csrc/fk_fold.inc b/fastkmer_amd/csrc/fk_fold.inc
--- /dev/null
+++ b/fastkmer_amd/csrc/fk_fold.inc
@@ -0,0 +1,158 @@
+
+constexpr uint32_t FOLD_HS = 2 * FOLD_HC;
+constexpr int FOLD_KPT = FOLD_HC / NT;
+constexpr int FOLD_SPT = FOLD_HS / NT;
+constexpr uint32_t FOLD_MAXC = 64;
+static_assert((FOLD_HS & (FOLD_HS - 1)) == 0 && FOLD_HC % NT == 0 && FOLD_MAXC <= NT, "fold table");
+
+template <bool SAMPLE>
+__global__ __launch_bounds__(NT) void k_fold_sc(const uint64_t *__restrict__ keys, const uint64_t *__restrict__ cb,
+                                                uint64_t nsc, int k, int F, int F2, uint32_t wmax, uint32_t stride,
+                                                uint64_t *__restrict__ mid, uint32_t *__restrict__ fcount,
+                                                unsigned long long *io) {
+    __shared__ unsigned long long s_k[FOLD_HS];
+    __shared__ uint32_t s_c[FOLD_HS];
+    __shared__ uint64_t s_cb[FOLD_MAXC + 1];
+    __shared__ uint32_t s_cc[FOLD_MAXC], s_cp[FOLD_MAXC];
+    __shared__ uint32_t s_tot;
+    const uint32_t tid = threadIdx.x;
+    const uint64_t sc = (uint64_t)blockIdx.x * stride;
+    if (sc >= nsc) return;
+    const uint32_t ncs = 1u << F2;
+    const uint64_t g0 = sc << F2;
+    if (tid <= ncs) s_cb[tid] = cb[g0 + tid];
+    __syncthreads();
+    const WKeySpec ws = wkey_spec(k);
+    const int sh = 2 * k - F;
+    uint64_t cursor = s_cb[0];
+    unsigned long long tin = 0, tout = 0;
+    for (uint32_t c = 0; c < ncs;) {
+        const uint64_t b0 = s_cb[c];
+        const uint32_t lane = tid & 63u;
+        const bool fits = lane >= c && lane < ncs && s_cb[lane + 1] - b0 <= FOLD_HC;
+        const uint64_t fm = __ballot(fits) >> c;
+        const uint32_t run = ~fm ? (uint32_t)__builtin_ctzll(~fm) : 64u;
+        const uint32_t e = c + (run ? run : 1u);
+        const uint64_t nb = s_cb[e] - b0;
+        if (nb > FOLD_HC || nb == 0) {
+            if constexpr (!SAMPLE) {
+                for (uint64_t i = tid; i < nb; i += NT) mid[cursor + i] = keys[b0 + i];
+                if (tid >= c && tid < e) fcount[g0 + tid] = (uint32_t)(s_cb[tid + 1] - s_cb[tid]);
+            }
+            tin += nb, tout += nb, cursor += nb;
+            c = e;
+            continue;
+        }
+        for (uint32_t s = tid; s < FOLD_HS; s += NT) s_k[s] = EMPTY_KEY, s_c[s] = 0;
+        if (tid < FOLD_MAXC) s_cc[tid] = 0;
+        __syncthreads();
+        uint64_t x[FOLD_KPT];
+#pragma unroll
+        for (int q = 0; q < FOLD_KPT; ++q) {
+            const uint32_t i = q * NT + tid;
+            x[q] = i < nb ? keys[b0 + i] : EMPTY_KEY;
+        }
+#pragma unroll
+        for (int q = 0; q < FOLD_KPT; ++q) {
+            if (x[q] == EMPTY_KEY) continue;
+            uint32_t wt;
+            const uint64_t key = wkey_split(x[q], ws, wt);
+            uint32_t s = (uint32_t)((key * 0x9e3779b97f4a7c15ull) >> (64 - __builtin_ctz(FOLD_HS)));
+            for (;;) {
+                unsigned long long cur = s_k[s];
+                if (cur == EMPTY_KEY) cur = atomicCAS(&s_k[s], EMPTY_KEY, (unsigned long long)key);
+                if (cur == EMPTY_KEY || cur == key) {
+                    atomicAdd(&s_c[s], wt);
+                    break;
+                }
+                s = (s + 1) & (FOLD_HS - 1);
+            }
+        }
+        __syncthreads();
+#pragma unroll
+        for (int q = 0; q < FOLD_SPT; ++q) {
+            const uint32_t s = q * NT + tid;
+            const unsigned long long key = s_k[s];
+            if (key != EMPTY_KEY) atomicAdd(&s_cc[(uint32_t)(key >> sh) & (ncs - 1)], (s_c[s] + wmax - 1) / wmax);
+        }
+        __syncthreads();
+        if (tid < 64) {
+            const uint32_t v = tid < ncs ? s_cc[tid] : 0u;
+            const uint32_t inc = wave_incl_sum<uint32_t>(v);
+            s_cp[tid] = inc - v;
+            if (tid == 63) s_tot = inc;
+            if constexpr (!SAMPLE)
+                if (tid >= c && tid < e) fcount[g0 + tid] = v;
+        }
+        __syncthreads();
+        const uint32_t btot = s_tot;
+        if constexpr (!SAMPLE) {
+#pragma unroll
+            for (int q = 0; q < FOLD_SPT; ++q) {
+                const uint32_t s = q * NT + tid;
+                const unsigned long long key = s_k[s];
+                if (key == EMPTY_KEY) continue;
+                const uint32_t m = s_c[s], ne = (m + wmax - 1) / wmax;
+                const uint64_t at = cursor + atomicAdd(&s_cp[(uint32_t)(key >> sh) & (ncs - 1)], ne);
+                for (uint32_t t = 0; t < ne; ++t) {
+                    const uint32_t w = t + 1 < ne ? wmax : m - (ne - 1) * wmax;
+                    mid[at + t] = key | ((uint64_t)(w - 1) << ws.wsh);
+                }
+            }
+        }
+        tin += nb, tout += btot, cursor += btot;
+        c = e;
+        __syncthreads();
+    }
+    if constexpr (SAMPLE) {
+        if (tid == 0) {
+            atomicAdd(&io[0], tin);
+            atomicAdd(&io[1], tout);
+        }
+    }
+}
+
+__global__ __launch_bounds__(NT) void k_fold_compact(const uint64_t *__restrict__ mid,
+                                                     const uint64_t *__restrict__ cb_raw,
+                                                     const uint64_t *__restrict__ cb_new,
+                                                     const uint32_t *__restrict__ fcount, int F2,
+                                                     uint64_t *__restrict__ keys, uint64_t *__restrict__ total) {
+    const uint32_t ncs = 1u << F2;
+    const uint64_t g0 = (uint64_t)blockIdx.x << F2;
+    const uint64_t src = cb_raw[g0], dst = cb_new[g0], n = cb_new[g0 + ncs] - dst;
+    for (uint64_t i = threadIdx.x; i < n; i += NT) keys[dst + i] = mid[src + i];
+    if (threadIdx.x < ncs) {
+        const uint64_t g = g0 + threadIdx.x;
+        total[g] -= (cb_raw[g + 1] - cb_raw[g]) - fcount[g];
+    }
+}
+
+hipError_t launch_fold_sc(const uint64_t *keys, const uint64_t *cb, uint32_t nlbins, int k, int F, int F2,
+                          uint32_t wmax, uint64_t *mid, uint32_t *fcount, hipStream_t s) {
+    const uint64_t nsc = (uint64_t)nlbins << (F - F2);
+    if (!nsc) return hipSuccess;
+    if (F2 > 6 || 2 * k > WKEY_MAX_BITS || wmax < 1 || wmax > WKEY_WMAX || nsc > 0x7fffffffull) return hipErrorInvalidValue;
+    k_fold_sc<false><<<(unsigned)nsc, NT, 0, s>>>(keys, cb, nsc, k, F, F2, wmax, 1u, mid, fcount, nullptr);
+    return hipGetLastError();
+}
+
+hipError_t launch_fold_sample(const uint64_t *keys, const uint64_t *cb, uint32_t nlbins, int k, int F, int F2,
+                              uint32_t wmax, uint32_t stride, unsigned long long *io, hipStream_t s) {
+    const uint64_t nsc = (uint64_t)nlbins << (F - F2);
+    if (!nsc) return hipSuccess;
+    if (F2 > 6 || 2 * k > WKEY_MAX_BITS || wmax < 1 || wmax > WKEY_WMAX || !stride || nsc > 0x7fffffffull)
+        return hipErrorInvalidValue;
+    k_fold_sc<true><<<(unsigned)((nsc + stride - 1) / stride), NT, 0, s>>>(keys, cb, nsc, k, F, F2, wmax, stride, nullptr,
+                                                                          nullptr, io);
+    return hipGetLastError();
+}
+
+hipError_t launch_fold_compact(const uint64_t *mid, const uint64_t *cb_raw, const uint64_t *cb_new,
+                               const uint32_t *fcount, uint32_t nlbins, int F, int F2, uint64_t *keys,
+                               uint64_t *total, hipStream_t s) {
+    const uint64_t nsc = (uint64_t)nlbins << (F - F2);
+    if (!nsc) return hipSuccess;
+    if (F2 > 6 || nsc > 0x7fffffffull) return hipErrorInvalidValue;
+    k_fold_compact<<<(unsigned)nsc, NT, 0, s>>>(mid, cb_raw, cb_new, fcount, F2, keys, total);
+    return hipGetLastError();
+}
diff --git a/fastkmer_amd/csrc/fk_internal.h b/fastkmer_amd/csrc/fk_internal.h
--- a/fastkmer_amd/csrc/fk_internal.h
+++ b/fastkmer_amd/csrc/fk_internal.h
@@ -39,13 +39,15 @@
     const uint64_t *pk[STAGE_MAXP] = {};
     const uint64_t *pcb[STAGE_MAXP] = {};
     const struct PieceStarts *starts = nullptr;
+    bool weighted = false;
 };
 struct PieceStarts {
     uint64_t s[STAGE_MAXP];
     uint32_t pre[STAGE_MAXP];
 };
 hipError_t launch_bucket_finish(const BucketSrc &src, struct Bucket *buckets, uint64_t nb, uint32_t nlbins,
-                                uint64_t total_keys, PieceStarts *out, hipStream_t s);
+                                const uint64_t *total_keys , PieceStarts *out,
+                                hipStream_t s);
 
 struct Chunk {
     uint64_t rec_begin, rec_end;
@@ -151,6 +153,16 @@
 hipError_t launch_bucket_count64_big(const BucketSrc &src, const Bucket *buckets, uint64_t nlist, int k,
                                      uint64_t *out_keys, uint32_t *out_counts, uint64_t *bucket_unique,
                                      unsigned long long *oversize, const uint32_t *list, hipStream_t s);
+constexpr int WKEY_MAX_BITS = 60;
+constexpr uint32_t WKEY_WMAX = 15;
+constexpr uint32_t FOLD_HC = 1024;
+hipError_t launch_fold_sc(const uint64_t *keys, const uint64_t *cb, uint32_t nlbins, int k, int F, int F2,
+                          uint32_t wmax, uint64_t *mid, uint32_t *fcount, hipStream_t s);
+hipError_t launch_fold_sample(const uint64_t *keys, const uint64_t *cb, uint32_t nlbins, int k, int F, int F2,
+                              uint32_t wmax, uint32_t stride, unsigned long long *io, hipStream_t s);
+hipError_t launch_fold_compact(const uint64_t *mid, const uint64_t *cb_raw, const uint64_t *cb_new,
+                               const uint32_t *fcount, uint32_t nlbins, int F, int F2, uint64_t *keys,
+                               uint64_t *total, hipStream_t s);
 constexpr uint32_t WAVE_BUCKET_CAP = 512;
 constexpr uint32_t WAVE_SLOTS = 640;
 constexpr uint32_t WAVE_MID_CAP = 1024;
@@ -204,8 +216,9 @@
                                  SubBucket *subs, SplitParent *parents, unsigned int *counts, uint32_t *fb0,
                                  uint32_t *fb1, uint32_t block_cap, int k, int F, hipStream_t s, bool retry = false);
 hipError_t launch_sub_count64_seq(const Bucket *buckets, const uint32_t *list, uint32_t nl, const SplitParent *parents,
-                                  const SubBucket *subs, const uint64_t *skeys, uint64_t *out_keys,
-                                  uint32_t *out_counts, uint64_t *bucket_unique, hipStream_t s, bool ordered);
+                                  const SubBucket *subs, const uint64_t *skeys, int k, bool weighted,
+                                  uint64_t *out_keys, uint32_t *out_counts, uint64_t *bucket_unique, hipStream_t s,
+                                  bool ordered);
 struct SubBucket128 {
     uint64_t src;
     uint64_t lo_hi, lo_lo;
diff --git a/fastkmer_amd/csrc/fk_kernels.hip b/fastkmer_amd/csrc/fk_kernels.hip
--- a/fastkmer_amd/csrc/fk_kernels.hip
+++ b/fastkmer_amd/csrc/fk_kernels.hip
@@ -301,6 +301,7 @@
 #include "fk_partition.inc"
 #include "fk_radix_rank.inc"
 #include "fk_count_sorted.inc"
+#include "fk_fold.inc"
 #include "fk_expand2.inc"
 #include "fk_sort_radix.inc"
 #include "fk_compact.inc"
diff --git a/fastkmer_amd/csrc/fk_radix_rank.inc b/fastkmer_amd/csrc/fk_radix_rank.inc
--- a/fastkmer_amd/csrc/fk_radix_rank.inc
+++ b/fastkmer_amd/csrc/fk_radix_rank.inc
@@ -4,14 +4,21 @@
 template <int KW>
 __device__ __forceinline__ uint32_t digit_of(u128 key, int sh) { return (uint32_t)(key >> sh) & 15u; }
 
+template <int KW>
+__device__ __forceinline__ typename KeyOf<KW>::T sort_kmask(int k) {
+    typedef typename KeyOf<KW>::T K;
+    if constexpr (KW == 1) return 2 * k <= WKEY_MAX_BITS ? (1ull << (2 * k)) - 1ull : ~0ull;
+    else return ~(K)0;
+}
+
 template <typename K, int IPT>
 __device__ __forceinline__ void tile_rank(const K (&key)[IPT], int n_valid_here, int sh, uint32_t *s_cnt,
                                           uint32_t *s_tmp, uint32_t (&pos)[IPT], uint32_t (&dig)[IPT],
-                                          uint32_t *digit_total ) {
+                                          uint32_t *digit_total , uint32_t dmask = 15u) {
     uint64_t lo = 0, hi = 0;
 #pragma unroll
     for (int it = 0; it < IPT; ++it) {
-        const uint32_t d = (uint32_t)(key[it] >> sh) & 15u;
+        const uint32_t d = (uint32_t)(key[it] >> sh) & dmask;
         dig[it] = d;
         if (it < n_valid_here) {
             const int f = 8 * (d & 7);
diff --git a/fastkmer_amd/csrc/fk_sort_radix.inc b/fastkmer_amd/csrc/fk_sort_radix.inc
--- a/fastkmer_amd/csrc/fk_sort_radix.inc
+++ b/fastkmer_amd/csrc/fk_sort_radix.inc
@@ -74,7 +74,9 @@
         kand = s_red[1][0] & s_red[1][1] & s_red[1][2] & s_red[1][3];
         __syncthreads();
     }
-    const K diff = kor ^ kand;
+    const K kmask = sort_kmask<KW>(k);
+    const K diff = (kor ^ kand) & kmask;
+    const bool weighted = ((kor & ~kmask) != 0);
     int lo_bit = 0, hi_bit = -1;
     if (diff != 0) {
         if constexpr (KW == 1) {
@@ -88,7 +90,7 @@
     }
     for (int sh = lo_bit & ~3; sh <= hi_bit; sh += 4) {
         uint32_t pos[IPT], dig[IPT];
-        tile_rank<K, IPT>(key, nv, sh, s_cnt, s_tmp, pos, dig, nullptr);
+        tile_rank<K, IPT>(key, nv, sh, s_cnt, s_tmp, pos, dig, nullptr, (uint32_t)(kmask >> sh) & 15u);
 #pragma unroll
         for (int it = 0; it < IPT; ++it)
             if (it < nv) s_keys[pos[it]] = key[it];
@@ -97,7 +99,7 @@
         for (int it = 0; it < IPT; ++it) key[it] = (it < nv) ? s_keys[my0 + it] : ~(K)0;
         __syncthreads();
     }
-    if (hi_bit < 0) {
+    if (hi_bit < 0 && !weighted) {
         if (threadIdx.x == 0) {
             store_key(out_keys, b.begin, key[0]);
             out_counts[b.begin] = (uint32_t)n;
@@ -112,7 +114,7 @@
 #pragma unroll
     for (int it = 0; it < IPT; ++it) {
         const int i = my0 + it;
-        if (i < n && (i == 0 || s_keys[i - 1] != key[it])) heads |= 1u << it;
+        if (i < n && (i == 0 || ((s_keys[i - 1] ^ key[it]) & kmask) != 0)) heads |= 1u << it;
     }
     uint32_t nu;
     uint32_t u = block_excl_sum<uint32_t>((uint32_t)__popc(heads), s_tmp, &nu);
@@ -123,8 +125,13 @@
     __syncthreads();
     for (uint32_t q = threadIdx.x; q < nu; q += NT) {
         const uint32_t hp = s_cnt[q];
-        store_key(out_keys, b.begin + q, s_keys[hp]);
-        out_counts[b.begin + q] = s_cnt[q + 1] - hp;
+        store_key(out_keys, b.begin + q, s_keys[hp] & kmask);
+        uint32_t cnt = s_cnt[q + 1] - hp;
+        if constexpr (KW == 1) {
+            if (weighted)
+                for (uint32_t j = hp, e = hp + cnt; j < e; ++j) cnt += (uint32_t)(s_keys[j] >> (2 * k));
+        }
+        out_counts[b.begin + q] = cnt;
     }
     if (threadIdx.x == 0) bucket_unique[qi] = nu;
 }
@@ -160,7 +167,7 @@
     __shared__ uint64_t s_hist[16];
     __shared__ K s_red[2][NT / 64];
     __shared__ K s_carry;
-    __shared__ uint64_t s_state[2];
+    __shared__ uint64_t s_state[3];
     __shared__ uint64_t s_soff;
 
     const uint32_t qi = list ? list[blockIdx.x] : blockIdx.x;
@@ -210,7 +217,9 @@
         kand = s_red[1][0] & s_red[1][1] & s_red[1][2] & s_red[1][3];
         __syncthreads();
     }
-    const K diff = kor ^ kand;
+    const K kmask = sort_kmask<KW>(k);
+    const int wsh = KW == 1 && 2 * k <= WKEY_MAX_BITS ? 2 * k : 0;
+    const K diff = (kor ^ kand) & kmask;
     int lo_bit = 0, hi_bit = -1;
     if (diff != 0) {
         if constexpr (KW == 1) {
@@ -223,12 +232,13 @@
         }
     }
     for (int sh = lo_bit & ~3; sh <= hi_bit; sh += 4) {
+        const uint32_t dmask = (uint32_t)(kmask >> sh) & 15u;
         if (threadIdx.x < 16) s_hist[threadIdx.x] = 0;
         __syncthreads();
         for (uint64_t i = threadIdx.x; i < n; i += NT) {
             K x;
             load_key(bufA, offA + i, x);
-            atomicAdd((unsigned long long *)&s_hist[(uint32_t)(x >> sh) & 15u], 1ull);
+            atomicAdd((unsigned long long *)&s_hist[(uint32_t)(x >> sh) & dmask], 1ull);
         }
         __syncthreads();
         if (threadIdx.x == 0) {
@@ -251,7 +261,7 @@
                     key[it] = ~(K)0;
             }
             uint32_t pos[IPT], dig[IPT];
-            tile_rank<K, IPT>(key, nv, sh, s_cnt, s_tmp, pos, dig, s_dtot);
+            tile_rank<K, IPT>(key, nv, sh, s_cnt, s_tmp, pos, dig, s_dtot, dmask);
 #pragma unroll
             for (int it = 0; it < IPT; ++it) {
                 if (it < nv) {
@@ -275,6 +285,7 @@
     if (threadIdx.x == 0) {
         s_state[0] = 0;
         s_state[1] = ~0ull;
+        s_state[2] = 0;
     }
     __syncthreads();
     for (uint64_t t0 = 0; t0 < n; t0 += TILE) {
@@ -296,47 +307,59 @@
             load_key(bufA, offA + my0 - 1, pk);
         else
             pk = ~(K)0;
-        uint32_t heads = 0;
+        uint32_t heads = 0, wsum = 0;
+        uint32_t wt[IPT];
 #pragma unroll
         for (int it = 0; it < IPT; ++it) {
-            if (it < nv && ((my0 + it) == 0 || key[it] != pk)) heads |= 1u << it;
+            if (it < nv && ((my0 + it) == 0 || ((key[it] ^ pk) & kmask) != 0)) heads |= 1u << it;
             pk = key[it];
+            wt[it] = it < nv ? 1u : 0u;
+            if constexpr (KW == 1)
+                if (wsh && it < nv) wt[it] += (uint32_t)(key[it] >> wsh);
+            wsum += wt[it];
         }
         __syncthreads();
 #pragma unroll
         for (int it = 0; it < IPT; ++it)
             if ((uint64_t)it + my0 == t0 + tlen - 1) s_carry = key[it];
-        uint32_t nh;
+        uint32_t nh, wtile;
         uint32_t u = block_excl_sum<uint32_t>((uint32_t)__popc(heads), s_tmp, &nh);
+        uint32_t wpre = block_excl_sum<uint32_t>(wsum, s_tmp, &wtile);
         const uint64_t ubase = s_state[0];
         const uint64_t open_head = s_state[1];
+        const uint64_t w0 = s_state[2];
         const uint32_t u0 = u;
 #pragma unroll
-        for (int it = 0; it < IPT; ++it)
-            if ((heads >> it) & 1u) s_cnt[u++] = (uint32_t)(threadIdx.x * IPT + it);
-        if (threadIdx.x == 0) s_cnt[nh] = (uint32_t)tlen;
+        for (int it = 0; it < IPT; ++it) {
+            if ((heads >> it) & 1u) s_cnt[u++] = wpre;
+            wpre += wt[it];
+        }
+        if (threadIdx.x == 0) s_cnt[nh] = wtile;
         __syncthreads();
         if (nh > 0 && threadIdx.x == 0 && open_head != ~0ull)
-            out_counts[b.begin + ubase - 1] = (uint32_t)(t0 + s_cnt[0] - open_head);
+            out_counts[b.begin + ubase - 1] = (uint32_t)(w0 + s_cnt[0] - open_head);
         u = u0;
 #pragma unroll
         for (int it = 0; it < IPT; ++it) {
             if ((heads >> it) & 1u) {
-                store_key(out_keys, b.begin + ubase + u, key[it]);
+                store_key(out_keys, b.begin + ubase + u, key[it] & kmask);
                 if (u + 1 < nh) out_counts[b.begin + ubase + u] = s_cnt[u + 1] - s_cnt[u];
                 ++u;
             }
         }
         __syncthreads();
-        if (threadIdx.x == 0 && nh > 0) {
-            s_state[0] = ubase + nh;
-            s_state[1] = t0 + s_cnt[nh - 1];
+        if (threadIdx.x == 0) {
+            if (nh > 0) {
+                s_state[0] = ubase + nh;
+                s_state[1] = w0 + s_cnt[nh - 1];
+            }
+            s_state[2] = w0 + wtile;
         }
         __syncthreads();
     }
     if (threadIdx.x == 0) {
         const uint64_t ub = s_state[0];
-        if (ub > 0) out_counts[b.begin + ub - 1] = (uint32_t)(n - s_state[1]);
+        if (ub > 0) out_counts[b.begin + ub - 1] = (uint32_t)(s_state[2] - s_state[1]);
         bucket_unique[qi] = ub;
     }
 }
diff --git a/include/fastkmer.h b/include/fastkmer.h
--- a/include/fastkmer.h
+++ b/include/fastkmer.h
@@ -187,6 +187,10 @@
 int fk_debug_wave_count(int32_t device, int32_t k, int32_t F, uint32_t c0, uint32_t c1, int32_t slots,
                         const uint64_t *keys, uint32_t n, uint64_t *out_keys, uint32_t *out_counts,
                         uint32_t *n_out);
+int fk_debug_wave_count_w(int32_t device, int32_t k, int32_t F, uint32_t c0, uint32_t c1, int32_t slots,
+                          const uint64_t *keys, uint32_t n, uint64_t *out_keys, uint32_t *out_counts,
+                          uint32_t *n_out);
+int fk_debug_fold_stats(const fk_ctx *ctx, uint64_t out[4]);
 
 int fk_debug_comm_hold(fk_ctx *ctx, int32_t max_seconds);
 int fk_debug_comm_release(fk_ctx *ctx);
```

After: 41.43 billion bases/s (median of 6 runs). 2.4% higher.
